# chymaera96/NeuralSampleID

Measured on AMD Instinct MI355X. Metric: audio clips/sec (contrastive step, grafp encoder), higher is better.
Workload: dtype bf16; 1 GPU; B=256 bf16 k=3 hipGraph 2-stream: grafp.yaml GraphEncoder('t') full contrastive step (fwd x2 views + NT-Xent + bwd + clip + Adam), synthetic (64,128) log-mel clip pairs per GPU, random-init weights; global_batch=256, k=3, parallelism=dp1, collectives=none (single process), gemm_arithmetic=bf16 MFMA operands, fp32 accumulate, activation_storage=bf16, views=two HIP streams (parallel graph branches), hipgraph=True

## Files before the change

include/nsid.h:

```cpp
#ifndef NSID_H
#define NSID_H
#include <stddef.h>
#include <stdint.h>

#ifdef __cplusplus
extern "C" {
#endif

#define NSID_OK 0
#define NSID_EINVAL (-1)
#define NSID_ELAUNCH (-2)

#define NSID_ACT_NONE 0
#define NSID_ACT_RELU 1
#define NSID_ACT_LEAKY 2
#define NSID_ACT_ELU 3

#define NSID_ROW_TILE 128

#define NSID_F32 0
#define NSID_BF16 1

#define NSID_GEMM_FP32 0
#define NSID_GEMM_BF16 1

int nsid_version(void);
int nsid_debug_gemm_trace(void* device_buf);
int nsid_debug_knn_trace(void* device_buf);
int nsid_set_gemm_precision(int mode);
int nsid_get_gemm_precision(void);
int nsid_set_tuning(const char* key, long value);
int nsid_get_tuning(const char* key, long* value);
int nsid_reset_tuning(void);
int nsid_tuning_count(void);
const char* nsid_tuning_key(int i);
long nsid_debug_counter(const char* key);
int nsid_debug_counters_reset(void);
int nsid_debug_counter_count(void);
const char* nsid_debug_counter_key(int i);
long nsid_gemm_g256_launches(void);
int nsid_row_tiles(int M);
long nsid_workspace_bytes(const char* op, long rows, long cols);

int nsid_linear_fwd(const void* x, int ldx, const void* w, int w_dtype, const float* bias, void* out, int ldo, int M,
                    int Nout, int K, int groups, const float* in_scale, const float* in_shift, int act_in, int act_out,
                    float* stat, int ksplit, int act_dtype , void* stream);
int nsid_linear_fwd_res(const void* x, int ldx, const void* w, int w_dtype, const float* bias, const void* addend, int ldadd,
                        void* out, int ldo, int M, int Nout, int K, int groups, const float* in_scale,
                        const float* in_shift, int act_in, int act_dtype, void* stream);
int nsid_ffn_fused_fwd(const void* x, const void* w1, const float* b1, const void* w2, const float* b2, void* out, int M, int C,
                       int H, void* stream);
int nsid_mrconv_fused_fwd(const void* y, const int32_t* idx, int B, int N, int C, int k, const void* w, const float* bias, void* out,
                          void* stream);
int nsid_linear_bwd_data(const void* dout, int ldd, const void* w, int w_dtype, const void* addend, int ldadd,
                         void* din, int ldi, int M, int Nout, int K, int groups,
                         int act_dtype , void* stream);
int nsid_linear_bwd_data_bn(const void* dout, int ldd, const void* w, int w_dtype, const void* addend, int ldadd,
                            void* din, int ldi, int M, int Nout, int K, int groups, int act_dtype, const void* bn_r,
                            const float* bn_scale, const float* bn_shift, const float* bn_mean, const float* bn_invstd,
                            int bn_act, float* bn_partial, void* stream);
int nsid_linear_bwd_data_bnapply(const void* dy, const void* r, const float* coef4, int act, void* dr, const void* w, int w_dtype,
                                 const void* addend, int ldadd, void* din, int ldi, int M, int Nout, int K, int groups,
                                 int act_dtype, const void* bn_r, const float* bn_scale, const float* bn_shift,
                                 const float* bn_mean, const float* bn_invstd, int bn_act, float* bn_partial, void* stream);
int nsid_linear_bwd_weight(const void* dout, int ldd, const void* x, int ldx, float* dw, int M, int Nout, int K,
                           int groups, const float* in_scale, const float* in_shift, int act_in,
                           int act_dtype , void* stream);
typedef struct nsid_wgrad_problem {
  const void* dout[2];
  const void* x[2];
  const float* in_scale[2];
  const float* in_shift[2];
  float* dw;
  int ldd, ldx, M, Nout, K, groups, act_in;
  int ds_out_nodes;
} nsid_wgrad_problem;
int nsid_linear_bwd_weight_grouped(const nsid_wgrad_problem* problems, int n, int act_dtype,
                                   int max_workgroups ,
                                   void* stream);
int nsid_colsum_acc(const void* x, int ldx, int M, int C, float* out, int dtype, void* stream);

int nsid_bn_finalize(const float* stat, int tiles, int C, int M, const float* gamma, const float* beta,
                     float* running_mean, float* running_var, int64_t* num_batches_tracked, float momentum,
                     float eps, float* scale, float* shift, float* mean, float* invstd, void* stream);
int nsid_bn_finalize_deferred(const float* stat, int tiles, int C, int M, const float* gamma, const float* beta, float eps,
                              float* scale, float* shift, float* mean, float* invstd, float* uvar, void* stream);
int nsid_bn_running_update(int n, const int* C, float* const* running_mean, float* const* running_var,
                           int64_t* const* num_batches_tracked, const float* const* mean_a, const float* const* uvar_a,
                           const float* const* mean_b, const float* const* uvar_b, float momentum, void* stream);
int nsid_bn_eval_affine(const float* gamma, const float* beta, const float* running_mean, const float* running_var,
                        float eps, int C, float* scale, float* shift, void* stream);
int nsid_bn_apply(const void* r, const float* scale, const float* shift, int act, const void* residual,
                  void* out, int M, int C, int dtype, void* stream);
int nsid_bn_bwd_reduce(const void* dout, const void* r, int M, int C, const float* scale, const float* shift,
                       const float* mean, const float* invstd, int act, float* partial, int dtype, void* stream);
int nsid_bn_bwd_finalize(const float* partial, int tiles, int C, int M, float* dgamma, float* dbeta, float* coef,
                         void* stream);
int nsid_bn_bwd_finalize_fused(const float* partial, int tiles, int C, int M, float* dgamma, float* dbeta, float* coef,
                               const float* scale, const float* shift, const float* mean, const float* invstd, float* coef4,
                               void* stream);
int nsid_bn_bwd_apply(const void* dout, const void* r, int M, int C, const float* scale, const float* shift,
                      const float* mean, const float* invstd, int act, const float* coef, void* dr, int dtype,
                      void* stream);

int nsid_knn_graph(const void* r, int ldr, const float* scale, const float* shift, int B, int N, int C, int k,
                   int dilation, int32_t* idx, int dtype, void* stream);

int nsid_mr_aggregate_fwd(const void* r, int ldr, const float* scale, const float* shift, const int32_t* idx, int B,
                          int N, int C, int k, void* u, uint8_t* argmax, int dtype, void* stream);
int nsid_mr_aggregate_bwd(const void* du, const int32_t* idx, const uint8_t* argmax, int B, int N, int C, int k,
                          void* dy, int dtype, void* stream);
int nsid_mr_aggregate_bwd_bn(const void* du, const int32_t* idx, const uint8_t* argmax, int B, int N, int C, int k, void* dy,
                             const void* bn_r, int bn_ldr, const float* bn_scale, const float* bn_shift, const float* bn_mean,
                             const float* bn_invstd, int bn_act, float* partial, int dtype, void* stream);

int nsid_batched_index_select_fwd(const float* x, const int32_t* idx, int B, int C, int N, int Nq, int k, float* out,
                                  void* stream);
int nsid_batched_index_select_bwd(const float* dout, const int32_t* idx, int B, int C, int N, int Nq, int k,
                                  float* dx , void* stream);

int nsid_downsample3_fwd(const void* x, int B, int N, int C, const void* wp, int w_dtype, const float* bias, void* out,
                         int Cout, float* stat, int act_dtype, void* stream);
int nsid_downsample3_bwd_weight(const void* dout, const void* x, float* dwp , int B, int N, int C, int Cout,
                                int act_dtype, void* stream);
int nsid_downsample3_bwd_data(const void* dout, const void* wp, const void* w_odd, int w_dtype, void* dx, int B, int N,
                              int C, int Cout, int act_dtype, void* stream);
int nsid_pack_ds_weight_bwd(const float* w, int Cout, int Cin, float* w_odd, void* stream);
int nsid_im2col3_fwd(const void* x, int B, int N, int C, void* col, int dtype, void* stream);
int nsid_im2col3_bwd(const void* dcol, int B, int N, int C, void* dx, int dtype, void* stream);
int nsid_pack_ds_weight(const float* w, int Cout, int Cin, float* wp, void* stream);
int nsid_dsact_fwd(const void* x, int B, int N, int C, const float* in_scale, const float* in_shift, int act_in, const float* w,
                   const float* bias, void* out, int Cout, float* stat, const float* out_scale, const float* out_shift, int act_out,
                   int act_dtype, void* stream);
int nsid_dsact_bwd_weight(const void* dout, const void* x, const float* in_scale, const float* in_shift, int act_in,
                          float* dw , int B, int N, int C, int Cout, int act_dtype, void* stream);
int nsid_dsact_bwd_data(const void* dout, const float* w, void* dx, int B, int N, int C, int Cout, const void* r_prev,
                        const float* scale, const float* shift, const float* mean, const float* invstd, int act, float* partial,
                        int act_dtype, void* stream);
int nsid_dsact_part_rows(int B, int N);
#define NSID_DS_PREPACK_MAX_LAYERS 8
int nsid_ds_prepack(int n, const float* const* w, void* const* wp16, void* const* wb16, float* const* dwp, const int* Cout,
                    const int* Cin, void* stream);
int nsid_unpack_ds_wgrad(const float* dwp, int Cout, int Cin, float* dw , void* stream);

int nsid_peak_patchify_fwd(const float* spec, const float* w, const float* bias, int B, int H, int W, int pb, int pf,
                           int F, void* out, int ldo, float* minmax, int out_dtype, void* stream);
int nsid_peak_patchify_bwd(const float* spec, const float* minmax, const void* out, const void* dout, int ldo,
                           int B, int H, int W, int pb, int pf, int F, float* dw , float* dbias ,
                           int out_dtype, void* stream);
int nsid_peak_patchify_bwd_ws(const float* spec, const float* minmax, const void* out, const void* dout, int ldo, int B, int H,
                              int W, int pb, int pf, int F, float* dw, float* dbias, float* ws, int out_dtype, void* stream);

int nsid_node_mean_fwd(const void* x, int B, int N, int C, float* out, int x_dtype, void* stream);
int nsid_node_mean_bwd(const float* dout, int B, int N, int C, void* dx, int dx_dtype, void* stream);
int nsid_elu_bwd(const float* dout, const float* out, long n, float* din, void* stream);
int nsid_l2norm_fwd(const float* p, int B, int d, float eps, float* z, float* norm, void* stream);
int nsid_l2norm_bwd(const float* dz, const float* z, const float* norm, int B, int d, float eps, float* dp,
                    void* stream);

int nsid_reflect_pad(const float* x, long L, int pad, float* out, void* stream);
int nsid_power_mel_db(const float* spec, long ld, int n_freq, const float* fb, const int* band, int n_mels, int T,
                      float* out, void* stream);
int nsid_unfold_segments(const float* logmel, int n_mels, int T, int n_frames, int step, int S, float* out, void* stream);
int nsid_logmel_fft(const float* wave, long in_stride, int B, long L, int n_fft, int hop, const float* window,
                    const float* twiddle, const float* fb, const int* band, int n_mels, float* out, long out_clip_stride,
                    long out_mel_stride, void* stream);

#define NSID_CQT_GROUP_BINS 8
#define NSID_CQT_RC 256
int nsid_cqt(const float* wave, long in_stride, int B, long L, int hop, int width, int n_bins, const int* groups, int n_groups,
             const float* taps, long taps_len, const float* scale, float* out, long out_clip_stride, long out_bin_stride,
             void* stream);

#define NSID_PACK_COLS 4
#define NSID_LOGMEL_RUN 8
#define NSID_CQT_TILE 32
int nsid_logmel_fft_ragged(const float* pack, const long* songs, int n_songs, long max_len, long total_runs, long total_cols,
                           int n_fft, int hop, const float* window, const float* twiddle, const float* fb, const int* band,
                           int n_mels, float* out, long ld, void* stream);
int nsid_cqt_ragged(const float* pack, const long* songs, int n_songs, long max_len, long total_tiles, long total_cols, int hop,
                    int width, int n_bins, const int* groups, int n_groups, const float* taps, long taps_len, const float* scale,
                    float* out, long ld, void* stream);
int nsid_unfold_segments_ragged(const float* spec, long ld, int n_rows, int n_frames, const long* seg_col, long s0, int nseg,
                                float* out, void* stream);

#define NSID_AUG_N_FFT 2048
#define NSID_AUG_HOP 512
#define NSID_AUG_BINS 1025
#define NSID_AUG_ZEROS 64
#define NSID_AUG_PRECISION 512
int nsid_aug_stft(const float* x_i, long stride_i, const float* x_j, long stride_j, int B, long L, const float* gain,
                  const float* window, const float* twiddle, float* spec, void* stream);
int nsid_aug_vocoder(const float* spec, int B, long L, const float* rate, float rate_lo, float rate_hi, float* out,
                     long T_out_max, void* stream);
int nsid_aug_istft(const float* spec, long T_out_max, int B, long L, const float* rate, float rate_lo, float rate_hi,
                   const float* window, const float* twiddle, float* wave, long wave_stride, void* stream);
int nsid_aug_finish(const float* wave, long wave_stride, int B, long L, const int* mode, const float* rate, float rate_lo,
                    float rate_hi, const float* table, float* out, long out_stride, void* stream);

#define NSID_AUG_FX_MAX_SECTIONS 64
#define NSID_AUG_FX_MAX_FRAMES 256
int nsid_aug_compress(const float* x, long stride_x, int B, long L, const int* mode1, const double* cmp, float* out, long stride_o,
                      void* stream);
int nsid_aug_biquad(const float* x, long stride_x, int B, long L, const int* mode1, const double* sos, int S, const int* n_sec,
                    float* out, long stride_o, void* stream);
int nsid_aug_frames(const float* x_i, long stride_i, const float* t1, long stride_t, const float* gain, int B, long L,
                    const int* mode2, const int* frame_size, const int* frame_ops, int F, float* out, long stride_o, void* stream);

#define NSID_RESAMPLE_MAX_C 8
#define NSID_RESAMPLE_LDS_BYTES 65536
int nsid_resample_sinc(const float* x, long stride_x, int C, long T, int orig, int nw, int width, const float* table,
                       const int* first, int ntap, int ts, float* y, long T_out, void* stream);
int nsid_stem_pairs_gate(const float* bank, long bank_elems, const long* base, const int* length, int n_tracks, const int* track,
                         const int* start, const float* key, const int* off_i, const int* off_j, int N, long L, long O, float silence,
                         int* status, float* snr, int* plan, void* stream);
int nsid_stem_pairs_build(const float* bank, long bank_elems, const long* base, const int* length, int n_tracks, const int* track,
                          const int* start, const int* off_i, const int* off_j, const int* status, const int* plan, int N, long L,
                          long O, int packed, int B_out, float* x_i, long stride_i, float* x_j, long stride_j, int* n_ok, void* stream);

int nsid_f32_to_bf16(const float* src, void* dst, long n, void* stream);

size_t nsid_ntxent_ws_floats(int Bg);
int nsid_ntxent_fwd_bwd(const float* z_i, const float* z_j, int Bg, int d, float tau, int p0, int np, float* ws,
                        float* loss_out, float* dz_i, float* dz_j, void* stream);

#define NSID_BL_MAX 2048
size_t nsid_baseline_loss_ws_floats(int M, int D);
int nsid_pair_ce_fwd_bwd(const float* z_i, const float* z_j, int B, int D, float* ws, float* out, float* dz_i, float* dz_j,
                         void* stream);
int nsid_triplet_fwd_bwd(const float* e, const int64_t* labels, int M, int D, double margin, float* ws, float* out, float* de,
                         void* stream);
int nsid_baseline_objective_fwd_bwd(const float* z_i, const float* z_j, int B, int D, double margin, double beta, double gamma,
                                    float* ws, float* out, float* dz_i, float* dz_j, void* stream);

#define NSID_BL_ROWS_MAX 4096
size_t nsid_baseline_loss_rows_ws_floats(int M, int D);
int nsid_baseline_objective_rows_fwd_bwd(const float* z_i_all, const float* z_j_all, int Bg, int D, int p0, int npairs,
                                         double margin, double beta, double gamma, float* ws, float* out, float* dz_i, float* dz_j,
// ... 125 lines not shown
```

neuralsampleid_amd/csrc/bn.hip:

```cpp
#include <cstdlib>
#include "nsid_common.h"

namespace {

constexpr int FIN_THREADS = 1024;

template <int FIN_CH>
__device__ __forceinline__ void tile_sums(const float* __restrict__ p0, const float* __restrict__ p1, int tiles,
                                          int C, int c, int tg, bool ok, double* red0, double* red1, double& sum,
                                          double& sq) {
  constexpr int FIN_TG = FIN_THREADS / FIN_CH;
  double a = 0.0, b = 0.0;
  if (ok) {
    constexpr int UB = 8;
    int t = tg;
    for (; t + (UB - 1) * FIN_TG < tiles; t += UB * FIN_TG) {
      float va[UB], vb[UB];
#pragma unroll
      for (int u = 0; u < UB; ++u) {
        va[u] = p0[(long)(t + u * FIN_TG) * C + c];
        vb[u] = p1[(long)(t + u * FIN_TG) * C + c];
      }
#pragma unroll
      for (int u = 0; u < UB; ++u) { a += (double)va[u]; b += (double)vb[u]; }
// ... 234 lines not shown
  long b = (nchunks + 255) / 256;
  const long cap = nsid_tune(NSID_T_stream_max_wg);
  return (int)(b > cap ? cap : (b < 1 ? 1 : b));
}

template <typename T>
__global__ __launch_bounds__(256) void colsum_atomic_kernel(const T* __restrict__ x, long ld, int M, int C,
                                                            float* __restrict__ out) {
  constexpr int N = Chunk<T>::N;
  constexpr int CQ = CR_CH / N, RG = 256 / CQ, ROWS = NSID_ROW_TILE / RG;
  __shared__ float red[RG][CR_CH];
  const int row0 = blockIdx.x * NSID_ROW_TILE;
  const int t = threadIdx.x, q = t % CQ, rgp = t / CQ;
  const int c = blockIdx.y * CR_CH + N * q;
  float s[N];
#pragma unroll
  for (int e = 0; e < N; ++e) s[e] = 0.f;
  if (c < C)
    for (int i = 0; i < ROWS; ++i) {
      const int row = row0 + rgp + RG * i;
      if (row < M) {
        float d[N];
        Chunk<T>::load(x + (long)row * ld + c, d);
#pragma unroll
        for (int e = 0; e < N; ++e) s[e] += d[e];
      }
    }
#pragma unroll
  for (int e = 0; e < N; ++e) red[rgp][N * q + e] = s[e];
  __syncthreads();
  if (t < CR_CH && blockIdx.y * CR_CH + t < C) {
    float a = 0.f;
    for (int g = 0; g < RG; ++g) a += red[g][t];
    atomicAdd(out + blockIdx.y * CR_CH + t, a);
  }
}

inline long chunk_keeping_grid(long nchunks, int CV, int U, long max_wg, bool* capped) {
  int g0 = CV, d256 = 256;
  while (d256 % 2 == 0 && g0 % 2 == 0) { d256 /= 2; g0 /= 2; }
  long want = (nchunks + 256L * U - 1) / (256L * U);
  if (capped) *capped = want > max_wg;
  if (want > max_wg) want = max_wg;
  if (want < 1) want = 1;
  return (want + g0 - 1) / g0 * g0;
}

inline int bn_fin_ch(int tiles) {
  const int t = (int)nsid_tune(NSID_T_bn_fin_tiles);
  return (t > 0 && tiles >= t) ? 16 : 64;
}
#define NSID_FIN_LAUNCH(kernel, tiles, C, stream, ...)                                                                      \
  do {                                                                                                                       \
    if (bn_fin_ch(tiles) == 16)                                                                                              \
      NSID_LAUNCH(kernel<16>, dim3(((C) + 15) / 16), dim3(FIN_THREADS), 0, static_cast<hipStream_t>(stream), __VA_ARGS__);   \
    else                                                                                                                     \
      NSID_LAUNCH(kernel<64>, dim3(((C) + 63) / 64), dim3(FIN_THREADS), 0, static_cast<hipStream_t>(stream), __VA_ARGS__);   \
  } while (0)

}

extern "C" int nsid_bn_finalize(const float* stat, int tiles, int C, int M, const float* gamma, const float* beta,
                                float* running_mean, float* running_var, int64_t* nbt, float momentum, float eps,
                                float* scale, float* shift, float* mean, float* invstd, void* stream) {
  NSID_REQUIRE(stat && gamma && beta && scale && shift && mean && invstd && C > 0 && M > 0);
  NSID_REQUIRE(tiles == nsid_row_tiles(M) || (tiles > 0 && tiles <= NSID_STEM7_STAT_MAX));
  NSID_REQUIRE((running_mean == nullptr) == (running_var == nullptr));
  NSID_FIN_LAUNCH(bn_finalize_kernel, tiles, C, stream, stat, tiles, C, M, gamma, beta, running_mean, running_var, nbt,
              momentum, eps, scale, shift, mean, invstd, static_cast<float*>(nullptr));
  return nsid_launch_status();
}

extern "C" int nsid_bn_finalize_deferred(const float* stat, int tiles, int C, int M, const float* gamma,
                                         const float* beta, float eps, float* scale, float* shift, float* mean,
                                         float* invstd, float* uvar, void* stream) {
  NSID_REQUIRE(stat && gamma && beta && scale && shift && mean && invstd && uvar && C > 0 && M > 0);
  NSID_REQUIRE(tiles == nsid_row_tiles(M));
  NSID_FIN_LAUNCH(bn_finalize_kernel, tiles, C, stream, stat, tiles, C, M, gamma, beta, static_cast<float*>(nullptr),
              static_cast<float*>(nullptr), static_cast<int64_t*>(nullptr), 0.f, eps, scale, shift, mean, invstd, uvar);
  return nsid_launch_status();
}

namespace {
constexpr int RU_LAYERS = 16;
struct RunUpdArgs {
  float* rm[RU_LAYERS]; float* rv[RU_LAYERS]; int64_t* nbt[RU_LAYERS];
  const float* mean_a[RU_LAYERS]; const float* uvar_a[RU_LAYERS];
  const float* mean_b[RU_LAYERS]; const float* uvar_b[RU_LAYERS];
  int C[RU_LAYERS];
  float momentum;
};
__global__ __launch_bounds__(256) void bn_running_update_kernel(const RunUpdArgs a) {
  const int l = blockIdx.x;
  const float m = a.momentum;
  const bool two = a.mean_b[l] != nullptr;
  if (threadIdx.x == 0 && a.nbt[l] != nullptr) *a.nbt[l] += two ? 2 : 1;
  for (int c = threadIdx.x; c < a.C[l]; c += blockDim.x) {
    float rm = running_blend(a.rm[l][c], a.mean_a[l][c], m);
    float rv = running_blend(a.rv[l][c], a.uvar_a[l][c], m);
    if (two) {
      rm = running_blend(rm, a.mean_b[l][c], m);
      rv = running_blend(rv, a.uvar_b[l][c], m);
    }
    a.rm[l][c] = rm;
    a.rv[l][c] = rv;
  }
}
}

extern "C" int nsid_bn_running_update(int n, const int* C, float* const* running_mean, float* const* running_var,
                                      int64_t* const* num_batches_tracked, const float* const* mean_a,
                                      const float* const* uvar_a, const float* const* mean_b,
                                      const float* const* uvar_b, float momentum, void* stream) {
  NSID_REQUIRE(n > 0 && C && running_mean && running_var && mean_a && uvar_a);
  for (int base = 0; base < n; base += RU_LAYERS) {
    RunUpdArgs a{};
    const int cnt = n - base < RU_LAYERS ? n - base : RU_LAYERS;
    for (int i = 0; i < cnt; ++i) {
      NSID_REQUIRE(C[base + i] > 0 && running_mean[base + i] && running_var[base + i] && mean_a[base + i] && uvar_a[base + i]);
      a.rm[i] = running_mean[base + i]; a.rv[i] = running_var[base + i];
      a.nbt[i] = num_batches_tracked ? num_batches_tracked[base + i] : nullptr;
      a.mean_a[i] = mean_a[base + i]; a.uvar_a[i] = uvar_a[base + i];
      a.mean_b[i] = mean_b ? mean_b[base + i] : nullptr; a.uvar_b[i] = uvar_b ? uvar_b[base + i] : nullptr;
      NSID_REQUIRE((a.mean_b[i] == nullptr) == (a.uvar_b[i] == nullptr));
      a.C[i] = C[base + i];
    }
    a.momentum = momentum;
    NSID_LAUNCH(bn_running_update_kernel, dim3(cnt), dim3(256), 0, static_cast<hipStream_t>(stream), a);
    const int rc = nsid_launch_status();
    if (rc != NSID_OK) return rc;
  }
  return NSID_OK;
}

extern "C" int nsid_bn_eval_affine(const float* gamma, const float* beta, const float* running_mean,
                                   const float* running_var, float eps, int C, float* scale, float* shift,
                                   void* stream) {
  NSID_REQUIRE(gamma && beta && running_mean && running_var && scale && shift && C > 0);
  NSID_LAUNCH(bn_eval_affine_kernel, dim3((C + 127) / 128), dim3(128), 0, static_cast<hipStream_t>(stream), gamma, beta,
              running_mean, running_var, eps, C, scale, shift);
  return nsid_launch_status();
}

extern "C" int nsid_bn_apply(const void* r, const float* scale, const float* shift, int act, const void* residual,
                             void* out, int M, int C, int dtype, void* stream) {
  NSID_REQUIRE(r && scale && shift && out && M > 0 && C > 0 && NSID_DTYPE_OK(dtype));
  NSID_REQUIRE(C % (dtype == NSID_BF16 ? 8 : 4) == 0 && nsid_aligned16(r) && nsid_aligned16(out));
  NSID_DISPATCH_DTYPE(dtype, T, {
    const long nchunks = (long)M * C / Chunk<T>::N;
    NSID_LAUNCH((bn_apply_kernel<T>), dim3(stream_grid(nchunks)), dim3(256), 0, static_cast<hipStream_t>(stream),
                static_cast<const T*>(r), scale, shift, act, static_cast<const T*>(residual), static_cast<T*>(out),
                nchunks, C / Chunk<T>::N);
  });
  return nsid_launch_status();
}

extern "C" int nsid_bn_bwd_reduce(const void* dout, const void* r, int M, int C, const float* scale,
                                  const float* shift, const float* mean, const float* invstd, int act, float* partial,
                                  int dtype, void* stream) {
  NSID_REQUIRE(dout && r && scale && shift && mean && invstd && partial && M > 0 && C > 0 && NSID_DTYPE_OK(dtype));
  NSID_REQUIRE(C % (dtype == NSID_BF16 ? 8 : 4) == 0);
  NSID_REQUIRE(act == NSID_ACT_NONE || act == NSID_ACT_RELU || act == NSID_ACT_LEAKY);
  const int tiles = nsid_row_tiles(M);
  NSID_DISPATCH_DTYPE(dtype, T, {
    NSID_LAUNCH((col_reduce_kernel<1, T>), dim3(tiles, (C + CR_CH - 1) / CR_CH), dim3(256), 0,
                static_cast<hipStream_t>(stream), static_cast<const T*>(dout), static_cast<const T*>(r), (long)C, M, C,
                scale, shift, mean, invstd, bn_slope(act), partial, tiles);
  });
  return nsid_launch_status();
}

extern "C" int nsid_bn_bwd_finalize(const float* partial, int tiles, int C, int M, float* dgamma, float* dbeta,
                                    float* coef, void* stream) {
  NSID_REQUIRE(partial && coef && C > 0 && M > 0 && tiles >= 1);
  NSID_FIN_LAUNCH(bn_bwd_finalize_kernel, tiles, C, stream, partial, tiles, C, M, dgamma, dbeta, coef, static_cast<const float*>(nullptr),
              static_cast<const float*>(nullptr), static_cast<const float*>(nullptr), static_cast<const float*>(nullptr),
              static_cast<float*>(nullptr));
  return nsid_launch_status();
}

extern "C" int nsid_bn_bwd_finalize_fused(const float* partial, int tiles, int C, int M, float* dgamma, float* dbeta,
                                          float* coef, const float* scale, const float* shift, const float* mean,
                                          const float* invstd, float* coef4, void* stream) {
  NSID_REQUIRE(partial && coef && coef4 && scale && shift && mean && invstd && C > 0 && M > 0 && tiles >= 1);
  NSID_FIN_LAUNCH(bn_bwd_finalize_kernel, tiles, C, stream, partial, tiles, C, M, dgamma, dbeta, coef, scale, shift, mean, invstd, coef4);
  return nsid_launch_status();
}

extern "C" int nsid_bn_bwd_apply(const void* dout, const void* r, int M, int C, const float* scale,
                                 const float* shift, const float* mean, const float* invstd, int act,
                                 const float* coef, void* dr, int dtype, void* stream) {
  NSID_REQUIRE(dout && r && scale && shift && mean && invstd && coef && dr && M > 0 && C > 0 && NSID_DTYPE_OK(dtype));
  NSID_REQUIRE(C % (dtype == NSID_BF16 ? 8 : 4) == 0);
  NSID_REQUIRE(act == NSID_ACT_NONE || act == NSID_ACT_RELU || act == NSID_ACT_LEAKY);
  NSID_DISPATCH_DTYPE(dtype, T, {
    constexpr int U = 4;
    const int CV = C / Chunk<T>::N;
    const long nchunks = (long)M * CV;
    int g0 = CV, d256 = 256;
    while (d256 % 2 == 0 && g0 % 2 == 0) { d256 /= 2; g0 /= 2; }
    long want = (nchunks + 256L * U - 1) / (256L * U);
    const long max_wg = nsid_tune(NSID_T_bn_bwd_apply_max_wg);
    nsid_count(NSID_C_bn_bwd_apply);
    if (want > max_wg) { want = max_wg; nsid_count(NSID_C_bn_bwd_apply_capped); }
    const long grid = (want + g0 - 1) / g0 * g0;
    NSID_LAUNCH((bn_bwd_apply_kernel<T, U>), dim3((int)grid), dim3(256), 0, static_cast<hipStream_t>(stream),
                static_cast<const T*>(dout), static_cast<const T*>(r), (long)M, CV, scale, shift, mean,
                invstd, bn_slope(act), coef, static_cast<T*>(dr));
  });
  return nsid_launch_status();
// ... 12 lines not shown
```

neuralsampleid_amd/csrc/gemm.hip:

```cpp
#include <algorithm>
#include <cstdlib>
#include "nsid_common.h"

namespace {

inline float act_slope(int act) { return act == NSID_ACT_RELU ? 0.f : (act == NSID_ACT_LEAKY ? 0.2f : 1.f); }

struct GemmArgs {
  const void* A; long lda; long a_goff;
  const void* B; long ldb; long b_goff;
  void* C; long ldc; long c_goff;
  int I, J, R;
  const float* a_scale; const float* a_shift; float a_slope; long a_aff_goff;
  const float* b_scale; const float* b_shift; float b_slope; long b_aff_goff;
  const float* bias; long bias_goff;
  const void* addend; long ldadd;
  float* stat; long stat_plane;
  long stat_ld;
  int rsplit;
  int rchunk;
  int atomic_out;
  int split_major;
  const void* bn_r; long bn_ldr;
  const float* bn_scale; const float* bn_shift; const float* bn_mean; const float* bn_invstd; float bn_slope;
// ... 632 lines not shown
                }
              p.bn_partial[((long)ti * STILES + t2) * p.bn_ld + col] = a0;
              p.bn_partial[p.bn_plane + ((long)ti * STILES + t2) * p.bn_ld + col] = a1;
            }
          }
        }
      }
    }
  }
  if (p.stat != nullptr) {
    const float* red = lds + WAVES * RB * ((BN / 2) + 4);
    if (threadIdx.x < BN) {
      const int j = j0 + threadIdx.x;
      if (FULL || j < p.J) {
        const long col = g * p.c_goff + j;
#pragma unroll
        for (int t2 = 0; t2 < STILES; ++t2) {
          float s = 0.f, q = 0.f;
#pragma unroll
          for (int k = 4 * WPT * t2; k < 4 * WPT * (t2 + 1); ++k) {
            s += red[(0 * WROWS * 4 + k) * BN + threadIdx.x];
            q += red[(1 * WROWS * 4 + k) * BN + threadIdx.x];
          }
          p.stat[((long)ti * STILES + t2) * p.stat_ld + col] = s;
          p.stat[p.stat_plane + ((long)ti * STILES + t2) * p.stat_ld + col] = q;
        }
      }
    }
  }
  if (trace && threadIdx.x == 0) {
    unsigned hw, xcc;
    asm volatile("s_getreg_b32 %0, hwreg(HW_REG_HW_ID)" : "=s"(hw));
    asm volatile("s_getreg_b32 %0, hwreg(HW_REG_XCC_ID)" : "=s"(xcc));
    const long lin = blockIdx.x + (long)gridDim.x * (blockIdx.y + (long)gridDim.y * blockIdx.z);
    trace[4 * lin + 0] = t_start;
    trace[4 * lin + 1] = t_loop;
    trace[4 * lin + 2] = __builtin_amdgcn_s_memrealtime();
    trace[4 * lin + 3] = ((unsigned long long)xcc << 32) | hw;
  }
}

template <int BM, int BN, bool A_RMAJOR, bool B_RMAJOR, bool H, bool ST, bool AAFF, bool WB = false, bool FULL = false,
          bool ARELU = false, int KS = 1, int PADX = 0, bool ABN = false>
__global__ __launch_bounds__(NT, KS > 1 ? 2 : ((FULL && WB && BM == 128 && !AAFF && (BN == 128) != ABN) ? 3 : 2))
void gemm_kernel(const GemmArgs p) {
  int bid = p.split_major ? blockIdx.y : blockIdx.x;
  const int split = p.split_major ? blockIdx.x : blockIdx.y;
  if (!p.split_major) {
    const int nwg = gridDim.x;
    if ((nwg & 7) == 0) bid = (bid & 7) * (nwg >> 3) + (bid >> 3);
  }
  gemm_body<BM, BN, A_RMAJOR, B_RMAJOR, H, ST, AAFF, WB, FULL, ARELU, KS, PADX, ABN>(p, bid, split, blockIdx.z);
}

template <int BM, int BN, bool FULL, bool H = true, bool ST = true, int PADX = 0>
__device__ __forceinline__ void wgrad_grouped_item(const WgGroupArgs& ga, const int w);

template <int BM, int BN, bool FULL, bool H = true, bool ST = true, int PADX = 0>
__global__ __launch_bounds__(256, FULL ? 1 : 2) void wgrad_grouped_kernel(const WgGroupArgs ga) {
  const int total = ga.wg0[ga.n];
  for (int w = blockIdx.x; w < total; w += gridDim.x) wgrad_grouped_item<BM, BN, FULL, H, ST, PADX>(ga, w);
}

template <int BM, int BN, bool FULL, bool H, bool ST, int PADX>
__device__ __forceinline__ void wgrad_grouped_item(const WgGroupArgs& ga, const int w) {
  int pi, split, bid, g, seg;
  if (!wgg_decode(ga, w, pi, split, bid, g, seg)) return;
  const WgProb& q = ga.prob[pi];
  GemmArgs p{};
  p.A = q.A[seg]; p.lda = q.lda; p.a_goff = q.I;
  p.B = q.B[seg]; p.ldb = q.ldb; p.b_goff = q.J;
  p.C = q.C; p.ldc = q.J; p.c_goff = (long)q.I * q.J;
  p.I = q.I; p.J = q.J; p.R = q.R;
  p.b_scale = q.bsc[seg]; p.b_shift = q.bsh[seg]; p.b_slope = q.slope; p.b_aff_goff = q.J;
  p.a_slope = 1.f; p.bn_slope = 1.f;
  p.atomic_out = 1;
  p.rchunk = q.rchunk; p.rsplit = q.nsplit;
  if constexpr (PADX == 2) {
    p.pad_period = q.pad_period; p.pad_phase = 0; p.pad_c0 = 0; p.pad_c1 = q.pad_c1; p.pad_safe = q.pad_c1;
  }
  gemm_body<BM, BN, false, false, H, ST, false, false, FULL, false, FULL ? 2 : 1, PADX>(p, bid, split, g);
}

__global__ void elu_inplace_kernel(float* __restrict__ x, long rows, int cols, long ld) {
  const long n = rows * cols;
  for (long i = (long)blockIdx.x * blockDim.x + threadIdx.x; i < n; i += (long)gridDim.x * blockDim.x) {
    float* q = x + (i / cols) * ld + (i % cols);
    const float v = *q;
    *q = v > 0.f ? v : expm1f(v);
  }
}

int g_gemm_precision = NSID_GEMM_FP32;
long g_g256_launches = 0;

template <int BM, int BN, bool AR, bool BR>
int launch(GemmArgs p, int groups, hipStream_t s, int act_dtype, bool w_bf16 = false) {
  const int tiles = ((p.I + BM - 1) / BM) * ((p.J + BN - 1) / BN);
  const bool st16 = act_dtype == NSID_BF16;
  const bool half = g_gemm_precision == NSID_GEMM_BF16 || st16;
  const int bk = half ? 32 : 16;
  p.rchunk = (p.rchunk + bk - 1) / bk * bk;
  p.rsplit = (p.R + p.rchunk - 1) / p.rchunk;
  p.split_major = p.rsplit > 1 && (p.rsplit % 8) == 0;
  dim3 grid(p.split_major ? p.rsplit : tiles, p.split_major ? tiles : p.rsplit, groups);
  constexpr bool CAN_AFF = AR && BR;
  const bool aff = CAN_AFF && p.a_scale != nullptr;
#define NSID_GEMM_GO(HH, SS)                                                                              \
  do {                                                                                                    \
    if (aff) NSID_LAUNCH((gemm_kernel<BM, BN, AR, BR, HH, SS, CAN_AFF>), grid, dim3(256), 0, s, p);        \
    else NSID_LAUNCH((gemm_kernel<BM, BN, AR, BR, HH, SS, false>), grid, dim3(256), 0, s, p);              \
  } while (0)
  const bool full = st16 && p.I % BM == 0 && p.J % BN == 0 && p.rchunk % (2 * bk) == 0 && p.R % p.rchunk == 0;
  const long deep_maxwg = nsid_tune(NSID_T_gemm_deep_max_wg);
  const int deep_kinds = (int)nsid_tune(NSID_T_gemm_deep_kinds);
  constexpr int kind_bit = AR ? (BR ? 1 : 2) : 4;
  const long wgs = (long)tiles * p.rsplit * groups;
  const int ks = (full && wgs <= deep_maxwg && nsid_tune(NSID_T_gemm_deep_ks) == 2 && (deep_kinds & kind_bit) && p.rchunk % 128 == 0) ? 2 : 1;
  if (p.abn_r != nullptr) {
    if (!(AR && !BR && BM == 128)) return NSID_EINVAL;
    if (!(st16 && w_bf16 && full)) return 1;
  }
  nsid_count(AR ? (BR ? NSID_C_gemm_fwd : NSID_C_gemm_bwd_data) : NSID_C_gemm_bwd_weight);
  if (p.split_major) nsid_count(NSID_C_gemm_split_major);
  if (aff) nsid_count(NSID_C_gemm_affine_load);
  if (AR && !BR && p.bn_r != nullptr) nsid_count(NSID_C_gemm_bn_sums);
  if (!AR) nsid_count(BM == BN ? NSID_C_wgrad_square : NSID_C_wgrad_rect);
  {
    const bool deep_path = st16 && full && (AR ? w_bf16 : true);
    if (deep_path) {
      nsid_count(NSID_C_gemm_full);
      if (ks == 2) nsid_count(NSID_C_gemm_ks2);
    }
  }
#define NSID_GEMM_DEEP_GO(AFF_, WB_, RELU_)                                                                                  \
  do {                                                                                                                       \
    if (ks == 2) NSID_LAUNCH((gemm_kernel<BM, BN, AR, BR, true, true, AFF_, WB_, true, RELU_, 2>), grid, dim3(256), 0, s, p); \
    else NSID_LAUNCH((gemm_kernel<BM, BN, AR, BR, true, true, AFF_, WB_, true, RELU_>), grid, dim3(256), 0, s, p);           \
  } while (0)
  if (p.abn_r != nullptr) {
    if constexpr (AR && !BR && BM == 128) {
      nsid_count(NSID_C_gemm_bn_apply_load);
      NSID_LAUNCH((gemm_kernel<BM, BN, AR, BR, true, true, false, true, true, false, 1, 0, true>), grid, dim3(256), 0, s, p);
      return nsid_launch_status();
    } else {
      return NSID_EINVAL;
    }
  }
  if constexpr (AR) {
    if (st16 && w_bf16) {
      const bool act_only = CAN_AFF && p.a_scale == nullptr && p.a_slope != 1.f;
      if (act_only) {
        if constexpr (CAN_AFF) {
          if (!full || p.a_slope != 0.f) return NSID_EINVAL;
          NSID_GEMM_DEEP_GO(false, true, true);
        }
      } else if (full) {
        if (aff) NSID_GEMM_DEEP_GO(CAN_AFF, true, false);
        else NSID_GEMM_DEEP_GO(false, true, false);
      } else {
        if (aff) NSID_LAUNCH((gemm_kernel<BM, BN, AR, BR, true, true, CAN_AFF, true>), grid, dim3(256), 0, s, p);
        else NSID_LAUNCH((gemm_kernel<BM, BN, AR, BR, true, true, false, true>), grid, dim3(256), 0, s, p);
      }
      return nsid_launch_status();
    }
  } else {
    if (st16 && full) {
      NSID_GEMM_DEEP_GO(false, false, false);
// ... 54 lines not shown
  p.bias = bias; p.bias_goff = Cout;
  p.stat = stat; p.stat_ld = Cout; p.stat_plane = (long)nsid_row_tiles(M) * Cout;
  p.rsplit = 1; p.rchunk = 3 * C;
  p.pad_period = No; p.pad_phase = 0; p.pad_c0 = 0; p.pad_c1 = C; p.pad_safe = C;
  hipStream_t s = static_cast<hipStream_t>(stream);
  const bool wb = w_dtype == NSID_BF16;
  if (Cout <= 64) return launch_pad<128, 64, true, true, 1>(p, 1, s, act_dtype, wb);
  return launch_pad<128, 128, true, true, 1>(p, 1, s, act_dtype, wb);
}


extern "C" int nsid_downsample3_bwd_weight(const void* dout, const void* x, float* dwp, int B, int N, int C, int Cout,
                                           int act_dtype, void* stream) {
  NSID_REQUIRE(dout && x && dwp && B > 0 && N > 0 && N % 2 == 0 && C > 0 && Cout > 0 && NSID_DTYPE_OK(act_dtype));
  const int ch = act_dtype == NSID_BF16 ? 8 : 4;
  NSID_REQUIRE(C % ch == 0 && Cout % ch == 0 && nsid_aligned16(dout) && nsid_aligned16(x));
  const int No = N / 2, M = B * No;
  const long esz = act_dtype == NSID_BF16 ? 2 : 4;
  GemmArgs p{};
  p.A = dout; p.lda = Cout; p.a_goff = Cout;
  p.B = static_cast<const char*>(x) - (long)C * esz; p.ldb = 2L * C; p.b_goff = 3L * C;
  p.C = dwp; p.ldc = 3L * C; p.c_goff = (long)Cout * 3 * C;
  p.I = Cout; p.J = 3 * C; p.R = M;
  p.b_slope = 1.f;
  p.atomic_out = 1;
  p.pad_period = No; p.pad_phase = 0; p.pad_c0 = 0; p.pad_c1 = C; p.pad_safe = C;
  const long tiles = (long)((Cout + 63) / 64) * ((3 * C + 63) / 64);
  long S = std::min<long>((M + 1023) / 1024, std::max<long>(1, 1024 / tiles));
  S = std::max<long>(S, (256 + tiles - 1) / tiles);
  S = std::min<long>(S, (M + 255) / 256);
  p.rsplit = (int)std::max<long>(S, 1);
  p.rchunk = (M + p.rsplit - 1) / p.rsplit;
  return launch_pad<64, 64, false, false, 2>(p, 1, static_cast<hipStream_t>(stream), act_dtype, false);
}

extern "C" int nsid_downsample3_bwd_data(const void* dout, const void* wp, const void* w_odd, int w_dtype, void* dx, int B,
                                         int N, int C, int Cout, int act_dtype, void* stream) {
  NSID_REQUIRE(dout && wp && w_odd && dx && B > 0 && N > 0 && N % 2 == 0 && C > 0 && Cout > 0 && NSID_DTYPE_OK(act_dtype));
  const int ch = act_dtype == NSID_BF16 ? 8 : 4;
  NSID_REQUIRE(C % ch == 0 && Cout % ch == 0 && nsid_aligned16(dout) && nsid_aligned16(wp) && nsid_aligned16(w_odd) &&
               nsid_aligned16(dx) && NSID_DTYPE_OK(w_dtype) && (w_dtype == NSID_F32 || act_dtype == NSID_BF16));
  const int No = N / 2, M = B * No;
  const long esz = act_dtype == NSID_BF16 ? 2 : 4, wsz = w_dtype == NSID_BF16 ? 2 : 4;
  hipStream_t s = static_cast<hipStream_t>(stream);
  const bool wb = w_dtype == NSID_BF16;
  GemmArgs p{};
  p.A = dout; p.lda = Cout; p.a_goff = Cout;
  p.B = static_cast<const char*>(wp) + (long)C * wsz; p.ldb = 3L * C; p.b_goff = 0;
  p.C = dx; p.ldc = 2L * C; p.c_goff = C;
  p.I = M; p.J = C; p.R = Cout;
  p.rsplit = 1; p.rchunk = Cout;
  p.bn_slope = 1.f;
  int rc = C <= 64 ? launch<128, 64, true, false>(p, 1, s, act_dtype, wb) : launch<128, 128, true, false>(p, 1, s, act_dtype, wb);
  if (rc != NSID_OK) return rc;
  GemmArgs q{};
  q.A = dout; q.lda = Cout; q.a_goff = 2L * Cout;
  q.B = w_odd; q.ldb = C; q.b_goff = 0;
  q.C = static_cast<char*>(dx) + (long)C * esz; q.ldc = 2L * C; q.c_goff = C;
  q.I = M; q.J = C; q.R = 2 * Cout;
  q.rsplit = 1; q.rchunk = 2 * Cout;
  q.bn_slope = 1.f;
  q.pad_period = No; q.pad_phase = No - 1; q.pad_c0 = Cout; q.pad_c1 = 2 * Cout; q.pad_safe = 0;
  return C <= 64 ? launch_pad<128, 64, true, false, 1>(q, 1, s, act_dtype, wb)
                 : launch_pad<128, 128, true, false, 1>(q, 1, s, act_dtype, wb);
}

void* g_gemm_trace_host = nullptr;
extern "C" int nsid_debug_gemm_trace(void* buf) {
  g_gemm_trace_host = buf;
  return hipMemcpyToSymbol(HIP_SYMBOL(g_gemm_trace), &buf, sizeof(buf)) == hipSuccess ? NSID_OK : NSID_EINVAL;
}
extern "C" int nsid_set_gemm_precision(int mode) {
  if (mode != NSID_GEMM_FP32 && mode != NSID_GEMM_BF16) return NSID_EINVAL;
  g_gemm_precision = mode;
  return NSID_OK;
}
extern "C" int nsid_get_gemm_precision(void) { return g_gemm_precision; }
extern "C" long nsid_gemm_g256_launches(void) { return g_g256_launches; }
extern "C" int nsid_row_tiles(int M) { return (M + NSID_ROW_TILE - 1) / NSID_ROW_TILE; }

static int linear_fwd_impl(const void* x, int ldx, const void* w, int w_dtype, const float* bias, void* out, int ldo,
                           int M, int Nout, int K, int groups, const float* in_scale, const float* in_shift, int act_in,
                           int act_out, float* stat, int ksplit, int act_dtype, const void* addend, int ldadd,
                           void* stream);

extern "C" int nsid_linear_fwd(const void* x, int ldx, const void* w, int w_dtype, const float* bias, void* out, int ldo,
                               int M, int Nout, int K, int groups, const float* in_scale, const float* in_shift,
                               int act_in, int act_out, float* stat, int ksplit, int act_dtype, void* stream) {
  return linear_fwd_impl(x, ldx, w, w_dtype, bias, out, ldo, M, Nout, K, groups, in_scale, in_shift, act_in, act_out, stat,
                         ksplit, act_dtype, nullptr, 0, stream);
}

extern "C" int nsid_linear_fwd_res(const void* x, int ldx, const void* w, int w_dtype, const float* bias,
                                   const void* addend, int ldadd, void* out, int ldo, int M, int Nout, int K, int groups,
                                   const float* in_scale, const float* in_shift, int act_in, int act_dtype,
                                   void* stream) {
  const int ch = act_dtype == NSID_BF16 ? 8 : 4;
  NSID_REQUIRE(addend && ldadd % ch == 0 && ldadd >= groups * Nout && nsid_aligned16(addend));
  return linear_fwd_impl(x, ldx, w, w_dtype, bias, out, ldo, M, Nout, K, groups, in_scale, in_shift, act_in,
                         NSID_ACT_NONE, nullptr, 1, act_dtype, addend, ldadd, stream);
}

static int linear_fwd_impl(const void* x, int ldx, const void* w, int w_dtype, const float* bias, void* out, int ldo,
                           int M, int Nout, int K, int groups, const float* in_scale, const float* in_shift, int act_in,
                           int act_out, float* stat, int ksplit, int act_dtype, const void* addend, int ldadd,
                           void* stream) {
  NSID_REQUIRE(x && w && out && M > 0 && Nout > 0 && K > 0 && groups > 0 && ksplit >= 1 && NSID_DTYPE_OK(act_dtype));
  NSID_REQUIRE(NSID_DTYPE_OK(w_dtype) && (w_dtype == NSID_F32 || (act_dtype == NSID_BF16 && K % 8 == 0)));
  const int ch = act_dtype == NSID_BF16 ? 8 : 4;
  NSID_REQUIRE(K % ch == 0 && ldx % ch == 0 && nsid_aligned16(x) && nsid_aligned16(w) && K % 4 == 0);
  NSID_REQUIRE(act_dtype == NSID_F32 || (ksplit == 1 && (act_out == NSID_ACT_NONE || act_out == NSID_ACT_RELU) && Nout % 8 == 0 && ldo % 8 == 0));
  NSID_REQUIRE(act_out != NSID_ACT_RELU || (ksplit == 1 && stat == nullptr && addend == nullptr));
  NSID_REQUIRE((ldx >= groups * K || (groups == 1 && ldx > 0)) && ldo >= groups * Nout);
  NSID_REQUIRE(Nout % 4 == 0 && ldo % 4 == 0 && nsid_aligned16(out) && (bias == nullptr || nsid_aligned16(bias)));
  NSID_REQUIRE((in_scale == nullptr) == (in_shift == nullptr));
  NSID_REQUIRE(ksplit == 1 || (stat == nullptr && (act_out == NSID_ACT_NONE || (act_out == NSID_ACT_ELU && act_dtype == NSID_F32))));
  NSID_REQUIRE(act_in != NSID_ACT_ELU && (act_out == NSID_ACT_NONE || act_out == NSID_ACT_ELU || act_out == NSID_ACT_RELU));
  NSID_REQUIRE(in_scale != nullptr || act_in == NSID_ACT_NONE ||
               (act_in == NSID_ACT_RELU && act_dtype == NSID_BF16 && w_dtype == NSID_BF16));
  GemmArgs p{};
  p.A = x; p.lda = ldx; p.a_goff = K;
  p.B = w; p.ldb = K; p.b_goff = (long)Nout * K;
  p.C = out; p.ldc = ldo; p.c_goff = Nout;
  p.I = M; p.J = Nout; p.R = K;
  p.a_scale = in_scale; p.a_shift = in_shift; p.a_slope = act_slope(act_in); p.a_aff_goff = K;
  p.bias = bias; p.bias_goff = Nout;
  p.addend = addend; p.ldadd = ldadd;
  p.stat = stat; p.stat_ld = (long)groups * Nout; p.stat_plane = (long)nsid_row_tiles(M) * groups * Nout;
  p.rsplit = ksplit;
  p.rchunk = (K + ksplit - 1) / ksplit;
  p.atomic_out = ksplit > 1;
  p.relu_out = act_out == NSID_ACT_RELU;
  hipStream_t s = static_cast<hipStream_t>(stream);
  const long t128 = (long)nsid_row_tiles(M) * ((Nout + 127) / 128) * groups;
  const bool half = g_gemm_precision == NSID_GEMM_BF16 || act_dtype == NSID_BF16;
  const int force_narrow = (int)nsid_tune(NSID_T_fwd_narrow);
  bool narrow = half ? (Nout <= 64 || (Nout <= 128 && K <= 256 && in_scale == nullptr)) : Nout <= 64;
  if (half && t128 < 128) narrow = true;
  if (force_narrow >= 0 && Nout > 64) narrow = force_narrow != 0;
  const bool wb = w_dtype == NSID_BF16;
  if ((nsid_tune(NSID_T_ws_gemm) & 1) && act_dtype == NSID_BF16 && wb && ksplit == 1 && act_out == NSID_ACT_NONE && addend == nullptr &&
      act_in != NSID_ACT_ELU) {
    const int rcw = nsid_ws_fwd_launch(x, ldx, w, bias, out, ldo, M, Nout, K, groups, in_scale, in_shift, act_slope(act_in), stat,
                                       p.stat_plane, p.stat_ld, s);
    if (rcw != 1) { nsid_count(NSID_C_ws_fwd); return rcw; }
  }
  const long g256_min = nsid_tune(NSID_T_g256_min);
  if (g256_min > 0 && (stat == nullptr || nsid_tune(NSID_T_g256_train) != 0) && act_dtype == NSID_BF16 && wb && groups == 1 && in_scale == nullptr && ksplit == 1 &&
      (act_out == NSID_ACT_NONE || act_out == NSID_ACT_RELU) && act_in == NSID_ACT_NONE && ldx >= K &&
      (long)(M / 256) * (Nout / 256) >= g256_min) {
    const int rc256 = nsid_gemm256_fwd_launch(x, ldx, w, bias, addend, ldadd, out, ldo, M, Nout, K, act_out == NSID_ACT_RELU, stat,
                                              p.stat_plane, p.stat_ld, s);
    if (rc256 != 1) { ++g_g256_launches; nsid_count(NSID_C_gemm256); return rc256; }
  }
  const int rc = narrow ? launch<128, 64, true, true>(p, groups, s, act_dtype, wb) : launch<128, 128, true, true>(p, groups, s, act_dtype, wb);
  if (rc != NSID_OK || act_out != NSID_ACT_ELU) return rc;
  const long n = (long)M * groups * Nout;
  NSID_LAUNCH(elu_inplace_kernel, dim3((int)((n + 255) / 256 > 2048 ? 2048 : (n + 255) / 256)), dim3(256), 0, s,
              static_cast<float*>(out), (long)M, groups * Nout, (long)ldo);
  return nsid_launch_status();
}

struct AbnArgs {
  const void* r; const float* coef4; int act; void* dr;
};
static int linear_bwd_data_impl(const void* dout, int ldd, const void* w, int w_dtype, const void* addend, int ldadd,
                                void* din, int ldi, int M, int Nout, int K, int groups, int act_dtype, void* stream,
                                const void* bn_r, const float* bn_scale, const float* bn_shift, const float* bn_mean,
                                const float* bn_invstd, int bn_act, float* bn_partial, const AbnArgs* abn = nullptr);

extern "C" int nsid_linear_bwd_data(const void* dout, int ldd, const void* w, int w_dtype, const void* addend, int ldadd,
                                    void* din, int ldi, int M, int Nout, int K, int groups, int act_dtype,
                                    void* stream) {
  return linear_bwd_data_impl(dout, ldd, w, w_dtype, addend, ldadd, din, ldi, M, Nout, K, groups, act_dtype, stream,
                              nullptr, nullptr, nullptr, nullptr, nullptr, NSID_ACT_NONE, nullptr);
}

extern "C" int nsid_linear_bwd_data_bn(const void* dout, int ldd, const void* w, int w_dtype, const void* addend,
                                       int ldadd, void* din, int ldi, int M, int Nout, int K, int groups, int act_dtype,
                                       const void* bn_r, const float* bn_scale, const float* bn_shift,
                                       const float* bn_mean, const float* bn_invstd, int bn_act, float* bn_partial,
                                       void* stream) {
  NSID_REQUIRE(bn_r && bn_scale && bn_shift && bn_mean && bn_invstd && bn_partial && act_dtype == NSID_BF16);
  NSID_REQUIRE(ldi == groups * K && (groups * K) % 8 == 0 && nsid_aligned16(bn_r));
  NSID_REQUIRE(bn_act == NSID_ACT_NONE || bn_act == NSID_ACT_RELU || bn_act == NSID_ACT_LEAKY);
  return linear_bwd_data_impl(dout, ldd, w, w_dtype, addend, ldadd, din, ldi, M, Nout, K, groups, act_dtype, stream,
                              bn_r, bn_scale, bn_shift, bn_mean, bn_invstd, bn_act, bn_partial);
}

extern "C" int nsid_linear_bwd_data_bnapply(const void* dy, const void* r, const float* coef4, int act, void* dr, const void* w,
                                            int w_dtype, const void* addend, int ldadd, void* din, int ldi, int M, int Nout, int K,
                                            int groups, int act_dtype, const void* bn_r, const float* bn_scale,
                                            const float* bn_shift, const float* bn_mean, const float* bn_invstd, int bn_act,
                                            float* bn_partial, void* stream) {
  NSID_REQUIRE(dy && r && coef4 && dr && nsid_aligned16(r) && nsid_aligned16(dr) && nsid_aligned16(coef4));
  NSID_REQUIRE(dr != dy && dr != r);
  NSID_REQUIRE(act == NSID_ACT_NONE || act == NSID_ACT_RELU || act == NSID_ACT_LEAKY);
  if (act_dtype != NSID_BF16 || w_dtype != NSID_BF16 || (groups * Nout) % 8 != 0) return 1;
  if (bn_r != nullptr) {
    NSID_REQUIRE(bn_scale && bn_shift && bn_mean && bn_invstd && bn_partial && ldi == groups * K && (groups * K) % 8 == 0 &&
                 nsid_aligned16(bn_r));
    NSID_REQUIRE(bn_act == NSID_ACT_NONE || bn_act == NSID_ACT_RELU || bn_act == NSID_ACT_LEAKY);
  }
  const AbnArgs abn{r, coef4, act, dr};
  return linear_bwd_data_impl(dy, groups * Nout, w, w_dtype, addend, ldadd, din, ldi, M, Nout, K, groups, act_dtype, stream, bn_r,
                              bn_scale, bn_shift, bn_mean, bn_invstd, bn_act, bn_partial, &abn);
}

static int linear_bwd_data_impl(const void* dout, int ldd, const void* w, int w_dtype, const void* addend, int ldadd,
                                void* din, int ldi, int M, int Nout, int K, int groups, int act_dtype, void* stream,
                                const void* bn_r, const float* bn_scale, const float* bn_shift, const float* bn_mean,
                                const float* bn_invstd, int bn_act, float* bn_partial, const AbnArgs* abn) {
  NSID_REQUIRE(dout && w && din && M > 0 && Nout > 0 && K > 0 && groups > 0 && NSID_DTYPE_OK(act_dtype));
  NSID_REQUIRE(NSID_DTYPE_OK(w_dtype) && (w_dtype == NSID_F32 || (act_dtype == NSID_BF16 && K % 8 == 0)));
  const bool wb = w_dtype == NSID_BF16;
  const int ch = act_dtype == NSID_BF16 ? 8 : 4;
  NSID_REQUIRE(Nout % ch == 0 && K % ch == 0 && ldd % ch == 0 && ldi % ch == 0 && nsid_aligned16(dout) && nsid_aligned16(w));
  NSID_REQUIRE(addend == nullptr || ldadd % ch == 0);
  NSID_REQUIRE(ldd >= groups * Nout && ldi >= groups * K && ldi % 4 == 0 && nsid_aligned16(din));
  NSID_REQUIRE(addend == nullptr || (ldadd % 4 == 0 && ldadd >= groups * K && nsid_aligned16(addend)));
  GemmArgs p{};
  p.A = dout; p.lda = ldd; p.a_goff = Nout;
  p.B = w; p.ldb = K; p.b_goff = (long)Nout * K;
  p.C = din; p.ldc = ldi; p.c_goff = K;
  p.I = M; p.J = K; p.R = Nout;
  p.addend = addend; p.ldadd = ldadd;
  p.rsplit = 1; p.rchunk = Nout;
  p.bn_r = bn_r; p.bn_ldr = (long)groups * K;
  p.bn_scale = bn_scale; p.bn_shift = bn_shift; p.bn_mean = bn_mean; p.bn_invstd = bn_invstd;
  p.bn_slope = act_slope(bn_act);
  p.bn_partial = bn_partial; p.bn_ld = (long)groups * K; p.bn_plane = (long)nsid_row_tiles(M) * groups * K;
  hipStream_t s = static_cast<hipStream_t>(stream);
  const long t128 = (long)nsid_row_tiles(M) * ((K + 127) / 128) * groups;
  const bool half = g_gemm_precision == NSID_GEMM_BF16 || act_dtype == NSID_BF16;
  const int force_narrow = (int)nsid_tune(NSID_T_bwd_narrow);
  bool narrow = half ? (K <= 64 || (K <= 128 && Nout <= 256)) : K <= 64;
  if (half && t128 < 128) narrow = true;
  if (force_narrow >= 0 && K > 64) narrow = force_narrow != 0;
  if ((nsid_tune(NSID_T_ws_gemm) & (abn ? 4 : 2)) && act_dtype == NSID_BF16 && wb &&
      (bn_r == nullptr || bn_partial != nullptr)) {
    const int rcw = nsid_ws_bwd_data_launch(dout, ldd, w, addend, ldadd, din, ldi, M, Nout, K, groups, bn_r, p.bn_ldr, bn_scale, bn_shift,
                                            bn_mean, bn_invstd, p.bn_slope, bn_partial, p.bn_plane, p.bn_ld, abn ? abn->r : nullptr,
                                            abn ? abn->coef4 : nullptr, (long)groups * Nout, abn ? act_slope(abn->act) : 1.f,
                                            abn ? abn->dr : nullptr, (long)groups * Nout, s);
    if (rcw != 1) { nsid_count(abn ? NSID_C_ws_bwd_bnapply : NSID_C_ws_bwd_data); return rcw; }
  }
  if (abn != nullptr) {
    narrow = K <= 64;
    p.abn_r = abn->r; p.abn_coef = abn->coef4; p.abn_plane = (long)groups * Nout; p.abn_slope = act_slope(abn->act);
    p.abn_dr = abn->dr; p.abn_lddr = (long)groups * Nout;
    if (K % (narrow ? 64 : 128) != 0 || M % 128 != 0 || Nout % 64 != 0) return 1;
  }
  if (act_dtype == NSID_F32 && addend == nullptr && bn_r == nullptr && abn == nullptr && groups == 1 && Nout >= 1024 && ldi == K) {
    const long tiles = (long)nsid_row_tiles(M) * ((K + (narrow ? 63 : 127)) / (narrow ? 64 : 128));
    const long maxt = nsid_tune(NSID_T_bwd_split_max_tiles);
    const long S = maxt > 0 && tiles <= maxt ? std::min<long>(256 / tiles, Nout / 256) : 1;
    if (S > 1) {
      const int rcz = nsid_fill_zero(din, (size_t)M * K * 4, stream);
      if (rcz != NSID_OK) return rcz;
      p.rsplit = (int)S;
      p.rchunk = (int)((Nout + S - 1) / S);
      p.atomic_out = 1;
      nsid_count(NSID_C_gemm_bwd_split);
    }
  }
  if (narrow) return launch<128, 64, true, false>(p, groups, s, act_dtype, wb);
  return launch<128, 128, true, false>(p, groups, s, act_dtype, wb);
}

extern "C" int nsid_linear_bwd_weight(const void* dout, int ldd, const void* x, int ldx, float* dw, int M, int Nout,
                                      int K, int groups, const float* in_scale, const float* in_shift, int act_in,
                                      int act_dtype, void* stream) {
  NSID_REQUIRE(dout && x && dw && M > 0 && Nout > 0 && K > 0 && groups > 0 && NSID_DTYPE_OK(act_dtype));
  const int ch = act_dtype == NSID_BF16 ? 8 : 4;
  NSID_REQUIRE(Nout % ch == 0 && K % ch == 0 && ldd % ch == 0 && ldx % ch == 0 && nsid_aligned16(dout) && nsid_aligned16(x));
  NSID_REQUIRE((in_scale == nullptr) == (in_shift == nullptr));
  GemmArgs p{};
  p.A = dout; p.lda = ldd; p.a_goff = Nout;
  p.B = x; p.ldb = ldx; p.b_goff = K;
  p.C = dw; p.ldc = K; p.c_goff = (long)Nout * K;
  p.I = Nout; p.J = K; p.R = M;
  p.b_scale = in_scale; p.b_shift = in_shift; p.b_slope = act_slope(act_in); p.b_aff_goff = K;
  p.atomic_out = 1;
  const bool use_wide = nsid_tune(NSID_T_wgrad_wide) != 0;
  if (use_wide && act_dtype == NSID_BF16 && nsid_aligned16(dout) && nsid_aligned16(x) &&
      (in_scale == nullptr || (nsid_aligned16(in_scale) && nsid_aligned16(in_shift)))) {
    const int rc = nsid_wgrad2_launch(dout, ldd, x, ldx, dw, M, Nout, K, groups, in_scale, in_shift, act_slope(act_in),
                                      static_cast<hipStream_t>(stream));
    if (rc != 1) return rc;
  }
  const long rect = nsid_tune(NSID_T_wgrad_rect);
  const long wg_rect = nsid_tune(NSID_T_wgrad_wgs_rect);
  const long wg_sq = nsid_tune(NSID_T_wgrad_wgs_sq);
  if (rect && act_dtype == NSID_BF16 && Nout % 128 == 0 && K % 64 == 0 && M % 1024 == 0) {
    const long tiles_r = (long)(Nout / 128) * (K / 64) * groups;
    const long S = std::min<long>(M / 1024, std::max<long>(1, wg_rect / tiles_r));
    const long rect_min = nsid_tune(NSID_T_wgrad_rect_min);
    if (tiles_r * S >= rect_min) {
      p.rsplit = (int)S;
      p.rchunk = (int)(M / S);
      return launch<128, 64, false, false>(p, groups, static_cast<hipStream_t>(stream), act_dtype);
    }
  }
  const bool half = g_gemm_precision == NSID_GEMM_BF16 || act_dtype == NSID_BF16;
  const long t128 = (long)((Nout + 127) / 128) * ((K + 127) / 128) * groups;
  const bool small = half || (Nout <= 64 || K <= 64) || t128 * ((M + 511) / 512) < 256;
  const int bm = small ? 64 : 128;
  const long tiles = (long)((Nout + bm - 1) / bm) * ((K + bm - 1) / bm) * groups;
  long S;
  if (half) {
    S = std::min<long>((M + 1023) / 1024, std::max<long>(1, wg_sq / tiles));
    const long sq_min = nsid_tune(NSID_T_wgrad_sq_min);
    S = std::max<long>(S, (sq_min + tiles - 1) / tiles);
    S = std::min<long>(S, (M + 255) / 256);
  } else {
    S = std::min<long>((512 + tiles - 1) / tiles, (M + 511) / 512);
  }
  int rsplit = (int)std::max<long>(S, 1);
  p.rsplit = rsplit;
  p.rchunk = (M + rsplit - 1) / rsplit;
  hipStream_t s = static_cast<hipStream_t>(stream);
  if (small) return launch<64, 64, false, false>(p, groups, s, act_dtype);
  return launch<128, 128, false, false>(p, groups, s, act_dtype);
}

extern "C" int nsid_linear_bwd_weight_grouped(const nsid_wgrad_problem* problems, int n, int act_dtype, int max_workgroups,
                                              void* stream) {
  NSID_REQUIRE(problems && n > 0 && NSID_DTYPE_OK(act_dtype) && max_workgroups >= 0);
  const bool st16 = act_dtype == NSID_BF16;
  const int ch = st16 ? 8 : 4;
  hipStream_t s = static_cast<hipStream_t>(stream);
  const long rows_target = std::max<long>(128, nsid_tune(NSID_T_wgg_rows));
  const long rows_sq = std::max<long>(128, nsid_tune(NSID_T_wgg_rows_sq)), rows_gen = std::max<long>(32, nsid_tune(NSID_T_wgg_rows_gen));
  const bool use_w3 = nsid_tune(NSID_T_wgg_w3) != 0;
  const bool use_w4 = nsid_tune(NSID_T_wgrad256) != 0;
  const long rows_w4 = std::max<long>(128, nsid_tune(NSID_T_wgg_rows256));
  constexpr int NCLS = 8;
  WgGroupArgs ga[NCLS];
  long wgs[NCLS] = {0, 0, 0, 0, 0, 0, 0, 0};
  const bool half = g_gemm_precision == NSID_GEMM_BF16 || st16;
  for (int c = 0; c < NCLS; ++c) ga[c].n = 0;
// ... 102 lines not shown
```

neuralsampleid_amd/csrc/misc.hip:

```cpp
#include <algorithm>
#include "nsid_common.h"

namespace {

inline int grid_for(long n, int cap = 2048) {
  long b = (n + 255) / 256;
  return (int)(b > cap ? cap : (b < 1 ? 1 : b));
}

template <typename T>
__global__ __launch_bounds__(256) void im2col3_fwd_kernel(const T* __restrict__ x, int B, int N, int No, int C,
                                                          T* __restrict__ col) {
  constexpr int NV = Chunk<T>::N;
  const int CV = C / NV;
  const long total = (long)B * No * 3 * CV;
  for (long q = (long)blockIdx.x * blockDim.x + threadIdx.x; q < total; q += (long)gridDim.x * blockDim.x) {
    const int cv = (int)(q % CV);
    const int t = (int)((q / CV) % 3);
    const long orow = q / (3L * CV);
    const int b = (int)(orow / No), no = (int)(orow % No);
    const int n = 2 * no - 1 + t;
    float v[NV];
#pragma unroll
    for (int e = 0; e < NV; ++e) v[e] = 0.f;
// ... 308 lines not shown
__global__ __launch_bounds__(256) void patchify_bwd2_kernel(const float* __restrict__ spec, const float* __restrict__ minmax,
                                                            const T* __restrict__ out, const T* __restrict__ dout, int ldo,
                                                            float* __restrict__ ws) {
  constexpr int H = 64, W = 128, PBk = 4, PFk = 8, F = 8, Hp = 16, Wp = 16, NP = 256, LDW = W + PATCH_PAD;
  __shared__ __attribute__((aligned(16))) float g[NP * F];
  __shared__ __attribute__((aligned(16))) float xs[H * LDW];
  __shared__ float red[(Wp + Hp) * F];
  const int t = threadIdx.x, b = blockIdx.x;
  const float* x = spec + (long)b * H * W;
  const float lo = minmax[2 * b], range = minmax[2 * b + 1] - lo;
  {
    const long o = ((long)b * NP + t) * ldo;
    float ov[8], dv[8];
    if constexpr (Chunk<T>::N == 8) {
      Chunk<T>::load(out + o, ov);
      Chunk<T>::load(dout + o, dv);
    } else {
      Chunk<T>::load(out + o, ov); Chunk<T>::load(out + o + 4, ov + 4);
      Chunk<T>::load(dout + o, dv); Chunk<T>::load(dout + o + 4, dv + 4);
    }
    f32x4 v[8];
#pragma unroll
    for (int u = 0; u < 8; ++u) v[u] = *reinterpret_cast<const f32x4*>(x + 4 * (t + 256 * u));
#pragma unroll
    for (int e = 0; e < 8; ++e) g[t * F + e] = ov[e] > 0.f ? dv[e] : 0.f;
#pragma unroll
    for (int u = 0; u < 8; ++u) {
      const int i4 = 4 * (t + 256 * u), hh = i4 / W, ww = i4 % W;
      *reinterpret_cast<f32x4*>(xs + hh * LDW + ww) =
          f32x4{(v[u][0] - lo) / range, (v[u][1] - lo) / range, (v[u][2] - lo) / range, (v[u][3] - lo) / range};
    }
  }
  __syncthreads();
  {
    const int f = t % F, k2 = t / F;
    float a = 0.f;
    if (k2 < Wp) { for (int ph = 0; ph < Hp; ++ph) a += g[(ph * Wp + k2) * F + f]; }
    else { for (int pw = 0; pw < Wp; ++pw) a += g[((k2 - Wp) * Wp + pw) * F + f]; }
    red[t] = a;
  }
  __syncthreads();
  const int f = t >> 5, ij = t & 31, i = ij >> 3, j = ij & 7;
  float a_t = 0.f, a_f = 0.f;
#pragma unroll
  for (int q = 0; q < 16; ++q) {
    a_t += red[q * F + f] * linspace01(q * PFk + j, W);
    a_f += red[(Wp + q) * F + f] * linspace01(q * PBk + i, H);
  }
  float part[4] = {0.f, 0.f, 0.f, 0.f};
  for (int ph = 0; ph < Hp; ++ph) {
    const float* srow = g + (ph * Wp) * F + f;
    const float* xrow = xs + (ph * PBk + i) * LDW + j;
#pragma unroll
    for (int pw = 0; pw < Wp; ++pw) part[pw & 3] += srow[pw * F] * xrow[pw * PFk];
  }
  float* wsb = ws + (long)b * PB2_OUT;
  wsb[f * 96 + ij] = a_t;
  wsb[f * 96 + 32 + ij] = a_f;
  wsb[f * 96 + 64 + ij] = (part[0] + part[1]) + (part[2] + part[3]);
  if (t < F) {
    float a = 0.f;
    for (int pw = 0; pw < Wp; ++pw) a += red[pw * F + t];
    wsb[768 + t] = a;
  }
}

__global__ __launch_bounds__(256) void patchify_bwd2_reduce_kernel(const float* __restrict__ ws, int B, float* __restrict__ dw,
                                                                   float* __restrict__ dbias) {
  __shared__ float part[256];
  const int t = threadIdx.x, q = blockIdx.x * 64 + (t & 63), sl = t >> 6;
  float a = 0.f;
  if (q < PB2_OUT)
    for (int b = sl; b < B; b += 4) a += ws[(long)b * PB2_OUT + q];
  part[t] = a;
  __syncthreads();
  if (sl == 0 && q < PB2_OUT) {
    a = (part[t] + part[t + 64]) + (part[t + 128] + part[t + 192]);
    atomicAdd(q < 768 ? dw + q : dbias + (q - 768), a);
  }
}

template <typename T>
__global__ __launch_bounds__(256) void node_mean_fwd_kernel(const T* __restrict__ x, int N, int C,
                                                            float* __restrict__ out) {
  constexpr int NV = Chunk<T>::N;
  const int b = blockIdx.x, CV = C / NV;
  for (int cv = blockIdx.y * blockDim.x + threadIdx.x; cv < CV; cv += gridDim.y * blockDim.x) {
    float s[NV];
#pragma unroll
    for (int e = 0; e < NV; ++e) s[e] = 0.f;
    for (int n = 0; n < N; ++n) {
      float v[NV];
      Chunk<T>::load(x + ((long)b * N + n) * C + NV * cv, v);
#pragma unroll
      for (int e = 0; e < NV; ++e) s[e] += v[e];
    }
#pragma unroll
    for (int e = 0; e < NV; ++e) out[(long)b * C + NV * cv + e] = s[e] / (float)N;
  }
}
template <typename T>
__global__ __launch_bounds__(256) void node_mean_bwd_kernel(const float* __restrict__ dout, int N, int C,
                                                            long nchunks, T* __restrict__ dx) {
  constexpr int NV = Chunk<T>::N;
  const int CV = C / NV;
  for (long q = (long)blockIdx.x * blockDim.x + threadIdx.x; q < nchunks; q += (long)gridDim.x * blockDim.x) {
    const int cv = (int)(q % CV);
    const long b = q / ((long)CV * N);
    float v[NV];
#pragma unroll
    for (int e = 0; e < NV; ++e) v[e] = dout[b * C + NV * cv + e] / (float)N;
    Chunk<T>::store(dx + q * NV, v);
  }
}

__global__ void elu_bwd_kernel(const float* __restrict__ dout, const float* __restrict__ out, long n,
                               float* __restrict__ din) {
  for (long i = (long)blockIdx.x * blockDim.x + threadIdx.x; i < n; i += (long)gridDim.x * blockDim.x) {
    const float o = out[i];
    din[i] = dout[i] * (o > 0.f ? 1.f : o + 1.f);
  }
}

__global__ __launch_bounds__(256) void l2norm_fwd_kernel(const float* __restrict__ p, int B, int d, float eps,
                                                         float* __restrict__ z, float* __restrict__ norm) {
  const int row = blockIdx.x * 4 + (threadIdx.x >> 6), lane = threadIdx.x & 63;
  if (row >= B) return;
  float ss = 0.f;
  for (int c = lane; c < d; c += 64) { const float v = p[(long)row * d + c]; ss += v * v; }
  ss = wave_sum(ss);
  const float nr = sqrtf(ss), den = fmaxf(nr, eps);
  for (int c = lane; c < d; c += 64) z[(long)row * d + c] = p[(long)row * d + c] / den;
  if (lane == 0) norm[row] = nr;
}
__global__ __launch_bounds__(256) void l2norm_bwd_kernel(const float* __restrict__ dz, const float* __restrict__ z,
                                                         const float* __restrict__ norm, int B, int d, float eps,
                                                         float* __restrict__ dp) {
  const int row = blockIdx.x * 4 + (threadIdx.x >> 6), lane = threadIdx.x & 63;
  if (row >= B) return;
  float dot = 0.f;
  for (int c = lane; c < d; c += 64) dot += z[(long)row * d + c] * dz[(long)row * d + c];
  dot = wave_sum(dot);
  const float nr = norm[row];
  for (int c = lane; c < d; c += 64) {
    const long o = (long)row * d + c;
    dp[o] = nr > eps ? (dz[o] - z[o] * dot) / nr : dz[o] / eps;
  }
}

constexpr int SUMSQ_PER_BLOCK = 256 * 4 * 16;
__global__ __launch_bounds__(256) void sumsq_kernel(const float* __restrict__ g, long n, float* __restrict__ partial) {
  __shared__ double red[4];
  const long base = (long)blockIdx.x * SUMSQ_PER_BLOCK;
  double s = 0.0;
  for (int it = 0; it < 16; ++it) {
    const long i = base + ((long)it * 256 + threadIdx.x) * 4;
    if (i + 3 < n) {
      const f32x4 v = *reinterpret_cast<const f32x4*>(g + i);
      s += (double)v[0] * v[0] + (double)v[1] * v[1] + (double)v[2] * v[2] + (double)v[3] * v[3];
    } else {
      for (long j = i; j < n && j < i + 4; ++j) s += (double)g[j] * g[j];
    }
  }
  s = wave_sum_d(s);
  if ((threadIdx.x & 63) == 0) red[threadIdx.x >> 6] = s;
  __syncthreads();
  if (threadIdx.x == 0) partial[blockIdx.x] = (float)(red[0] + red[1] + red[2] + red[3]);
}

__global__ __launch_bounds__(256) void adam_kernel(float* __restrict__ p, const float* __restrict__ g,
                                                   float* __restrict__ m, float* __restrict__ v, long n,
                                                   const float* __restrict__ hyper, const int64_t* __restrict__ step,
                                                   const float* __restrict__ partial, int nblocks,
                                                   float* __restrict__ gnorm_out) {
  __shared__ float coef_s;
  __shared__ int skip_s;
  __shared__ double red[4];
  {
    double s = 0.0;
    for (int i = threadIdx.x; i < nblocks; i += blockDim.x) s += (double)partial[i];
    s = wave_sum_d(s);
    if ((threadIdx.x & 63) == 0) red[threadIdx.x >> 6] = s;
    __syncthreads();
    if (threadIdx.x == 0) {
      const float norm = (float)sqrt(red[0] + red[1] + red[2] + red[3]);
      const float max_norm = hyper[4];
      float c = 1.f;
      if (max_norm > 0.f) { c = max_norm / (norm + 1e-6f); c = c < 1.f ? c : 1.f; }
      coef_s = c;
      skip_s = !isfinite(norm);
      if (blockIdx.x == 0 && gnorm_out != nullptr) gnorm_out[0] = norm;
    }
    __syncthreads();
  }
  if (skip_s) return;
  const float coef = coef_s;
  const float lr = hyper[0], b1 = hyper[1], b2 = hyper[2], eps = hyper[3];
  const double t = (double)(*step + 1);
  const float bc1 = (float)(1.0 - pow((double)b1, t));
  const float bc2_sqrt = (float)sqrt(1.0 - pow((double)b2, t));
// ... 81 lines not shown
extern "C" int nsid_pack_ds_weight_bwd(const float* w, int Cout, int Cin, float* wb, void* stream) {
  NSID_REQUIRE(w && wb && Cout > 0 && Cin > 0);
  NSID_LAUNCH(pack_ds_weight_bwd_kernel, dim3(grid_for(2L * Cout * Cin)), dim3(256), 0, static_cast<hipStream_t>(stream),
              w, Cout, Cin, wb);
  return nsid_launch_status();
}
extern "C" int nsid_unpack_ds_wgrad(const float* dwp, int Cout, int Cin, float* dw, void* stream) {
  NSID_REQUIRE(dwp && dw && Cout > 0 && Cin > 0);
  NSID_LAUNCH(unpack_ds_wgrad_kernel, dim3(grid_for((long)Cout * 3 * Cin)), dim3(256), 0,
                     static_cast<hipStream_t>(stream), dwp, Cout, Cin, dw);
  return nsid_launch_status();
}

extern "C" int nsid_ds_prepack(int n, const float* const* w, void* const* wp16, void* const* wb16, float* const* dwp, const int* Cout,
                               const int* Cin, void* stream) {
  NSID_REQUIRE(n > 0 && n <= DSP_LAYERS && w && wp16 && wb16 && Cout && Cin);
  DsPrepArgs a{};
  long most = 0;
  for (int i = 0; i < n; ++i) {
    NSID_REQUIRE(w[i] && wp16[i] && wb16[i] && Cout[i] > 0 && Cin[i] > 0);
    a.w[i] = w[i]; a.wp16[i] = static_cast<__bf16*>(wp16[i]); a.wb16[i] = static_cast<__bf16*>(wb16[i]);
    a.dwp[i] = dwp ? dwp[i] : nullptr; a.Cout[i] = Cout[i]; a.Cin[i] = Cin[i];
    most = std::max(most, (long)Cout[i] * 3 * Cin[i]);
  }
  NSID_LAUNCH(ds_prepack_kernel, dim3(grid_for(most, 256), n), dim3(256), 0, static_cast<hipStream_t>(stream), a);
  return nsid_launch_status();
}
extern "C" int nsid_peak_patchify_fwd(const float* spec, const float* w, const float* bias, int B, int H, int W, int pb,
                                      int pf, int F, void* out, int ldo, float* minmax, int out_dtype, void* stream) {
  NSID_REQUIRE(spec && w && bias && out && B > 0 && H > 1 && W > 1 && pb > 0 && pf > 0 && F > 0);
  NSID_REQUIRE(H % pb == 0 && W % pf == 0 && ldo >= F && NSID_DTYPE_OK(out_dtype));
  const size_t bytes = ((size_t)F * 3 * pb * pf + 8 + (size_t)H * (W + 8)) * sizeof(float);
  NSID_REQUIRE(bytes <= NSID_LDS_MAX && W % 4 == 0 && (F * 3 * pb * pf) % 4 == 0 && nsid_aligned16(spec) && pb * pf <= 64);
  NSID_DISPATCH_DTYPE(out_dtype, T, {
    if (pb == 4 && pf == 8) {
      NSID_LAUNCH_LDS((patchify_fwd_kernel<T, 32, 4, 8>), dim3(B), dim3(256), bytes, static_cast<hipStream_t>(stream), spec, w,
                      bias, H, W, pb, pf, F, static_cast<T*>(out), ldo, minmax);
    } else if (pb * pf == 32) {
      NSID_LAUNCH_LDS((patchify_fwd_kernel<T, 32>), dim3(B), dim3(256), bytes, static_cast<hipStream_t>(stream), spec, w,
                      bias, H, W, pb, pf, F, static_cast<T*>(out), ldo, minmax);
    } else {
      NSID_LAUNCH_LDS((patchify_fwd_kernel<T, 64>), dim3(B), dim3(256), bytes, static_cast<hipStream_t>(stream), spec, w,
                      bias, H, W, pb, pf, F, static_cast<T*>(out), ldo, minmax);
    }
  });
  return nsid_launch_status();
}
extern "C" int nsid_peak_patchify_bwd(const float* spec, const float* minmax, const void* out, const void* dout,
                                      int ldo, int B, int H, int W, int pb, int pf, int F, float* dw, float* dbias,
                                      int out_dtype, void* stream) {
  NSID_REQUIRE(spec && minmax && out && dout && dw && dbias && B > 0 && H % pb == 0 && W % pf == 0 && ldo >= F);
  NSID_REQUIRE(NSID_DTYPE_OK(out_dtype));
  int bands = 1;
  auto lds_bytes = [&](int nb) {
    const int Hb = H / nb;
    return ((size_t)(Hb / pb) * (W / pf) * F + (size_t)Hb * (W + 8) + (size_t)(Hb / pb + W / pf) * F) * sizeof(float);
  };
  while (lds_bytes(bands) > 64 * 1024 && (H / pb) % (2 * bands) == 0) bands *= 2;
  const size_t bytes = lds_bytes(bands);
  NSID_REQUIRE(bytes <= 64 * 1024 && (long)F * 3 * pb * pf <= 4 * 256 && F <= 256 && W % 4 == 0 && nsid_aligned16(spec));
  NSID_REQUIRE(((H / bands / pb) * (W / pf) * F) % 4 == 0 && (long)B * bands < (1L << 30));
  NSID_DISPATCH_DTYPE(out_dtype, T, {
    NSID_LAUNCH((patchify_bwd_kernel<T>), dim3(B * bands < 256 ? B * bands : 256), dim3(256), bytes, static_cast<hipStream_t>(stream),
                spec, minmax, static_cast<const T*>(out), static_cast<const T*>(dout), ldo, B, H, W, pb, pf, F, dw, dbias, bands);
  });
  return nsid_launch_status();
}

extern "C" int nsid_peak_patchify_bwd_ws(const float* spec, const float* minmax, const void* out, const void* dout, int ldo, int B,
                                         int H, int W, int pb, int pf, int F, float* dw, float* dbias, float* ws, int out_dtype,
                                         void* stream) {
  NSID_REQUIRE(spec && minmax && out && dout && dw && dbias && ws && B > 0 && ldo >= F && NSID_DTYPE_OK(out_dtype));
  NSID_REQUIRE(H == 64 && W == 128 && pb == 4 && pf == 8 && F == 8 && ldo % (out_dtype == NSID_BF16 ? 8 : 4) == 0);
  NSID_REQUIRE(nsid_aligned16(spec) && nsid_aligned16(out) && nsid_aligned16(dout));
  hipStream_t s = static_cast<hipStream_t>(stream);
  NSID_DISPATCH_DTYPE(out_dtype, T, {
    NSID_LAUNCH((patchify_bwd2_kernel<T>), dim3(B), dim3(256), 0, s, spec, minmax, static_cast<const T*>(out),
                static_cast<const T*>(dout), ldo, ws);
  });
  NSID_LAUNCH(patchify_bwd2_reduce_kernel, dim3((PB2_OUT + 63) / 64), dim3(256), 0, s, ws, B, dw, dbias);
  return nsid_launch_status();
}

extern "C" int nsid_node_mean_fwd(const void* x, int B, int N, int C, float* out, int x_dtype, void* stream) {
  NSID_REQUIRE(x && out && B > 0 && N > 0 && C > 0 && NSID_DTYPE_OK(x_dtype) && nsid_aligned16(x));
  const int nv = x_dtype == NSID_BF16 ? 8 : 4;
  NSID_REQUIRE(C % nv == 0);
  NSID_DISPATCH_DTYPE(x_dtype, T, {
    NSID_LAUNCH((node_mean_fwd_kernel<T>), dim3(B, (C / nv + 255) / 256), dim3(256), 0,
                static_cast<hipStream_t>(stream), static_cast<const T*>(x), N, C, out);
  });
  return nsid_launch_status();
}
extern "C" int nsid_node_mean_bwd(const float* dout, int B, int N, int C, void* dx, int dx_dtype, void* stream) {
  NSID_REQUIRE(dout && dx && B > 0 && N > 0 && C > 0 && NSID_DTYPE_OK(dx_dtype) && nsid_aligned16(dx));
  const int nv = dx_dtype == NSID_BF16 ? 8 : 4;
  NSID_REQUIRE(C % nv == 0);
  const long nchunks = (long)B * N * (C / nv);
  NSID_DISPATCH_DTYPE(dx_dtype, T, {
    NSID_LAUNCH((node_mean_bwd_kernel<T>), dim3(grid_for(nchunks)), dim3(256), 0, static_cast<hipStream_t>(stream),
                dout, N, C, nchunks, static_cast<T*>(dx));
  });
  return nsid_launch_status();
}
extern "C" int nsid_elu_bwd(const float* dout, const float* out, long n, float* din, void* stream) {
  NSID_REQUIRE(dout && out && din && n > 0);
  NSID_LAUNCH(elu_bwd_kernel, dim3(grid_for(n)), dim3(256), 0, static_cast<hipStream_t>(stream), dout, out, n,
                     din);
  return nsid_launch_status();
}
extern "C" int nsid_l2norm_fwd(const float* p, int B, int d, float eps, float* z, float* norm, void* stream) {
  NSID_REQUIRE(p && z && norm && B > 0 && d > 0);
  NSID_LAUNCH(l2norm_fwd_kernel, dim3((B + 3) / 4), dim3(256), 0, static_cast<hipStream_t>(stream), p, B, d, eps,
                     z, norm);
  return nsid_launch_status();
}
extern "C" int nsid_l2norm_bwd(const float* dz, const float* z, const float* norm, int B, int d, float eps, float* dp,
                               void* stream) {
  NSID_REQUIRE(dz && z && norm && dp && B > 0 && d > 0);
  NSID_LAUNCH(l2norm_bwd_kernel, dim3((B + 3) / 4), dim3(256), 0, static_cast<hipStream_t>(stream), dz, z, norm,
                     B, d, eps, dp);
  return nsid_launch_status();
}

extern "C" int nsid_sumsq_blocks(long n) { return (int)((n + SUMSQ_PER_BLOCK - 1) / SUMSQ_PER_BLOCK); }
extern "C" int nsid_sumsq_partial(const float* g, long n, float* partial, void* stream) {
  NSID_REQUIRE(g && partial && n > 0 && nsid_aligned16(g));
  NSID_LAUNCH(sumsq_kernel, dim3(nsid_sumsq_blocks(n)), dim3(256), 0, static_cast<hipStream_t>(stream), g, n,
                     partial);
  return nsid_launch_status();
}
extern "C" int nsid_adam_step(float* p, const float* g, float* m, float* v, long n, const float* hyper, int64_t* step,
                              const float* partial, int nblocks, float* gnorm_out, void* stream) {
  NSID_REQUIRE(p && g && m && v && hyper && step && partial && n > 0 && nblocks > 0);
  hipStream_t s = static_cast<hipStream_t>(stream);
  NSID_LAUNCH(adam_kernel, dim3(grid_for(n, 4096)), dim3(256), 0, s, p, g, m, v, n, hyper, step, partial,
                     nblocks, gnorm_out);
  NSID_LAUNCH(adam_tick_kernel, dim3(1), dim3(1), 0, s, step, (const float*)gnorm_out);
  return nsid_launch_status();
}

__global__ void reflect_pad_kernel(const float* __restrict__ x, long L, int pad, float* __restrict__ out) {
  const long n = L + 2L * pad;
  for (long i = (long)blockIdx.x * blockDim.x + threadIdx.x; i < n; i += (long)gridDim.x * blockDim.x) {
    long j = i - pad;
    if (j < 0) j = -j;
    if (j >= L) j = 2 * (L - 1) - j;
    out[i] = x[j];
  }
}

__global__ __launch_bounds__(256) void power_mel_db_kernel(const float* __restrict__ spec, long ld, int n_freq,
                                                           const float* __restrict__ fb, const int* __restrict__ band,
                                                           int n_mels, int T, float* __restrict__ out) {
  extern __shared__ float pw[];
  const int t = blockIdx.x;
  const float* row = spec + (long)t * ld;
  for (int f = threadIdx.x; f < n_freq; f += blockDim.x) {
    const float re = row[f], im = row[n_freq + f];
    pw[f] = re * re + im * im;
  }
  __syncthreads();
  for (int m = threadIdx.x; m < n_mels; m += blockDim.x) {
    float acc = 0.f;
    for (int f = band[2 * m]; f < band[2 * m + 1]; ++f) acc += fb[(long)m * n_freq + f] * pw[f];
    out[(long)m * T + t] = 10.0f * log10f(fmaxf(acc, 1e-10f));
  }
}

__global__ void unfold_segments_kernel(const float* __restrict__ lm, int n_mels, int T, int n_frames, int step, int S,
                                       float* __restrict__ out) {
  const long n = (long)S * n_mels * n_frames;
  for (long i = (long)blockIdx.x * blockDim.x + threadIdx.x; i < n; i += (long)gridDim.x * blockDim.x) {
    const int f = (int)(i % n_frames), m = (int)((i / n_frames) % n_mels);
    const long s = i / ((long)n_frames * n_mels);
    out[i] = lm[(long)m * T + s * step + f];
  }
}

__global__ void unfold_segments_ragged_kernel(const float* __restrict__ spec, long ld, int n_rows, int n_frames,
                                              const long* __restrict__ seg_col, long s0, int nseg, float* __restrict__ out) {
  const long n = (long)nseg * n_rows * n_frames;
  for (long i = (long)blockIdx.x * blockDim.x + threadIdx.x; i < n; i += (long)gridDim.x * blockDim.x) {
    const int f = (int)(i % n_frames), m = (int)((i / n_frames) % n_rows);
    const long s = i / ((long)n_frames * n_rows);
    out[i] = spec[(long)m * ld + seg_col[s0 + s] + f];
  }
}

extern "C" int nsid_unfold_segments_ragged(const float* spec, long ld, int n_rows, int n_frames, const long* seg_col, long s0,
                                           int nseg, float* out, void* stream) {
  NSID_REQUIRE(spec && seg_col && out && n_rows > 0 && n_frames > 0 && ld >= n_frames && s0 >= 0 && nseg > 0);
  nsid_count(NSID_C_unfold_segments_ragged);
  NSID_LAUNCH(unfold_segments_ragged_kernel, dim3(grid_for((long)nseg * n_rows * n_frames)), dim3(256), 0,
              static_cast<hipStream_t>(stream), spec, ld, n_rows, n_frames, seg_col, s0, nseg, out);
  return nsid_launch_status();
}

extern "C" int nsid_reflect_pad(const float* x, long L, int pad, float* out, void* stream) {
  NSID_REQUIRE(x && out && L > 1 && pad >= 0 && pad < L);
  NSID_LAUNCH(reflect_pad_kernel, dim3(grid_for(L + 2L * pad)), dim3(256), 0, static_cast<hipStream_t>(stream), x, L, pad,
              out);
  return nsid_launch_status();
}
extern "C" int nsid_power_mel_db(const float* spec, long ld, int n_freq, const float* fb, const int* band, int n_mels,
                                 int T, float* out, void* stream) {
  NSID_REQUIRE(spec && fb && band && out && n_freq > 0 && n_mels > 0 && T > 0 && ld >= 2L * n_freq);
  NSID_REQUIRE((size_t)n_freq * sizeof(float) <= 48 * 1024);
  NSID_LAUNCH(power_mel_db_kernel, dim3(T), dim3(256), (size_t)n_freq * sizeof(float), static_cast<hipStream_t>(stream),
              spec, ld, n_freq, fb, band, n_mels, T, out);
  return nsid_launch_status();
}
extern "C" int nsid_unfold_segments(const float* logmel, int n_mels, int T, int n_frames, int step, int S, float* out,
                                    void* stream) {
  NSID_REQUIRE(logmel && out && n_mels > 0 && n_frames > 0 && step > 0 && S > 0 && (long)(S - 1) * step + n_frames <= T);
  NSID_LAUNCH(unfold_segments_kernel, dim3(grid_for((long)S * n_mels * n_frames)), dim3(256), 0,
              static_cast<hipStream_t>(stream), logmel, n_mels, T, n_frames, step, S, out);
  return nsid_launch_status();
}

__global__ __launch_bounds__(256) void f32_to_bf16_kernel(const float* __restrict__ src, __bf16* __restrict__ dst, long n8) {
  for (long i = (long)blockIdx.x * blockDim.x + threadIdx.x; i < n8; i += (long)gridDim.x * blockDim.x) {
    float v[8];
    Chunk<float>::load(src + 8 * i, v);
    Chunk<float>::load(src + 8 * i + 4, v + 4);
    Chunk<__bf16>::store(dst + 8 * i, v);
  }
}
extern "C" int nsid_f32_to_bf16(const float* src, void* dst, long n, void* stream) {
  NSID_REQUIRE(src && dst && n > 0 && n % 8 == 0 && nsid_aligned16(src) && nsid_aligned16(dst));
  NSID_LAUNCH(f32_to_bf16_kernel, dim3(grid_for(n / 8, 4096)), dim3(256), 0, static_cast<hipStream_t>(stream), src,
              static_cast<__bf16*>(dst), n / 8);
  return nsid_launch_status();
}

extern "C" int nsid_bcn_to_rows(const float* x, int B, int C, int N, void* rows, int ld, int rows_dtype, void* stream) {
  NSID_REQUIRE(x && rows && B > 0 && C > 0 && N > 0 && ld >= C && NSID_DTYPE_OK(rows_dtype));
  NSID_DISPATCH_DTYPE(rows_dtype, T, {
    NSID_LAUNCH((transpose_kernel<float, T>), dim3((N + 31) / 32, (C + 31) / 32, B), dim3(256), 0,
                static_cast<hipStream_t>(stream), x, (long)C * N, (long)N, static_cast<T*>(rows), (long)N * ld, (long)ld,
                C, N);
  });
  return nsid_launch_status();
}
extern "C" int nsid_rows_to_bcn(const void* rows, int ld, int B, int C, int N, float* x, int rows_dtype, void* stream) {
  NSID_REQUIRE(x && rows && B > 0 && C > 0 && N > 0 && ld >= C && NSID_DTYPE_OK(rows_dtype));
  NSID_DISPATCH_DTYPE(rows_dtype, T, {
    NSID_LAUNCH((transpose_kernel<T, float>), dim3((C + 31) / 32, (N + 31) / 32, B), dim3(256), 0,
                static_cast<hipStream_t>(stream), static_cast<const T*>(rows), (long)N * ld, (long)ld, x, (long)C * N,
                (long)N, N, C);
  });
  return nsid_launch_status();
}

__global__ __launch_bounds__(256) void fill_zero_kernel(f32x4* __restrict__ p, long n16) {
  const f32x4 z = {0.f, 0.f, 0.f, 0.f};
  for (long i = (long)blockIdx.x * blockDim.x + threadIdx.x; i < n16; i += (long)gridDim.x * blockDim.x) p[i] = z;
}
__global__ void fill_zero_tail_kernel(unsigned char* __restrict__ p, long n) {
  for (long i = (long)blockIdx.x * blockDim.x + threadIdx.x; i < n; i += (long)gridDim.x * blockDim.x) p[i] = 0;
}
__global__ void scale_f32_kernel(const float* __restrict__ x, const float* __restrict__ s, long n, float* __restrict__ out) {
  const float f = s != nullptr ? s[0] : 1.f;
  for (long i = (long)blockIdx.x * blockDim.x + threadIdx.x; i < n; i += (long)gridDim.x * blockDim.x) out[i] = x[i] * f;
}

extern "C" int nsid_fill_zero(void* p, size_t bytes, void* stream) {
  NSID_REQUIRE(p && bytes > 0 && nsid_aligned16(p));
  const long n16 = (long)(bytes / 16);
  hipStream_t s = static_cast<hipStream_t>(stream);
  if (n16 > 0) {
    NSID_LAUNCH(fill_zero_kernel, dim3(grid_for(n16, 2048)), dim3(256), 0, s, static_cast<f32x4*>(p), n16);
    if (nsid_launch_status() != NSID_OK) return NSID_ELAUNCH;
  }
  if (bytes % 16) {
    NSID_LAUNCH(fill_zero_tail_kernel, dim3(1), dim3(64), 0, s, static_cast<unsigned char*>(p) + 16 * n16,
                (long)(bytes % 16));
    return nsid_launch_status();
  }
  return NSID_OK;
}
extern "C" int nsid_scale_f32(const float* x, const float* scale, long n, float* out, void* stream) {
  NSID_REQUIRE(x && out && n > 0);
  NSID_LAUNCH(scale_f32_kernel, dim3(grid_for(n, 1024)), dim3(256), 0, static_cast<hipStream_t>(stream), x, scale, n, out);
  return nsid_launch_status();
}
```

neuralsampleid_amd/csrc/nsid_common.h:

```cpp
#pragma once
#include <hip/hip_runtime.h>
#include <stdint.h>
#include <stdio.h>

#include "../../include/nsid.h"

typedef float f32x2 __attribute__((ext_vector_type(2)));
typedef float f32x4 __attribute__((ext_vector_type(4)));
typedef uint32_t u32x4 __attribute__((ext_vector_type(4)));
typedef __bf16 bf16x4 __attribute__((ext_vector_type(4)));
typedef __bf16 bf16x8 __attribute__((ext_vector_type(8)));

template <typename T> struct Chunk;
template <> struct Chunk<float> {
  static constexpr int N = 4;
  __device__ static __forceinline__ void load(const float* p, float* v) {
    const f32x4 x = *reinterpret_cast<const f32x4*>(p);
#pragma unroll
    for (int e = 0; e < 4; ++e) v[e] = x[e];
  }
  __device__ static __forceinline__ void store(float* p, const float* v) {
    *reinterpret_cast<f32x4*>(p) = f32x4{v[0], v[1], v[2], v[3]};
  }
};
template <> struct Chunk<__bf16> {
  static constexpr int N = 8;
  __device__ static __forceinline__ void load(const __bf16* p, float* v) {
    const bf16x8 x = *reinterpret_cast<const bf16x8*>(p);
#pragma unroll
    for (int e = 0; e < 8; ++e) v[e] = (float)x[e];
  }
  __device__ static __forceinline__ void store(__bf16* p, const float* v) {
    bf16x8 x;
#pragma unroll
    for (int e = 0; e < 8; ++e) x[e] = (__bf16)v[e];
    *reinterpret_cast<bf16x8*>(p) = x;
  }
};

template <int N>
__device__ __forceinline__ void load_channels(const float* __restrict__ p, int c, float* v) {
#pragma unroll
  for (int e = 0; e < N; e += 4) {
    const f32x4 x = *reinterpret_cast<const f32x4*>(p + c + e);
    v[e] = x[0]; v[e + 1] = x[1]; v[e + 2] = x[2]; v[e + 3] = x[3];
  }
}

#define NSID_DISPATCH_DTYPE(dtype, T, ...)                    \
  do {                                                        \
    if ((dtype) == NSID_BF16) { typedef __bf16 T; __VA_ARGS__; } \
    else { typedef float T; __VA_ARGS__; }                    \
  } while (0)
#define NSID_DTYPE_OK(d) ((d) == NSID_F32 || (d) == NSID_BF16)

#define NSID_WAVE 64

__device__ __forceinline__ float nsid_act(float v, int act) {
  switch (act) {
    case NSID_ACT_RELU: return v < 0.f ? 0.f : v;
    case NSID_ACT_LEAKY: return v > 0.f ? v : 0.2f * v;
    case NSID_ACT_ELU: return v > 0.f ? v : expm1f(v);
    default: return v;
  }
}
__device__ __forceinline__ float nsid_act_grad(float pre, int act) {
  switch (act) {
    case NSID_ACT_RELU: return pre > 0.f ? 1.f : 0.f;
    case NSID_ACT_LEAKY: return pre > 0.f ? 1.f : 0.2f;
    default: return 1.f;
  }
}

__device__ __forceinline__ float wave_sum(float v) {
  v += __builtin_bit_cast(float, __builtin_amdgcn_update_dpp(0, __builtin_bit_cast(int, v), 0xB1, 0xF, 0xF, true));
  v += __builtin_bit_cast(float, __builtin_amdgcn_update_dpp(0, __builtin_bit_cast(int, v), 0x4E, 0xF, 0xF, true));
  v += __builtin_bit_cast(float, __builtin_amdgcn_update_dpp(0, __builtin_bit_cast(int, v), 0x141, 0xF, 0xF, true));
  v += __builtin_bit_cast(float, __builtin_amdgcn_update_dpp(0, __builtin_bit_cast(int, v), 0x140, 0xF, 0xF, true));
  v += __builtin_bit_cast(float, __builtin_amdgcn_update_dpp(0, __builtin_bit_cast(int, v), 0x142, 0xA, 0xF, true));
  v += __builtin_bit_cast(float, __builtin_amdgcn_update_dpp(0, __builtin_bit_cast(int, v), 0x143, 0xC, 0xF, true));
  return __builtin_bit_cast(float, __builtin_amdgcn_readlane(__builtin_bit_cast(int, v), 63));
}
__device__ __forceinline__ double wave_sum_d(double v) {
#pragma unroll
  for (int o = 32; o > 0; o >>= 1) v += __shfl_xor(v, o, 64);
  return v;
}
__device__ __forceinline__ float wave_max(float v) {
#pragma unroll
  for (int o = 32; o > 0; o >>= 1) v = fmaxf(v, __shfl_xor(v, o, 64));
  return v;
}
__device__ __forceinline__ float wave_min(float v) {
#pragma unroll
  for (int o = 32; o > 0; o >>= 1) v = fminf(v, __shfl_xor(v, o, 64));
  return v;
}

__device__ __forceinline__ int lane_id() { return (int)__builtin_amdgcn_mbcnt_hi(~0u, __builtin_amdgcn_mbcnt_lo(~0u, 0u)); }
__device__ __forceinline__ f32x4 ld4(const float* p) { return *reinterpret_cast<const f32x4*>(p); }

template <int VM, int LGKM = 0xF>
__device__ __forceinline__ void nsid_waitcnt() {
  static_assert(VM >= 0 && VM < 64 && LGKM >= 0 && LGKM < 16, "6-bit vmcnt, 4-bit lgkmcnt");
  __builtin_amdgcn_s_waitcnt((VM & 0xF) | ((VM >> 4) << 14) | (7 << 4) | (LGKM << 8));
}
template <int N> __device__ __forceinline__ void wait_vm() { nsid_waitcnt<N>(); }
__device__ __forceinline__ void wait_lgkm0() { nsid_waitcnt<63, 0>(); }

__device__ __forceinline__ void glds16(const char* sbase, unsigned voff, unsigned dst) {
  unsigned keep;
  asm volatile("s_mov_b32 %0, m0\n\ts_mov_b32 m0, %3\n\ts_nop 0\n\tglobal_load_lds_dwordx4 %1, %2\n\ts_mov_b32 m0, %0"
               : "=&s"(keep) : "v"(voff), "s"(sbase), "s"(dst) : "memory");
}

inline hipError_t g_nsid_launch_error = hipSuccess;
static inline void nsid_note_launch(hipError_t e) {
  if (g_nsid_launch_error == hipSuccess) g_nsid_launch_error = e;
}
static inline int nsid_launch_status() {
  const hipError_t e = g_nsid_launch_error;
  g_nsid_launch_error = hipSuccess;
  if (e != hipSuccess) fprintf(stderr, "[nsid] kernel launch failed: %s\n", hipGetErrorString(e));
  return e == hipSuccess ? NSID_OK : NSID_ELAUNCH;
}

#define NSID_LAUNCH(kernel, grid, block, shmem, stream, ...)                \
  do {                                                                      \
    (void)hipGetLastError();                                                \
    hipLaunchKernelGGL(kernel, grid, block, shmem, stream, __VA_ARGS__);    \
    nsid_note_launch(hipGetLastError());                                    \
  } while (0)

constexpr int NSID_LDS_MAX = 160 * 1024;
inline hipError_t nsid_set_lds_cap(const void* kernel) {
  hipFuncAttributes a;
  const hipError_t e = hipFuncGetAttributes(&a, kernel);
  if (e != hipSuccess) return e;
  return hipFuncSetAttribute(kernel, hipFuncAttributeMaxDynamicSharedMemorySize, NSID_LDS_MAX - (int)a.sharedSizeBytes);
}
template <auto Kernel>
inline hipError_t nsid_big_lds() {
  static const hipError_t e = nsid_set_lds_cap(reinterpret_cast<const void*>(Kernel));
  return e;
}
#define NSID_LAUNCH_LDS(kernel, grid, block, bytes, stream, ...)            \
  do {                                                                      \
    nsid_note_launch(nsid_big_lds<kernel>());                               \
    NSID_LAUNCH(kernel, grid, block, bytes, stream, __VA_ARGS__);           \
  } while (0)
static inline bool nsid_aligned16(const void* p) { return (reinterpret_cast<uintptr_t>(p) & 15u) == 0; }

#define NSID_REQUIRE(cond) \
  do {                     \
    if (!(cond)) return NSID_EINVAL; \
  } while (0)

#define NSID_TUNING_TABLE(X)                                                                                                  \
  X(stream_max_wg, 2048)                              \
  X(bn_bwd_apply_max_wg, 384)        \
  X(gemm_deep_ks, 2)                 \
  X(gemm_deep_max_wg, 1024)     \
  X(gemm_deep_kinds, 5)         \
  X(bwd_split_max_tiles, 64)    \
  X(fwd_narrow, -1)                                         \
  X(bwd_narrow, -1)                                                                                                           \
  X(g256_min, 512)                                  \
  X(g256_train, 0)                            \
  X(g256_grid, 0)                                           \
  X(wgrad_wide, 1)                                     \
  X(wgrad_rect, 1)                                                                          \
  X(wgrad_wgs_rect, 256)                         \
  X(wgrad_wgs_sq, 1024)                                                                                                       \
  X(wgrad_rect_min, 256)                                                                                                      \
  X(wgrad_sq_min, 256)                                                                                                        \
  X(w3_wgs, 256)                                                                                                              \
  X(w3_min_tiles, 64)                                                                                                         \
  X(knn_strips, 0)                                            \
  X(knn_pair_min, 512)                 \
  X(knn_raw16, 1)               \
  X(knn_raw_wpe, 6)             \
  X(knn_sel_min_n, 128)               \
  X(mr_grid_stride, 0)                              \
  X(mr_split, 0)                                             \
  X(ffn_regs, 3)                \
  X(mr_key_min_k, 8)            \
  X(mr_bwd_sorted_min_k, 3)     \
  X(ffn_waves, 8)                                                \
  X(ffn256, 1)                  \
  X(mrconv_variant, 7)          \
  X(mrconv_pg_wgs, 768)         \
  X(wgg_rows, 4096)             \
  X(wgg_rows_sq, 1024)          \
  X(wgg_rows_gen, 512)          \
  X(bn_fin_tiles, 0)            \
  X(wgg_w3, 1)                  \
  X(wgrad256, 1)                \
  X(wgg_rows256, 4096)          \
  X(ws_gemm, 7)

enum NsidTuneKey {
#define NSID_TUNE_ENUM(name, def) NSID_T_##name,
  NSID_TUNING_TABLE(NSID_TUNE_ENUM)
#undef NSID_TUNE_ENUM
  NSID_T_COUNT
};
extern long g_nsid_tune[NSID_T_COUNT];
static inline long nsid_tune(NsidTuneKey k) { return g_nsid_tune[k]; }

#define NSID_COUNTER_TABLE(X)                                                                  \
  X(gemm_fwd) X(gemm_bwd_data) X(gemm_bwd_weight)              \
  X(gemm_full)                                    \
  X(gemm_ks2)                                                           \
  X(gemm_bwd_split)          \
  X(gemm_split_major)           \
  X(gemm_affine_load)          \
  X(gemm_relu_load)                                                                             \
  X(gemm_bn_sums)              \
  X(gemm_bn_apply_load)     \
  X(gemm256)                                                                   \
  X(ws_fwd) X(ws_bwd_data) X(ws_bwd_bnapply)                    \
  X(wgrad_rect) X(wgrad_square) X(wgrad3) X(wgrad_grouped) X(wgrad_grouped_w3) X(wgrad_grouped_256)                                                 \
  X(bn_bwd_apply) X(bn_bwd_apply_capped)                                                        \
  X(knn2) X(knn2_pair) X(knn2_raw) X(knn_rank) X(knn_sel) X(knn_strips) X(knn_big)                                                  \
  X(mr_fwd_lds) X(mr_fwd_grid) X(mr_fwd_key) X(mr_bwd_sorted)                                                                  \
  X(ffn_fused)                                 \
  X(mrconv_fused)          \
  X(row_sqnorm) X(flat_l2_topk) X(flat_l2_topk_wide) X(seq_scores)    \
  X(clf_node_rows) X(clf_pair_scores)            \
  X(clf_node_rows_n) X(clf_pair_scores_n)        \
  X(clf_mine) X(clf_attn_fwd) X(clf_head_fwd) X(clf_head_bwd) X(clf_attn_bwd) X(clf_seg_reduce)    \
  X(clf_attn_fwd_n) X(clf_attn_bwd_n) X(clf_seg_reduce_n)    \
  X(logmel_fft)            \
  X(cqt)                   \
  X(aug_stft) X(aug_vocoder) X(aug_istft) X(aug_finish)    \
  X(aug_compress) X(aug_biquad) X(aug_frames)    \
  X(conv2d_3x3) X(conv2d_1x1) X(ibn_relu) X(stem7_pool) X(gem_pool)    \
  X(pair_ce) X(triplet) X(baseline_objective) X(baseline_objective_rows)    \
  X(gem_pool_bwd)          \
  X(conv2d_bwd_data) X(conv2d_bwd_weight) X(col_stat) X(ibn_relu_bwd) X(bn_add_relu) X(relu_bwd)    \
  X(stem7_stat) X(stem7_pool_train) X(stem7_bwd)    \
  X(resample_sinc) X(stem_pairs_gate) X(stem_pairs_build)    \
  X(logmel_fft_ragged) X(cqt_ragged) X(unfold_segments_ragged)    \
  X(song_vote) X(song_vote_clf) X(vote_candidates)    \
  X(pair_sim) X(local_align)    \
  X(flat_l2_topk_excl) X(flat_l2_topk_wide_excl)

constexpr int NSID_STEM7_STAT_MAX = 1024;

enum NsidCounterKey {
#define NSID_CNT_ENUM(name) NSID_C_##name,
  NSID_COUNTER_TABLE(NSID_CNT_ENUM)
#undef NSID_CNT_ENUM
  NSID_C_COUNT
};
extern long g_nsid_counter[NSID_C_COUNT];
static inline void nsid_count(NsidCounterKey k) { ++g_nsid_counter[k]; }

__device__ __forceinline__ int nsid_pack_song(const long* __restrict__ songs, const int n_songs, const long b) {
  int lo = 0, hi = n_songs - 1;
  while (lo < hi) {
    const int mid = (lo + hi + 1) >> 1;
    if (songs[(long)NSID_PACK_COLS * mid + 3] <= b) lo = mid; else hi = mid - 1;
  }
  return lo;
}

constexpr int WGG_MAXP = 28;
struct WgProb {
  const void* A[2];
  const void* B[2];
  const float* bsc[2];
  const float* bsh[2];
  float* C;
  int lda, ldb, I, J, R;
  int groups, rchunk;
  int seg_splits, nsplit;
  int tiles, nwg;
  float slope;
  int pad_period, pad_c1;
};
struct WgGroupArgs {
  int n, pad;
  int wg0[WGG_MAXP + 1];
  WgProb prob[WGG_MAXP];
};
static_assert(sizeof(WgProb) == 128 && sizeof(WgGroupArgs) + 256 <= 4096, "the problem table travels in the kernel arguments");


__device__ __forceinline__ bool wgg_decode(const WgGroupArgs& ga, const int w, int& pi, int& split, int& bid, int& g, int& seg) {
  pi = 0;
  for (int i = 1; i < ga.n; ++i) pi += (w >= ga.wg0[i]) ? 1 : 0;
  pi = __builtin_amdgcn_readfirstlane(pi);
  const WgProb& q = ga.prob[pi];
  const int l = w - ga.wg0[pi];
  if (l >= q.nwg) return false;
  const int S = q.nsplit;
  int rest;
  if (S < 8 && (8 % S) == 0) {
    const int x = l & 7, per = 8 / S;
    split = x % S;
    rest = (l >> 3) * per + x / S;
  } else {
    split = l % S;
    rest = l / S;
  }
  if (rest >= q.tiles * q.groups) return false;
  g = rest / q.tiles;
  bid = rest % q.tiles;
  seg = split >= q.seg_splits ? 1 : 0;
  split -= seg * q.seg_splits;
  return true;
}
int nsid_wgrad3_grouped_launch(const WgGroupArgs& ga, int grid, bool affine, hipStream_t stream);
int nsid_wgrad4_grouped_launch(const WgGroupArgs& ga, int grid, hipStream_t stream);

int nsid_wgrad2_launch(const void* dout, int ldd, const void* x, int ldx, float* dw, int M, int Nout, int K, int groups,
                       const float* in_scale, const float* in_shift, float slope, hipStream_t stream);

int nsid_gemm256_fwd_launch(const void* x, int ldx, const void* w, const float* bias, const void* addend, int ldadd, void* out,
                            int ldo, int M, int Nout, int K, bool relu_out, float* stat, long stat_plane, long stat_ld,
                            hipStream_t stream);
int nsid_ws_fwd_launch(const void* x, int ldx, const void* w, const float* bias, void* out, int ldo, int M, int Nout, int K,
                       int groups, const float* in_scale, const float* in_shift, float in_slope, float* stat, long stat_plane,
                       long stat_ld, hipStream_t stream);
int nsid_ws_bwd_data_launch(const void* dout, int ldd, const void* w, const void* addend, int ldadd, void* din, int ldi, int M, int Nout,
                            int K, int groups, const void* bn_r, long bn_ldr, const float* bn_scale, const float* bn_shift,
                            const float* bn_mean, const float* bn_invstd, float bn_slope, float* bn_partial, long bn_plane, long bn_ld,
// ... 8 lines not shown
```

neuralsampleid_amd/csrc/ntxent.hip:

```cpp
#include "nsid_common.h"

namespace {

constexpr int RB = 16;
constexpr int CBK = 128;

__device__ __forceinline__ const float* zrow(const float* z_i, const float* z_j, int row, int d) {
  return ((row & 1) ? z_j : z_i) + (long)(row >> 1) * d;
}

__device__ __forceinline__ void stage_rows(float* dst, int ld, const float* z_i, const float* z_j, int row0, int nrows,
                                           int M, int d) {
  const int d4 = d >> 2;
  constexpr int UB = 8;
  for (int q0 = threadIdx.x; q0 < nrows * d4; q0 += UB * blockDim.x) {
    f32x4 v[UB];
#pragma unroll
    for (int u = 0; u < UB; ++u) {
      const int q = q0 + u * blockDim.x;
      const int rr = q / d4, c = (q % d4) * 4;
      v[u] = f32x4{0.f, 0.f, 0.f, 0.f};
      if (q < nrows * d4 && row0 + rr < M) v[u] = *reinterpret_cast<const f32x4*>(zrow(z_i, z_j, row0 + rr, d) + c);
    }
#pragma unroll
    for (int u = 0; u < UB; ++u) {
      const int q = q0 + u * blockDim.x;
      const int rr = q / d4, c = (q % d4) * 4;
      if (q < nrows * d4) *reinterpret_cast<f32x4*>(dst + rr * ld + c) = v[u];
    }
  }
}

constexpr int PF_MAX = 16;
struct Prefetch { f32x4 v[PF_MAX]; };

__device__ __forceinline__ void prefetch_rows(Prefetch& pf, const float* z_i, const float* z_j, int row0, int nrows, int M,
                                              int d) {
  const int d4 = d >> 2;
#pragma unroll
  for (int u = 0; u < PF_MAX; ++u) {
    const int q = threadIdx.x + u * 256;
    const int rr = q / d4, c = (q % d4) * 4;
    pf.v[u] = f32x4{0.f, 0.f, 0.f, 0.f};
    if (q < nrows * d4 && row0 + rr < M) pf.v[u] = *reinterpret_cast<const f32x4*>(zrow(z_i, z_j, row0 + rr, d) + c);
  }
}

__device__ __forceinline__ void commit_rows(float* dst, int ld, const Prefetch& pf, int nrows, int d) {
  const int d4 = d >> 2;
#pragma unroll
  for (int u = 0; u < PF_MAX; ++u) {
    const int q = threadIdx.x + u * 256;
    const int rr = q / d4, c = (q % d4) * 4;
    if (q < nrows * d4) *reinterpret_cast<f32x4*>(dst + rr * ld + c) = pf.v[u];
  }
}

template <int NT>
__device__ __forceinline__ void sim_tiles(const float* zi_w, const float* zj_t, int ld, int d, int lr, int rq,
                                          f32x4 (&acc)[NT]) {
#pragma unroll
  for (int u = 0; u < NT; ++u) acc[u] = f32x4{0.f, 0.f, 0.f, 0.f};
  const float* pa = zj_t + lr * ld + 4 * rq;
  const float* pb = zi_w + lr * ld + 4 * rq;
  for (int ch = 0; ch < d; ch += 16) {
    const f32x4 fb = *reinterpret_cast<const f32x4*>(pb + ch);
    f32x4 fa[NT];
#pragma unroll
    for (int u = 0; u < NT; ++u) fa[u] = *reinterpret_cast<const f32x4*>(pa + u * 16 * ld + ch);
#pragma unroll
    for (int e = 0; e < 4; ++e)
#pragma unroll
      for (int u = 0; u < NT; ++u) acc[u] = __builtin_amdgcn_mfma_f32_16x16x4f32(fa[u][e], fb[e], acc[u], 0, 0, 0);
  }
}


__global__ __launch_bounds__(256) void ntxent_lse_kernel(const float* __restrict__ z_i, const float* __restrict__ z_j,
                                                         int M, int d, float tau, int cols_per_group,
                                                         float* __restrict__ lse, float* __restrict__ rowloss,
                                                         float* __restrict__ part_out) {
  extern __shared__ __attribute__((aligned(16))) float sm[];
  const int ld = d + 4;
  float* zi_s = sm;
  float* zj_s = sm + RB * ld;
  float* part = zj_s + CBK * ld;
  const int i0 = blockIdx.x * RB;
  const int lane = threadIdx.x & 63, wave = threadIdx.x >> 6, lr = lane & 15, rq = lane >> 4;
  stage_rows(zi_s, ld, z_i, z_j, i0, RB, M, d);
  const int i = i0 + lr;
  float mrun = -__builtin_inff(), srun = 0.f, pos = 0.f;
  constexpr int TPW = CBK / 16 / 4;
  const bool pipelined = CBK * (d >> 2) <= PF_MAX * 256;
  Prefetch pf;
  const int jbeg = blockIdx.y * cols_per_group, jend = min(M, jbeg + cols_per_group);
  if (pipelined) {
    prefetch_rows(pf, z_i, z_j, jbeg, CBK, M, d);
    __syncthreads();
    commit_rows(zj_s, ld, pf, CBK, d);
  }
  for (int j0 = jbeg; j0 < jend; j0 += CBK) {
    if (pipelined) {
      __syncthreads();
      prefetch_rows(pf, z_i, z_j, j0 + CBK, CBK, M, d);
    } else {
      __syncthreads();
      stage_rows(zj_s, ld, z_i, z_j, j0, CBK, M, d);
      __syncthreads();
    }
    f32x4 acc[TPW];
    sim_tiles<TPW>(zi_s, zj_s + 16 * (wave * TPW) * ld, ld, d, lr, rq, acc);
#pragma unroll
    for (int u = 0; u < TPW; ++u) {
#pragma unroll
      for (int e = 0; e < 4; ++e) {
        const int j = j0 + 16 * (wave * TPW + u) + 4 * rq + e;
        const float a = acc[u][e] / tau;
        if (j < M && j != i) {
          if (j == (i ^ 1)) pos = a;
          const float mn = fmaxf(mrun, a);
          srun = srun * expf(mrun - mn) + expf(a - mn);
          mrun = mn;
        }
      }
    }
    if (pipelined) {
      __syncthreads();
      commit_rows(zj_s, ld, pf, CBK, d);
    }
  }
#pragma unroll
  for (int o = 16; o <= 32; o <<= 1) {
    const float m2 = __shfl_xor(mrun, o, 64), s2 = __shfl_xor(srun, o, 64), p2 = __shfl_xor(pos, o, 64);
    const float mn = fmaxf(mrun, m2);
    const float e1 = mrun == -__builtin_inff() ? 0.f : expf(mrun - mn);
    const float e2 = m2 == -__builtin_inff() ? 0.f : expf(m2 - mn);
    srun = srun * e1 + s2 * e2;
    mrun = mn;
    pos += p2;
  }
  if (rq == 0) { part[(wave * 3 + 0) * 16 + lr] = mrun; part[(wave * 3 + 1) * 16 + lr] = srun; part[(wave * 3 + 2) * 16 + lr] = pos; }
  __syncthreads();
  if (threadIdx.x < 16 && i0 + (int)threadIdx.x < M) {
    float m = -__builtin_inff(), sacc = 0.f, p = 0.f;
#pragma unroll
    for (int w = 0; w < 4; ++w) {
      const float m2 = part[(w * 3 + 0) * 16 + threadIdx.x], s2 = part[(w * 3 + 1) * 16 + threadIdx.x];
      const float mn = fmaxf(m, m2);
      const float e1 = m == -__builtin_inff() ? 0.f : expf(m - mn);
      const float e2 = m2 == -__builtin_inff() ? 0.f : expf(m2 - mn);
      sacc = sacc * e1 + s2 * e2;
      m = mn;
      p += part[(w * 3 + 2) * 16 + threadIdx.x];
    }
    if (gridDim.y > 1) {
      float* po = part_out + (long)blockIdx.y * 3 * M + i0 + threadIdx.x;
      po[0] = m; po[M] = sacc; po[2 * M] = p;
    } else {
      const float l = m + logf(sacc);
      lse[i0 + threadIdx.x] = l;
      rowloss[i0 + threadIdx.x] = l - p;
    }
  }
}

__global__ void ntxent_lse_merge_kernel(const float* __restrict__ part, int groups, int M, float* __restrict__ lse,
                                        float* __restrict__ rowloss) {
  const int i = blockIdx.x * blockDim.x + threadIdx.x;
  if (i >= M) return;
  float m = -__builtin_inff(), sacc = 0.f, p = 0.f;
  for (int g = 0; g < groups; ++g) {
    const float m2 = part[(long)g * 3 * M + i], s2 = part[(long)g * 3 * M + M + i];
    const float mn = fmaxf(m, m2);
    const float e1 = m == -__builtin_inff() ? 0.f : expf(m - mn);
    const float e2 = m2 == -__builtin_inff() ? 0.f : expf(m2 - mn);
    sacc = sacc * e1 + s2 * e2;
    m = mn;
    p += part[(long)g * 3 * M + 2 * M + i];
  }
  const float l = m + logf(sacc);
  lse[i] = l;
  rowloss[i] = l - p;
}

template <int DT>
__global__ __launch_bounds__(256) void ntxent_grad_kernel(const float* __restrict__ z_i, const float* __restrict__ z_j,
                                                          int M, int d, float tau, const float* __restrict__ lse,
                                                          int row0, int nrows, int cols_per_group,
                                                          float* __restrict__ dz_i, float* __restrict__ dz_j) {
  extern __shared__ __attribute__((aligned(16))) float sm[];
  const int ld = d + 4;
  float* zi_s = sm;
  float* zj_s = sm + RB * ld;
  const int i0 = row0 + blockIdx.x * RB;
  const int lane = threadIdx.x & 63, wave = threadIdx.x >> 6, lr = lane & 15, rq = lane >> 4;
  stage_rows(zi_s, ld, z_i, z_j, i0, RB, M, d);
  const int i = i0 + lr;
  const bool iok = i < row0 + nrows && i < M;
  const float lse_i = iok ? lse[i] : 0.f;
  f32x4 out[DT];
#pragma unroll
  for (int c = 0; c < DT; ++c) out[c] = f32x4{0.f, 0.f, 0.f, 0.f};
  constexpr int TPW = CBK / 16 / 4;
  const bool pipelined = CBK * (d >> 2) <= PF_MAX * 256;
  Prefetch pf;
  const int jbeg = blockIdx.y * cols_per_group, jend = min(M, jbeg + cols_per_group);
  if (pipelined) {
    prefetch_rows(pf, z_i, z_j, jbeg, CBK, M, d);
    __syncthreads();
    commit_rows(zj_s, ld, pf, CBK, d);
  }
  for (int j0 = jbeg; j0 < jend; j0 += CBK) {
    if (pipelined) {
      __syncthreads();
      prefetch_rows(pf, z_i, z_j, j0 + CBK, CBK, M, d);
    } else {
      __syncthreads();
      stage_rows(zj_s, ld, z_i, z_j, j0, CBK, M, d);
      __syncthreads();
    }
    f32x4 acc[TPW];
    sim_tiles<TPW>(zi_s, zj_s + 16 * (wave * TPW) * ld, ld, d, lr, rq, acc);
#pragma unroll
    for (int u = 0; u < TPW; ++u) {
      const int jt = wave * TPW + u;
      f32x4 q;
#pragma unroll
      for (int e = 0; e < 4; ++e) {
        const int j = j0 + 16 * jt + 4 * rq + e;
        float v = 0.f;
        if (iok && j < M && j != i) {
          const float a = acc[u][e] / tau;
          v = expf(a - lse_i) + expf(a - lse[j]);
          if (j == (i ^ 1)) v -= 2.f;
        }
        q[e] = v;
      }
      const float* zb = zj_s + (16 * jt + 4 * rq) * ld + lr;
#pragma unroll
      for (int c = 0; c < DT; ++c)
#pragma unroll
        for (int e = 0; e < 4; ++e)
          out[c] = __builtin_amdgcn_mfma_f32_16x16x4f32(q[e], zb[e * ld + 16 * c], out[c], 0, 0, 0);
    }
    if (pipelined) {
      __syncthreads();
      commit_rows(zj_s, ld, pf, CBK, d);
    }
  }
  __syncthreads();
  float* red = zj_s;
#pragma unroll
  for (int e = 0; e < 4; ++e)
#pragma unroll
    for (int c = 0; c < DT; ++c) red[(wave * 16 + 4 * rq + e) * ld + 16 * c + lr] = out[c][e];
  __syncthreads();
  const float sc = 1.f / ((float)M * tau);
  for (int q = threadIdx.x; q < RB * d; q += blockDim.x) {
    const int rr = q / d, c = q % d;
    const int row = i0 + rr;
    if (row < row0 + nrows && row < M) {
      const float v = (red[rr * ld + c] + red[(16 + rr) * ld + c]) + (red[(32 + rr) * ld + c] + red[(48 + rr) * ld + c]);
      float* dst = ((row & 1) ? dz_j : dz_i) + (long)((row >> 1) - (row0 >> 1)) * d;
      if (gridDim.y > 1) atomicAdd(dst + c, v * sc);
      else dst[c] = v * sc;
    }
  }
}

__global__ __launch_bounds__(256) void ntxent_loss_kernel(const float* __restrict__ rowloss, int row0, int nrows, int M,
                                                          float* __restrict__ loss_out) {
  __shared__ double red[4];
  double s = 0.0;
  for (int i = threadIdx.x; i < nrows; i += blockDim.x) s += (double)rowloss[row0 + i];
  s = wave_sum_d(s);
  if ((threadIdx.x & 63) == 0) red[threadIdx.x >> 6] = s;
  __syncthreads();
  if (threadIdx.x == 0) loss_out[0] = (float)((red[0] + red[1] + red[2] + red[3]) / (double)M);
}

}

constexpr int LSE_MAX_GROUPS = 16;
extern "C" size_t nsid_ntxent_ws_floats(int Bg) { return (size_t)4 * Bg + 8 + (size_t)LSE_MAX_GROUPS * 3 * 2 * Bg; }

extern "C" int nsid_ntxent_fwd_bwd(const float* z_i, const float* z_j, int Bg, int d, float tau, int p0, int np,
                                   float* ws, float* loss_out, float* dz_i, float* dz_j, void* stream) {
  NSID_REQUIRE(z_i && z_j && ws && loss_out && Bg > 0 && np > 0 && p0 >= 0 && p0 + np <= Bg && tau > 0.f);
  NSID_REQUIRE(d % 16 == 0 && d <= 256 && nsid_aligned16(z_i) && nsid_aligned16(z_j));
  NSID_REQUIRE((dz_i == nullptr) == (dz_j == nullptr));
  const int M = 2 * Bg;
  float* lse = ws;
  float* rowloss = ws + M;
  hipStream_t s = static_cast<hipStream_t>(stream);
  const size_t bytes = ((size_t)(RB + CBK) * (d + 4) + 4 * 3 * 16) * sizeof(float);
  {
    const int row_tiles = (M + RB - 1) / RB, nblocks = (M + CBK - 1) / CBK;
    int cg = row_tiles >= 512 ? 1 : (512 + row_tiles - 1) / row_tiles;
    if (cg > nblocks) cg = nblocks;
    if (cg > LSE_MAX_GROUPS) cg = LSE_MAX_GROUPS;
    const int cols_per_group = (nblocks + cg - 1) / cg * CBK;
    cg = (M + cols_per_group - 1) / cols_per_group;
    float* part = ws + 2 * M + 8;
    NSID_LAUNCH_LDS(ntxent_lse_kernel, dim3(row_tiles, cg), dim3(256), bytes, s, z_i, z_j, M, d, tau, cols_per_group, lse,
                    rowloss, part);
    if (cg > 1) NSID_LAUNCH(ntxent_lse_merge_kernel, dim3((M + 255) / 256), dim3(256), 0, s, part, cg, M, lse, rowloss);
  }
  NSID_LAUNCH(ntxent_loss_kernel, dim3(1), dim3(256), 0, s, rowloss, 2 * p0, 2 * np, M, loss_out);
  if (dz_i != nullptr) {
    const int row0 = 2 * p0, nrows = 2 * np;
    const int row_tiles = (nrows + RB - 1) / RB, nblocks = (M + CBK - 1) / CBK;
    int cg = row_tiles >= 128 ? 1 : (256 + row_tiles - 1) / row_tiles;
    if (cg > nblocks) cg = nblocks;
    const int cols_per_group = (nblocks + cg - 1) / cg * CBK;
    cg = (M + cols_per_group - 1) / cols_per_group;
    if (cg > 1) {
      if (hipMemsetAsync(dz_i, 0, (size_t)np * d * sizeof(float), s) != hipSuccess ||
          hipMemsetAsync(dz_j, 0, (size_t)np * d * sizeof(float), s) != hipSuccess) {
        (void)nsid_launch_status();
        return NSID_ELAUNCH;
      }
    }
    dim3 grid(row_tiles, cg);
#define NSID_NTX_CASE(DTV)                                                                                   \
  case DTV:                                                                                                  \
    NSID_LAUNCH_LDS((ntxent_grad_kernel<DTV>), grid, dim3(256), bytes, s, z_i, z_j, M, d, tau, lse, row0,    \
                    nrows, cols_per_group, dz_i, dz_j);                                                      \
    break;
    switch (d / 16) {
      NSID_NTX_CASE(1) NSID_NTX_CASE(2) NSID_NTX_CASE(4) NSID_NTX_CASE(8) NSID_NTX_CASE(16)
      default:
        (void)nsid_launch_status();
        return NSID_EINVAL;
    }
#undef NSID_NTX_CASE
  }
  return nsid_launch_status();
}
```

neuralsampleid_amd/functional.py:

```python
from typing import Dict, List, Optional

import torch

from . import ops
from .ops import ACT_ELU, ACT_LEAKY, ACT_NONE, ACT_RELU, BNAffine

Tensor = torch.Tensor


class KnnTape:

    def __init__(self, replay: Optional[List[Tensor]] = None, cyclic: bool = False, patch=None):
        self.replay = list(replay) if replay is not None else None
        self.recorded: List[Tensor] = []
        self.pos = 0
        self.cyclic = cyclic
        self.patch = list(patch) if patch is not None else None
        self.patched: List[Tensor] = []


TAPE: Optional[KnnTape] = None

EXACT_BIAS_GRAD = False

# ... 424 lines not shown
    col, x, wp, r, aff, B, N, C = (S[k_] for k_ in ("col", "x", "wp", "r", "aff", "B", "N", "C"))
    Mo, Co = r.shape
    dr = ops.bn_backward(dout, r, aff, ACT_NONE, G["conv.1.weight"], G["conv.1.bias"], partial=_link_partial(S))
    _bias_grad_before_bn(dr, G["conv.0.bias"])
    prep = S.get("prep")
    if prep is not None:
        dwp = S.get("dwp_slot")
        if dwp is None:
            dwp = ops.zeros(prep["dwp"].shape[1:], prep["dwp"].device)
        if _deferring() and DEFER_DS and dr.dtype == torch.bfloat16:
            if S.get("dwp_slot") is not None:
                dwp = prep["dwp"][0]
            DEFERRED.add(dr, x, dwp, Mo, Co, 3 * C, 1, None, None, ACT_NONE, ("ds", B, N, C, G["conv.0.weight"]))
        else:
            ops.downsample3_bwd_weight(dr, x, dwp, B, N, C, Co)
            ops.unpack_ds_wgrad(dwp, G["conv.0.weight"])
        return ops.downsample3_bwd_data(dr, None, None, B, N, C, Co, w16=(prep["wp16"], prep["wb16"]))
    dwp = ops.zeros(wp.shape, wp.device)
    if col is None:
        ops.downsample3_bwd_weight(dr, x, dwp, B, N, C, Co)
        ops.unpack_ds_wgrad(dwp, G["conv.0.weight"])
        return ops.downsample3_bwd_data(dr, wp, ops.pack_ds_weight_bwd(P["conv.0.weight"]), B, N, C, Co)
    ops.linear_bwd_weight(dr, col, dwp, Mo, Co, 3 * C)
    ops.unpack_ds_wgrad(dwp, G["conv.0.weight"])
    dcol = ops.linear_bwd_data(dr, wp, Mo, Co, 3 * C)
    return ops.im2col3_bwd(dcol, B, N, C)


DGL_DOWNSAMPLES = 3


def dgl_chain_forward(nodes: Tensor, P, S: Optional[dict], B: int, N: int, training: bool) -> Tensor:
    if S is not None and not training:
        raise NotImplementedError("backward through the eval-mode DGL passthrough encoder is not implemented: run it under "
                                  "torch.no_grad() in eval mode, or train() it")
    M, K = nodes.shape
    C = P["stem.0.weight"].shape[0]
    r, aff = conv_bn(nodes, M, K, C, P["stem.0.weight"], None, _bn(P, S, "stem.1."), training)
    layers = [(r, aff, ACT_LEAKY, N, C)]
    act = ACT_LEAKY
    for l_ in range(DGL_DOWNSAMPLES):
        pre = f"ds{l_}.conv."
        w = P[pre + "0.weight"]
        Co, No = w.shape[0], ops.ds_out_nodes(N)
        gamma, beta, rm, rv, nbt, _ = _bn(P, S, pre + "1.")
        if training:
            r, stat = ops.dsact_fwd(r, B, N, C, w, P[pre + "0.bias"], Co, aff, act, want_stat=True)
            aff = bn_affine_from(stat, B * No, gamma, beta, rm, rv, nbt, True)
        else:
            r, _ = ops.dsact_fwd(r, B, N, C, w, P[pre + "0.bias"], Co, aff, act,
                                 out_aff=ops.bn_eval_affine(gamma, beta, rm, rv), act_out=ACT_RELU)
            aff = None
        act, N, C = (ACT_RELU if training else ACT_NONE), No, Co
        layers.append((r, aff, act, N, C))
    if not training:
        return r
    out = ops.bn_apply(r, aff, ACT_RELU)
    if S is not None:
        S.update(nodes=nodes, layers=layers, B=B)
    return out


def dgl_chain_backward(dout: Tensor, P, S, G) -> Tensor:
    layers, B, nodes = S["layers"], S["B"], S["nodes"]
    last = f"ds{DGL_DOWNSAMPLES - 1}.conv.1."
    dr = ops.bn_backward(dout, layers[-1][0], layers[-1][1], ACT_RELU, G[last + "weight"], G[last + "bias"])
    for l_ in reversed(range(DGL_DOWNSAMPLES)):
        pre = f"ds{l_}.conv."
        r, aff, act, N, C = layers[l_]
        Co = dr.shape[1]
        _bias_grad_before_bn(dr, G[pre + "0.bias"])
        ops.dsact_bwd_weight(dr, r, G[pre + "0.weight"], B, N, C, Co, aff, act)
        g, part = ops.dsact_bwd_data(dr, P[pre + "0.weight"], B, N, C, Co, r, aff, act, want_partial=True)
        bn = "stem.1." if l_ == 0 else f"ds{l_ - 1}.conv.1."
        dr = ops.bn_backward(g, r, aff, ACT_NONE, G[bn + "weight"], G[bn + "bias"], inplace=True, partial=part)
    M, K = nodes.shape
    C = dr.shape[1]
    ops.linear_bwd_weight(dr, nodes, ops.w2d(G["stem.0.weight"]), M, C, K)
    return ops.linear_bwd_data(dr, ops.w2d(P["stem.0.weight"]), M, C, K)


HEAD_FC1_KSPLIT = 1
HEAD_KSPLIT = True


def proj_mean_forward(x: Tensor, P, S: Optional[dict], B: int, N: int) -> Tensor:
    M, C = x.shape
    E = P["weight"].shape[0]
    xm = ops.node_mean_fwd(x, B, N, C)
    h, _ = ops.linear_fwd(xm, ops.w2d(P["weight"]), P["bias"], B, E, C,
                          ksplit=4 if (HEAD_KSPLIT and S is not None and C >= 512 and B <= 512) else 1)
    if S is not None:
        S.update(xm=xm, B=B, N=N, C=C, xdtype=x.dtype)
    return h


def proj_mean_backward(dh: Tensor, P, S, G) -> Tensor:
    xm, B, N, C = S["xm"], S["B"], S["N"], S["C"]
    E = dh.shape[1]
    _wgrad(dh, xm, ops.w2d(G["weight"]), B, E, C)
    _bias_grad(dh, G["bias"])
    dxm = ops.linear_bwd_data(dh, ops.w2d(P["weight"]), B, E, C)
    return ops.node_mean_bwd(dxm, B, N, C, S["xdtype"])


def projector_forward(h: Tensor, P, S: Optional[dict], eps: float = 1e-10) -> Tensor:
    B, Hin = h.shape
    Hid, D = P["0.weight"].shape[0], P["2.weight"].shape[0]
    a1, _ = ops.linear_fwd(h, P["0.weight"], P["0.bias"], B, Hid, Hin, act_out=ACT_ELU,
                           ksplit=HEAD_FC1_KSPLIT if (Hin >= 1024 and B <= 512 and h.dtype == torch.float32) else 1)
    ks = 8 if (Hid >= 2048 and S is not None) else 1
    p, _ = ops.linear_fwd(a1, P["2.weight"], P["2.bias"], B, D, Hid, ksplit=ks)
    z, norm = ops.l2norm_fwd(p, eps)
    if S is not None:
        S.update(h=h, a1=a1, z=z, norm=norm, eps=eps)
    return z


def projector_backward(dz: Tensor, P, S, G) -> Tensor:
    h, a1, z, norm, eps = S["h"], S["a1"], S["z"], S["norm"], S["eps"]
    B, Hin = h.shape
    Hid, D = a1.shape[1], z.shape[1]
    dp = ops.l2norm_bwd(dz, z, norm, eps)
    _wgrad(dp, a1, G["2.weight"], B, D, Hid)
    _bias_grad(dp, G["2.bias"])
    da1 = ops.linear_bwd_data(dp, P["2.weight"], B, D, Hid)
    dpre = ops.elu_bwd(da1, a1)
    _wgrad(dpre, h, G["0.weight"], B, Hid, Hin)
    _bias_grad(dpre, G["0.bias"])
    return ops.linear_bwd_data(dpre, P["0.weight"], B, Hid, Hin)


def patchify_forward(spec: Tensor, P, S: Optional[dict], pb: int, pf: int) -> Tensor:
    out, minmax = ops.peak_patchify_fwd(spec, P["convs.0.weight"], P["convs.0.bias"], pb, pf, ACT_DTYPE)
    if S is not None:
        S.update(spec=spec, minmax=minmax, out=out, pb=pb, pf=pf)
    return out


DEFER_PATCHIFY = 1


def patchify_backward(dout: Tensor, P, S, G) -> None:
    args = (S["spec"], S["minmax"], S["out"], dout, S["pb"], S["pf"], G["convs.0.weight"], G["convs.0.bias"])
    if _deferring() and DEFER_PATCHIFY:
        DEFERRED.add_call(lambda: ops.peak_patchify_bwd(*args), args[:4])
    else:
        ops.peak_patchify_bwd(*args)


class _BlockFn(torch.autograd.Function):

    @staticmethod
    def forward(ctx, fwd, bwd, names, buffers, meta, grad_on, x, *params):
        P = dict(zip(names, params))
        P.update(buffers)
        need = grad_on and any(ctx.needs_input_grad)
        S = {} if need else None
        out = fwd(x.contiguous(), P, S, *meta)
        ctx.S, ctx.P, ctx.bwd, ctx.names = S, P, bwd, names
        ctx.x_needs = x.requires_grad
        return out

    @staticmethod
    def backward(ctx, dout):
        P, S, names = ctx.P, ctx.S, ctx.names
        direct = DIRECT_GRADS and all(P[n].grad is not None and P[n].grad.is_contiguous() for n in names)
        G = {n: (P[n].grad if direct else ops.zeros(P[n].shape, P[n].device)) for n in names}
        global _IN_DIRECT_BACKWARD
        n_def = len(DEFERRED.items)
        _IN_DIRECT_BACKWARD = direct
        try:
            dx = ctx.bwd(dout.contiguous(), P, S, G)
        finally:
            _IN_DIRECT_BACKWARD = False
        ctx.S = None
        if direct and GRAD_READY_HOOK is not None:
            if len(DEFERRED.items) > n_def:
                DEFERRED.note_hook([P[n] for n in names], n_def)
            else:
                GRAD_READY_HOOK([P[n] for n in names])
        head = (None, None, None, None, None, None, dx if ctx.x_needs else None)
        return head + tuple(None if direct else G[n] for n in names)


def run_block(fwd, bwd, module_params: Dict[str, Tensor], module_buffers: Dict[str, Tensor], x: Tensor, *meta):
    names = tuple(module_params.keys())
    return _BlockFn.apply(fwd, bwd, names, module_buffers, meta, torch.is_grad_enabled(), x, *module_params.values())


class _ToRows(torch.autograd.Function):
    @staticmethod
    def forward(ctx, x):
        ctx.shape = x.shape
        return ops.bcn_to_rows(x.contiguous(), ACT_DTYPE)

    @staticmethod
    def backward(ctx, d):
        B, N = ctx.shape[0], ctx.shape[2]
        return ops.rows_to_bcn(d.contiguous(), B, N).reshape(ctx.shape)


class _FromRows(torch.autograd.Function):
    @staticmethod
    def forward(ctx, rows, B, N):
        ctx.rows_dtype = rows.dtype
        return ops.rows_to_bcn(rows.contiguous(), B, N)

    @staticmethod
    def backward(ctx, d):
        return ops.bcn_to_rows(d.contiguous(), ctx.rows_dtype), None, None


# ... 25 lines not shown
```

neuralsampleid_amd/ops.py:

```python
import math
import os
from typing import Optional, Tuple

import numpy as np
import torch

from ._lib import DEFINES as _H
from ._lib import call, get_tuning, launch_counters, lib, reset_tuning, set_tuning

ACT_NONE, ACT_RELU, ACT_LEAKY, ACT_ELU = _H["NSID_ACT_NONE"], _H["NSID_ACT_RELU"], _H["NSID_ACT_LEAKY"], _H["NSID_ACT_ELU"]
ROW_TILE = _H["NSID_ROW_TILE"]
BN_MOMENTUM = 0.1
BN_EPS = 1e-5


class KernelProfile:

    def __init__(self):
        self.records = []
        self.bracket_ms = self._empty_bracket_ms()

    @staticmethod
    def plug(ms: float = 120.0) -> None:
        torch.cuda._sleep(int(ms * 1e-3 * 2.0e9))
# ... 120 lines not shown
    return w.reshape(w.shape[0], -1)


WEIGHT_EPOCH = 0
STATS_EPOCH = 0


def bump_state_epoch(weights: bool = True, stats: bool = True) -> None:
    global WEIGHT_EPOCH, STATS_EPOCH
    if weights:
        WEIGHT_EPOCH += 1
    if stats:
        STATS_EPOCH += 1


class WeightShadows:

    def __init__(self):
        self.entries = {}

    def register(self, w: torch.Tensor, shadow: torch.Tensor, owner: torch.Tensor, fresh: bool = False) -> None:
        import weakref
        self.entries[w.data_ptr()] = [shadow, (w._version, WEIGHT_EPOCH) if fresh else None, w.numel(), weakref.ref(owner)]

    def mark_fresh(self, w: torch.Tensor) -> None:
        e = self.entries.get(w.data_ptr())
        if e is not None:
            e[1] = (w._version, WEIGHT_EPOCH)

    def clear(self) -> None:
        self.entries.clear()

    def purge(self) -> int:
        dead = [k for k, e in self.entries.items() if e[3]() is None]
        for k in dead:
            del self.entries[k]
        return len(dead)

    def operand(self, w: torch.Tensor) -> torch.Tensor:
        e = self.entries.get(w.data_ptr())
        if e is not None and e[3]() is None:
            del self.entries[w.data_ptr()]
            e = None
        if e is None or e[2] != w.numel():
            return f32_to_bf16(w)
        key = (w._version, WEIGHT_EPOCH)
        if e[1] != key:
            f32_to_bf16(w, e[0])
            e[1] = key
        return e[0]


SHADOWS = WeightShadows()


def register_weight_shadows(module) -> int:
    n = 0
    for p in module.parameters():
        if p.is_cuda and p.dim() >= 2 and p.numel() % 8 == 0 and p.data_ptr() not in SHADOWS.entries:
            SHADOWS.register(p.data, torch.empty(p.numel(), device=p.device, dtype=torch.bfloat16), owner=p)
            n += 1
    return n


def f32_to_bf16(src: torch.Tensor, dst: Optional[torch.Tensor] = None) -> torch.Tensor:
    _chk(src)
    n = src.numel()
    if dst is None:
        dst = torch.empty(((n + 7) // 8 * 8,), device=src.device, dtype=torch.bfloat16)
    if n % 8:
        dst[:n].copy_(src.reshape(-1))
        return dst
    _tk("f32_to_bf16_kernel", 6.0 * n, lambda: call("nsid_f32_to_bf16", _p(src), _p(dst), n, _stream()), (n, 1, 0, 1))
    return dst


def _weight(w: torch.Tensor, dt: int, K: int):
    if dt == BF16 and K % 8 == 0 and w.numel() % 8 == 0:
        return SHADOWS.operand(w), BF16
    return w, F32


def linear_fwd(x, w, bias, M, Nout, K, groups=1, in_scale=None, in_shift=None, act_in=ACT_NONE, act_out=ACT_NONE,
               want_stat=False, ksplit=1, out=None, addend=None, in_aff=None) -> Tuple[torch.Tensor, Optional[torch.Tensor]]:
    if in_aff is not None:
        in_scale, in_shift = in_aff.scale, in_aff.shift
    _chk(w, bias, in_scale, in_shift)
    dt = _act(x, out, addend)
    if addend is not None and (want_stat or ksplit != 1 or act_out != ACT_NONE):
        raise ValueError("the residual addend rides with a plain epilogue (no statistics, no split-K, no output activation)")
    ldx = x.shape[-1]
    if out is None:
        out = torch.empty((M, groups * Nout), device=x.device, dtype=x.dtype)
        if ksplit > 1:
            fill_zero(out)
    stat = torch.empty((2, row_tiles(M), groups * Nout), device=x.device, dtype=torch.float32) if want_stat else None
    half = dt == BF16 or lib.nsid_get_gemm_precision() == GEMM_BF16
    narrow = (Nout <= 64 or (Nout <= 128 and K <= 256 and in_scale is None)) if half else Nout <= 64
    if half and row_tiles(M) * ((Nout + 127) // 128) * groups < 128:
        narrow = True
    esz = x.element_size()
    wop, wdt = _weight(w, dt, K)
    name_ = "gemm_kernel<128,%d,true,true>" % (64 if narrow else 128)
    n256 = lib.nsid_gemm_g256_launches() if PROFILE is not None else 0
    nws = _cnt("ws_fwd")
    name = lambda: ("ws_fwd_kernel" if _cnt("ws_fwd") > nws else
                    ("gemm256_fwd_kernel" if lib.nsid_gemm_g256_launches() > n256 else name_))
    if in_scale is None and act_in != ACT_NONE:
        bn_ = 64 if narrow else 128
        bm_ = 128
        if not (act_in == ACT_RELU and dt == BF16 and wdt == BF16 and M % bm_ == 0 and Nout % bn_ == 0 and K % 64 == 0
                and ksplit == 1):
            raise ValueError("activation-on-load without an affine needs ReLU, bf16 storage, bf16 weights and whole tiles")
    if addend is not None:
        _timed(name, 2.0 * M * Nout * K * groups,
               groups * (esz * M * K + float(wop.element_size()) * Nout * K + 2 * esz * M * Nout), lambda: call(
            "nsid_linear_fwd_res", _p(x), ldx, _p(wop), wdt, _p(bias), _p(addend), addend.shape[-1], _p(out),
            out.shape[-1], M, Nout, K, groups, _p(in_scale), _p(in_shift), act_in, dt, _stream()), (M, Nout, K, groups))
        return out, None
    _timed(name, 2.0 * M * Nout * K * groups,
           groups * (esz * M * K + float(wop.element_size()) * Nout * K + esz * M * Nout), lambda: call(
        "nsid_linear_fwd", _p(x), ldx, _p(wop), wdt, _p(bias), _p(out), out.shape[-1], M, Nout, K, groups, _p(in_scale),
        _p(in_shift), act_in, act_out, _p(stat), ksplit, dt, _stream()), (M, Nout, K, groups))
    return out, stat


FUSE_EVAL_FFN = True


def ffn_fused_fwd(x, w1f, b1f, w2f, b2f, M, C, H):
    _chk(w1f, b1f, w2f, b2f)
    if _act(x) != BF16 or x.shape != (M, C) or not FUSE_EVAL_FFN:
        return None
    w1, d1 = _weight(w1f, BF16, C)
    w2, d2 = _weight(w2f, BF16, H)
    if d1 != BF16 or d2 != BF16:
        return None
    out = torch.empty_like(x)
    rc = [0]

    def launch():
        rc[0] = lib.nsid_ffn_fused_fwd(_p(x), _p(w1), _p(b1f), _p(w2), _p(b2f), _p(out), M, C, H, _stream())
    _timed("ffn_fused_kernel", 4.0 * M * C * H, 2.0 * x.element_size() * M * C + 4.0 * C * H, launch, (M, C, H, 1))
    if rc[0] == 1:
        if PROFILE is not None:
            PROFILE.records.pop()
        return None
    if rc[0] != 0:
        raise RuntimeError(f"nsid_ffn_fused_fwd failed: {rc[0]}")
    return out


FUSE_EVAL_MRCONV = True


def mrconv_fused_fwd(y, idx, B, N, C, wf, bf):
    _chk(wf, bf)
    if not FUSE_EVAL_MRCONV or _act(y) != BF16 or y.shape != (B * N, C) or idx.dtype != torch.int32 or not idx.is_contiguous():
        return None
    w, dw = _weight(wf, BF16, C // 2)
    if dw != BF16:
        return None
    k = idx.shape[-1]
    out = torch.empty((B * N, 2 * C), device=y.device, dtype=y.dtype)
    rc = [0]

    def launch():
        rc[0] = lib.nsid_mrconv_fused_fwd(_p(y), _p(idx), B, N, C, k, _p(w), _p(bf), _p(out), _stream())
    _timed("mrconv_fused_kernel", 2.0 * B * N * (C // 2) * (C // 2) * 4, float(B) * N * (3 * C * y.element_size() + k * 4), launch,
           (B * N, C // 2, C // 2, 4))
    if rc[0] == 1:
        if PROFILE is not None:
            PROFILE.records.pop()
        return None
    if rc[0] != 0:
        raise RuntimeError(f"nsid_mrconv_fused_fwd failed: {rc[0]}")
    return out


FUSE_BN_BWD_REDUCE = True


def linear_bwd_data(dout, w, M, Nout, K, groups=1, addend=None, out=None, bn=None):
    _chk(w)
    dt = _act(dout, addend, out)
    if out is None:
        out = torch.empty((M, groups * K), device=dout.device, dtype=dout.dtype)
    half = dt == BF16 or lib.nsid_get_gemm_precision() == GEMM_BF16
    narrow = (K <= 64 or (K <= 128 and Nout <= 256)) if half else K <= 64
    if half and row_tiles(M) * ((K + 127) // 128) * groups < 128:
        narrow = True
    name_ = "gemm_kernel<128,%d,true,false>" % (64 if narrow else 128)
    nws = _cnt("ws_bwd_data")
    name = lambda: "ws_bwd_kernel" if _cnt("ws_bwd_data") > nws else name_
    esz = dout.element_size()
    wop, wdt = _weight(w, dt, K)
    want_pair = bn is not None
    bn = bn or None
    fuse = bn is not None and FUSE_BN_BWD_REDUCE and dt == BF16 and out.shape[-1] == groups * K and (groups * K) % 8 == 0
    if fuse and tuple(bn[0].shape) != (M, groups * K):
        fuse = False
    nbytes = groups * (esz * M * Nout + float(wop.element_size()) * Nout * K
                       + esz * M * K * ((2 if addend is not None else 1) + (1 if fuse else 0)))
    if fuse:
        r, aff, act = bn
        _act(r, out)
        partial = torch.empty((2, row_tiles(M), groups * K), device=dout.device, dtype=torch.float32)
        _timed(name, 2.0 * M * Nout * K * groups, nbytes, lambda: call(
            "nsid_linear_bwd_data_bn", _p(dout), dout.shape[-1], _p(wop), wdt, _p(addend),
            0 if addend is None else addend.shape[-1], _p(out), out.shape[-1], M, Nout, K, groups, dt, _p(r),
            _p(aff.scale), _p(aff.shift), _p(aff.mean), _p(aff.invstd), act, _p(partial), _stream()),
            (M, Nout, K, groups))
        return out, partial
    _timed(name, 2.0 * M * Nout * K * groups, nbytes, lambda: call(
        "nsid_linear_bwd_data", _p(dout), dout.shape[-1], _p(wop), wdt, _p(addend),
        0 if addend is None else addend.shape[-1], _p(out), out.shape[-1], M, Nout, K, groups, dt, _stream()),
        (M, Nout, K, groups))
    return (out, None) if want_pair else out


FUSE_BN_BWD_APPLY = 4
SITE_FFN, SITE_GCONV, SITE_FC1, SITE_FC2, SITE_FFN2 = 1, 2, 4, 8, 16
WS_BWD_SHAPES = {(64, 64, 1), (32, 32, 4), (64, 128, 1), (256, 64, 1), (64, 256, 1), (128, 128, 1), (64, 64, 4), (128, 256, 1),
                 (128, 128, 4)}


def bn_backward_linear_bwd_data(dy, r, aff: "BNAffine", act, dgamma, dbeta, partial, w, M, Nout, K, groups=1, addend=None,
                                bn=None, site=SITE_FFN, inplace=True):
    dt = _act(dy, r, addend)
    C = r.shape[1]
    tiles = row_tiles(M)
    s = _stream()
    wop, wdt = _weight(w, dt, K)
    enabled = FUSE_BN_BWD_APPLY is True or (FUSE_BN_BWD_APPLY and (int(FUSE_BN_BWD_APPLY) & site))
    ws_form = (dt == BF16 and wdt == BF16 and M % 128 == 0 and (Nout, K, groups) in WS_BWD_SHAPES and (get_tuning("ws_gemm") & 4) != 0)
    enabled = enabled or ws_form
    fusable = (enabled and dt == BF16 and wdt == BF16 and tuple(r.shape) == (M, groups * Nout) and
               tuple(dy.shape) == (M, groups * Nout) and M % 128 == 0 and
               (ws_form or (Nout % 64 == 0 and K % 64 == 0 and (K <= 64 or K % 128 == 0))))
    if not fusable:
        dr = bn_backward(dy, r, aff, act, dgamma, dbeta, inplace=inplace, partial=partial)
        return (dr,) + linear_bwd_data(dr, w, M, Nout, K, groups, addend=addend, bn=bn if bn is not None else False)
    if partial is None:
        partial = torch.empty((2, tiles, C), device=r.device, dtype=torch.float32)
        part_ = partial
        _tk("col_reduce_kernel", 2.0 * r.element_size() * M * C, lambda: call(
            "nsid_bn_bwd_reduce", _p(dy), _p(r), M, C, _p(aff.scale), _p(aff.shift), _p(aff.mean), _p(aff.invstd), act, _p(part_),
            dt, s), (M, C, 0, 1))
    ptiles = partial.shape[1]
    coef = torch.empty((6, C), device=r.device, dtype=torch.float32)
    if not (DIAG_SKIP_FINALIZE & 2):
        _tk("bn_bwd_finalize_kernel", 8.0 * ptiles * C + 40.0 * C, lambda: call(
            "nsid_bn_bwd_finalize_fused", _p(partial), ptiles, C, M, _p(dgamma), _p(dbeta), _p(coef), _p(aff.scale), _p(aff.shift),
            _p(aff.mean), _p(aff.invstd), _p(coef[2]), s), (M, C, 0, 1))
    dr = torch.empty_like(dy)
    din = torch.empty((M, groups * K), device=dy.device, dtype=dy.dtype)
    want_pair = bn is not None
    bn = bn or None
    fuse_sums = bn is not None and FUSE_BN_BWD_REDUCE and (groups * K) % 8 == 0 and tuple(bn[0].shape) == (M, groups * K)
    part_out = torch.empty((2, tiles, groups * K), device=dy.device, dtype=torch.float32) if fuse_sums else None
    br, baff, bact = bn if fuse_sums else (None, None, ACT_NONE)
    esz = dy.element_size()
    nbytes = groups * (3 * esz * M * Nout + float(wop.element_size()) * Nout * K
                       + esz * M * K * ((2 if addend is not None else 1) + (1 if fuse_sums else 0)))
    rc = [0]

    def launch():
        rc[0] = lib.nsid_linear_bwd_data_bnapply(
            _p(dy), _p(r), _p(coef[2]), act, _p(dr), _p(wop), wdt, _p(addend), 0 if addend is None else addend.shape[-1], _p(din),
            din.shape[-1], M, Nout, K, groups, dt, _p(br), _p(baff.scale) if baff else None, _p(baff.shift) if baff else None,
            _p(baff.mean) if baff else None, _p(baff.invstd) if baff else None, bact, _p(part_out), s)
    _timed("ws_bwd_kernel +bn_apply_load" if ws_form else "gemm_kernel<128,%d,true,false> +bn_apply_load" % (64 if K <= 64 else 128),
           2.0 * M * Nout * K * groups, nbytes, launch, (M, Nout, K, groups))
    if rc[0] == 1:
        if PROFILE is not None:
            PROFILE.records.pop()
        call("nsid_bn_bwd_apply", _p(dy), _p(r), M, C, _p(aff.scale), _p(aff.shift), _p(aff.mean), _p(aff.invstd), act, _p(coef),
             _p(dr), dt, s)
        res = linear_bwd_data(dr, w, M, Nout, K, groups, addend=addend, out=din, bn=bn if bn is not None else False)
        return (dr,) + res
    if rc[0] != 0:
        raise RuntimeError(f"nsid_linear_bwd_data_bnapply failed: {rc[0]}")
    return dr, din, part_out


def linear_bwd_weight(dout, x, dw, M, Nout, K, groups=1, in_scale=None, in_shift=None, act_in=ACT_NONE) -> None:
    _chk(dw, in_scale, in_shift)
    dt = _act(dout, x)
    t128 = ((Nout + 127) // 128) * ((K + 127) // 128) * groups
    half = dt == BF16 or lib.nsid_get_gemm_precision() == GEMM_BF16
    small = half or Nout <= 64 or K <= 64 or t128 * ((M + 511) // 512) < 256
    name = "gemm_kernel<%s,false,false>" % ("64,64" if small else "128,128")
    if dt == BF16 and Nout % 128 == 0 and K % 64 == 0 and M % 1024 == 0:
        tiles_r = (Nout // 128) * (K // 64) * groups
        if tiles_r * min(M // 1024, max(1, 512 // tiles_r)) >= 256 and get_tuning("wgrad_rect") != 0:
            name = "gemm_kernel<128,64,false,false>"
    if dt == BF16 and Nout % 128 == 0 and K % 128 == 0 and M % 128 == 0 and (Nout // 128) * (K // 128) * groups >= 64:
        name = "wgrad3_kernel"
# ... 80 lines not shown


_IDENTITY_AFFINE = {}


def identity_affine(C: int, device) -> BNAffine:
    key = (C, str(device))
    a = _IDENTITY_AFFINE.get(key)
    if a is None:
        a = _IDENTITY_AFFINE[key] = BNAffine(torch.ones(C, device=device), torch.zeros(C, device=device), identity=True)
    return a


_FOLDED = {}


def folded_conv_bn(w2d, bias, gamma, beta, running_mean, running_var, eps=BN_EPS, source=None):
    import weakref
    src = w2d if source is None else source
    versions = (src.data_ptr(), src._version, None if bias is None else (bias.data_ptr(), bias._version), gamma._version,
                beta._version, running_mean._version, running_var._version, eps, WEIGHT_EPOCH, STATS_EPOCH)
    cacheable = not torch.cuda.is_current_stream_capturing()
    e = _FOLDED.get(id(gamma))
    if e is not None and e[0]() is gamma and e[1] == versions:
        return e[2], e[3]
    with torch.no_grad():
        if callable(w2d):
            w2d = w2d()
        s = gamma.detach() / torch.sqrt(running_var + eps)
        w_fold = (w2d.detach() * s[:, None]).contiguous()
        b_fold = (beta.detach() - running_mean * s) if bias is None else (bias.detach() * s + beta.detach() - running_mean * s)
        b_fold = b_fold.contiguous()
        if w_fold.numel() % 8 == 0:
            SHADOWS.register(w_fold, f32_to_bf16(w_fold), owner=w_fold, fresh=True)
    if cacheable:
        _cache_constants(_FOLDED, id(gamma), (weakref.ref(gamma), versions, w_fold, b_fold))
    return w_fold, b_fold


def _cache_constants(cache, key, entry) -> None:
    torch.cuda.current_stream().synchronize()
    if len(cache) > 4096:
        for k in [k for k, v in cache.items() if v[0]() is None]:
            del cache[k]
    cache[key] = entry


def bn_finalize(stat, M, gamma, beta, running_mean, running_var, num_batches_tracked,
                momentum=BN_MOMENTUM, eps=BN_EPS, tiles=None) -> BNAffine:
    C = gamma.numel()
    tiles = row_tiles(M) if tiles is None else int(tiles)
    buf = torch.empty((4, C), device=gamma.device, dtype=torch.float32)
    if running_mean is not None:
        bump_state_epoch(weights=False)
    _tk("bn_finalize_kernel", 8.0 * tiles * C + 16.0 * C, lambda: call(
        "nsid_bn_finalize", _p(stat), tiles, C, M, _p(gamma), _p(beta), _p(running_mean), _p(running_var),
        _p(num_batches_tracked), momentum, eps, _p(buf[0]), _p(buf[1]), _p(buf[2]), _p(buf[3]), _stream()), (M, C, 0, 1))
    return BNAffine(buf[0], buf[1], buf[2], buf[3])


DIAG_SKIP_FINALIZE = 0
_DIAG_CONST = {}


def _diag_const(C, device):
    key = (C, str(device))
    if key not in _DIAG_CONST:
        _DIAG_CONST[key] = (torch.ones(C, device=device), torch.zeros(C, device=device), torch.zeros((2, C), device=device))
    return _DIAG_CONST[key]


def bn_finalize_deferred(stat, M, gamma, beta, eps=BN_EPS):
    C = gamma.numel()
    if DIAG_SKIP_FINALIZE & 1:
        one, zero, _ = _diag_const(C, gamma.device)
        return BNAffine(one, zero, zero, one), one
    buf = torch.empty((5, C), device=gamma.device, dtype=torch.float32)
    _tk("bn_finalize_kernel", 8.0 * row_tiles(M) * C + 20.0 * C, lambda: call(
        "nsid_bn_finalize_deferred", _p(stat), row_tiles(M), C, M, _p(gamma), _p(beta), eps, _p(buf[0]), _p(buf[1]),
        _p(buf[2]), _p(buf[3]), _p(buf[4]), _stream()), (M, C, 0, 1))
    return BNAffine(buf[0], buf[1], buf[2], buf[3]), buf[4]


def bn_running_update(layers_a, layers_b=None, momentum=BN_MOMENTUM) -> None:
    import ctypes
    n = len(layers_a)
    if n == 0:
        return
    if layers_b is not None and len(layers_b) != n:
        raise ValueError("both views must have run the same BatchNorm layers")
    bump_state_epoch(weights=False)
    arr = lambda vals: (ctypes.c_void_p * n)(*[None if v is None else v.data_ptr() for v in vals])
    Cs = (ctypes.c_int * n)(*[la[0].numel() for la in layers_a])
    for la in layers_a:
        _chk(la[0], la[1], la[3], la[4])
    if layers_b is not None:
        for la, lb in zip(layers_a, layers_b):
            if la[0].data_ptr() != lb[0].data_ptr():
                raise ValueError("the two views disagree on the layer order")
            _chk(lb[3], lb[4])
    call("nsid_bn_running_update", n, Cs, arr([la[0] for la in layers_a]), arr([la[1] for la in layers_a]),
         arr([la[2] for la in layers_a]), arr([la[3] for la in layers_a]), arr([la[4] for la in layers_a]),
         None if layers_b is None else arr([lb[3] for lb in layers_b]),
         None if layers_b is None else arr([lb[4] for lb in layers_b]), momentum, _stream())


_EVAL_AFFINE = {}


def bn_eval_affine(gamma, beta, running_mean, running_var, eps=BN_EPS) -> BNAffine:
    import weakref
    versions = (gamma._version, beta._version, running_mean._version, running_var._version,
                beta.data_ptr(), running_mean.data_ptr(), running_var.data_ptr(), WEIGHT_EPOCH, STATS_EPOCH)
    cacheable = not torch.cuda.is_current_stream_capturing()
    e = _EVAL_AFFINE.get(id(gamma))
    if e is not None and e[0]() is gamma and e[1] == versions and e[2] == eps:
        if e[4] != _stream() and cacheable:
            torch.cuda.current_stream().wait_event(e[5])
        return e[3]
    C = gamma.numel()
    buf = torch.empty((2, C), device=gamma.device, dtype=torch.float32)
    call("nsid_bn_eval_affine", _p(gamma), _p(beta), _p(running_mean), _p(running_var), eps, C, _p(buf[0]),
         _p(buf[1]), _stream())
    aff = BNAffine(buf[0], buf[1])
    if cacheable:
        ev = torch.cuda.Event()
        ev.record()
        if len(_EVAL_AFFINE) > 4096:
            for k in [k for k, v in _EVAL_AFFINE.items() if v[0]() is None]:
                del _EVAL_AFFINE[k]
        _EVAL_AFFINE[id(gamma)] = (weakref.ref(gamma), versions, eps, aff, _stream(), ev)
    return aff


def bn_apply(r, aff: BNAffine, act=ACT_NONE, residual=None, out=None) -> torch.Tensor:
    dt = _act(r, residual, out)
    M, C = r.shape
    if out is None:
        out = torch.empty_like(r)
    _tk("bn_apply_kernel", r.element_size() * M * C * (3 if residual is not None else 2), lambda: call(
        "nsid_bn_apply", _p(r), _p(aff.scale), _p(aff.shift), act, _p(residual), _p(out), M, C, dt, _stream()), (M, C, 0, 1))
    return out


def bn_backward(dout, r, aff: BNAffine, act, dgamma, dbeta, inplace=False, partial=None) -> torch.Tensor:
    dt = _act(dout, r)
    M, C = r.shape
    tiles = row_tiles(M) if partial is None else partial.shape[1]
    s = _stream()
    coef = torch.empty((2, C), device=r.device, dtype=torch.float32)
    if partial is None:
        partial = torch.empty((2, tiles, C), device=r.device, dtype=torch.float32)
        part_ = partial
        _tk("col_reduce_kernel", 2.0 * r.element_size() * M * C, lambda: call(
            "nsid_bn_bwd_reduce", _p(dout), _p(r), M, C, _p(aff.scale), _p(aff.shift), _p(aff.mean), _p(aff.invstd),
            act, _p(part_), dt, s), (M, C, 0, 1))
    if DIAG_SKIP_FINALIZE & 2:
        coef = _diag_const(C, r.device)[2]
    else:
        _tk("bn_bwd_finalize_kernel", 8.0 * tiles * C + 16.0 * C, lambda: call(
            "nsid_bn_bwd_finalize", _p(partial), tiles, C, M, _p(dgamma), _p(dbeta), _p(coef), s), (M, C, 0, 1))
    dr = dout if inplace else torch.empty_like(dout)
    _tk("bn_bwd_apply_kernel", 3.0 * r.element_size() * M * C, lambda: call(
        "nsid_bn_bwd_apply", _p(dout), _p(r), M, C, _p(aff.scale), _p(aff.shift), _p(aff.mean), _p(aff.invstd),
        act, _p(coef), _p(dr), dt, s), (M, C, 0, 1))
    return dr
# ... 220 lines not shown
    return wp


def unpack_ds_wgrad(dwp, dw) -> None:
    _chk(dwp, dw)
    call("nsid_unpack_ds_wgrad", _p(dwp), dw.shape[0], dw.shape[1], _p(dw), _stream())


def dsact_fwd(x, B, N, C, w, bias, Cout, in_aff: Optional["BNAffine"] = None, act_in=ACT_NONE, want_stat=False,
              out_aff: Optional["BNAffine"] = None, act_out=ACT_NONE):
    dt = _act(x)
    _chk(w, bias, *((in_aff.scale, in_aff.shift) if in_aff is not None else ()),
         *((out_aff.scale, out_aff.shift) if out_aff is not None else ()))
    No = ds_out_nodes(N)
    M = B * No
    out = torch.empty((M, Cout), device=x.device, dtype=x.dtype)
    stat = torch.empty((2, row_tiles(M), Cout), device=x.device, dtype=torch.float32) if want_stat else None
    _timed("dsact_fwd_kernel", 2.0 * M * Cout * 3 * C, float(x.element_size()) * (B * N * C + M * Cout), lambda: call(
        "nsid_dsact_fwd", _p(x), B, N, C, _p(in_aff.scale) if in_aff else None, _p(in_aff.shift) if in_aff else None, act_in,
        _p(w), _p(bias), _p(out), Cout, _p(stat), _p(out_aff.scale) if out_aff else None, _p(out_aff.shift) if out_aff else None,
        act_out, dt, _stream()), (M, Cout, 3 * C, 1))
    return out, stat


def dsact_bwd_weight(dout, x, dw, B, N, C, Cout, in_aff: Optional["BNAffine"] = None, act_in=ACT_NONE) -> None:
    dt = _act(dout, x)
    _chk(dw, *((in_aff.scale, in_aff.shift) if in_aff is not None else ()))
    M = dout.shape[0]
    _timed("dsact_wgrad_kernel", 2.0 * M * Cout * 3 * C, float(x.element_size()) * (B * N * C + M * Cout), lambda: call(
        "nsid_dsact_bwd_weight", _p(dout), _p(x), _p(in_aff.scale) if in_aff else None, _p(in_aff.shift) if in_aff else None,
        act_in, _p(dw), B, N, C, Cout, dt, _stream()), (Cout, 3 * C, M, 1))


def dsact_bwd_data(dout, w, B, N, C, Cout, r_prev=None, aff: Optional["BNAffine"] = None, act=ACT_NONE, want_partial=False):
    dt = _act(dout, r_prev)
    _chk(w)
    if r_prev is not None:
        _chk(aff.scale, aff.shift)
    if want_partial:
        _chk(aff.mean, aff.invstd)
    dx = torch.empty((B * N, C), device=dout.device, dtype=dout.dtype)
    partial = torch.empty((2, int(lib.nsid_dsact_part_rows(B, N)), C), device=dout.device, dtype=torch.float32) \
        if want_partial else None
    M = dout.shape[0]
    _timed("dsact_dgrad_kernel", 2.0 * M * Cout * 3 * C, float(dout.element_size()) * (M * Cout + 2 * B * N * C), lambda: call(
        "nsid_dsact_bwd_data", _p(dout), _p(w), _p(dx), B, N, C, Cout, _p(r_prev), _p(aff.scale) if aff else None,
        _p(aff.shift) if aff else None, _p(aff.mean) if want_partial else None, _p(aff.invstd) if want_partial else None, act,
        _p(partial), dt, _stream()), (B * N, C, 3 * Cout, 1))
    return dx, partial


def peak_patchify_fwd(spec, w, bias, pb, pf, out_dtype=torch.float32):
    _chk(spec, w, bias)
    B, H, W = spec.shape
    F = w.shape[0]
    n = (H // pb) * (W // pf)
    out = torch.empty((B * n, F), device=spec.device, dtype=out_dtype)
    minmax = torch.empty((B, 2), device=spec.device, dtype=torch.float32)
    _tk("patchify_fwd_kernel", 4.0 * B * H * W + float(out.element_size()) * B * n * F, lambda: call(
        "nsid_peak_patchify_fwd", _p(spec), _p(w), _p(bias), B, H, W, pb, pf, F, _p(out), F, _p(minmax), _act(out),
        _stream()), (B * n, F, pb * pf * 3, 1))
    return out, minmax


PATCHIFY_BWD_WS = True


def peak_patchify_bwd(spec, minmax, out, dout, pb, pf, dw, dbias) -> None:
    _chk(spec, minmax, dw, dbias)
    B, H, W = spec.shape
    F = out.shape[-1]
    nbytes = 4.0 * B * H * W + 2.0 * out.element_size() * out.numel()
    if PATCHIFY_BWD_WS and (H, W, pb, pf, F) == (64, 128, 4, 8, 8) and out.is_contiguous() and dout.is_contiguous():
        ws = torch.empty((B, 776), device=spec.device, dtype=torch.float32)
        _tk("patchify_bwd2_kernel", nbytes + 8.0 * ws.numel(), lambda: call(
            "nsid_peak_patchify_bwd_ws", _p(spec), _p(minmax), _p(out), _p(dout), F, B, H, W, pb, pf, F, _p(dw), _p(dbias), _p(ws),
            _act(out, dout), _stream()), (out.shape[0], out.shape[1], pb * pf * 3, 1))
        return
    _tk("patchify_bwd_kernel", nbytes, lambda: call(
        "nsid_peak_patchify_bwd", _p(spec), _p(minmax), _p(out), _p(dout), out.shape[-1], B, H, W, pb, pf,
        out.shape[-1], _p(dw), _p(dbias), _act(out, dout), _stream()), (out.shape[0], out.shape[1], pb * pf * 3, 1))


def node_mean_fwd(x, B, N, C) -> torch.Tensor:
    out = torch.empty((B, C), device=x.device, dtype=torch.float32)
    _tk("node_mean_fwd_kernel", float(x.element_size()) * B * N * C, lambda: call(
        "nsid_node_mean_fwd", _p(x), B, N, C, _p(out), _act(x), _stream()), (B * N, C, 0, 1))
    return out


def node_mean_bwd(dout, B, N, C, dtype=torch.float32) -> torch.Tensor:
    _chk(dout)
    dx = torch.empty((B * N, C), device=dout.device, dtype=dtype)
    _tk("node_mean_bwd_kernel", float(dx.element_size()) * B * N * C, lambda: call(
        "nsid_node_mean_bwd", _p(dout), B, N, C, _p(dx), _act(dx), _stream()), (B * N, C, 0, 1))
    return dx


def elu_bwd(dout, out) -> torch.Tensor:
    _chk(dout, out)
    din = torch.empty_like(dout)
    call("nsid_elu_bwd", _p(dout), _p(out), out.numel(), _p(din), _stream())
    return din


def l2norm_fwd(p, eps):
    _chk(p)
    B, d = p.shape
    z = torch.empty_like(p)
    norm = torch.empty((B,), device=p.device, dtype=torch.float32)
    call("nsid_l2norm_fwd", _p(p), B, d, eps, _p(z), _p(norm), _stream())
    return z, norm


def l2norm_bwd(dz, z, norm, eps) -> torch.Tensor:
    _chk(dz, z, norm)
    B, d = z.shape
    dp = torch.empty_like(z)
    call("nsid_l2norm_bwd", _p(dz), _p(z), _p(norm), B, d, eps, _p(dp), _stream())
    return dp


def ntxent_fwd_bwd(z_i, z_j, tau, p0=0, npairs=None, want_grad=True):
    _chk(z_i, z_j)
    Bg, d = z_i.shape
    npairs = Bg if npairs is None else npairs
    ws = torch.empty((lib.nsid_ntxent_ws_floats(Bg),), device=z_i.device, dtype=torch.float32)
    loss = torch.empty((1,), device=z_i.device, dtype=torch.float32)
    dzi = torch.empty((npairs, d), device=z_i.device, dtype=torch.float32) if want_grad else None
    dzj = torch.empty((npairs, d), device=z_i.device, dtype=torch.float32) if want_grad else None
    _timed("ntxent_kernels", 2.0 * (2 * Bg) * (2 * npairs) * d * (2 if want_grad else 1), 4.0 * d * (2 * Bg + 2 * npairs), lambda: call(
        "nsid_ntxent_fwd_bwd", _p(z_i), _p(z_j), Bg, d, float(tau), p0, npairs, _p(ws), _p(loss), _p(dzi), _p(dzj),
        _stream()), (2 * npairs, 2 * Bg, d, 1))
    return loss, dzi, dzj


BL_MAX = _H["NSID_BL_MAX"]


def _bl_check(name, M, d):
    if d % 16 != 0 or not 16 <= d <= BL_MAX or not 1 <= M <= BL_MAX:
        raise ValueError(f"{name}: D % 16 == 0, 16 <= D <= {BL_MAX} and at most {BL_MAX} rows are supported, got {M} rows of {d}")


def _bl_ws(M, d, device):
    return torch.empty((lib.nsid_baseline_loss_ws_floats(M, d),), device=device, dtype=torch.float32)


def _bl_mining(ws, M):
    Mp = (M + 63) // 64 * 64
    ints = ws[Mp:4 * Mp].view(torch.int32)
    flags = ints[2 * Mp:2 * Mp + M]
    return {"pidx": ints[:M], "nidx": ints[Mp:Mp + M], "valid": (flags & 1).bool(), "active": (flags & 2).bool()}


def pair_ce_fwd_bwd(z_i, z_j, want_grad=True):
    _chk(z_i, z_j)
    B, d = z_i.shape
    if z_j.shape != z_i.shape:
        raise ValueError(f"pair_ce_fwd_bwd: z_i {tuple(z_i.shape)} and z_j {tuple(z_j.shape)} differ")
    _bl_check("pair_ce_fwd_bwd", 2 * B, d)
    ws = _bl_ws(2 * B, d, z_i.device)
    out = torch.empty((1,), device=z_i.device, dtype=torch.float32)
    dzi = torch.empty_like(z_i) if want_grad else None
    dzj = torch.empty_like(z_j) if want_grad else None
    M = 2 * B
    _timed("baseline_loss_kernels<ce>", 2.0 * M * M * d * (2 if want_grad else 1), 4.0 * d * M * (2 if want_grad else 1), lambda: call(
        "nsid_pair_ce_fwd_bwd", _p(z_i), _p(z_j), B, d, _p(ws), _p(out), _p(dzi), _p(dzj), _stream()), (M, M, d, 1))
    return out, dzi, dzj


def triplet_fwd_bwd(e, labels, margin=0.2, want_grad=True, mining=False):
    _chk(e)
    if not (labels.is_cuda and labels.dtype == torch.int64 and labels.is_contiguous()):
        raise RuntimeError("triplet_fwd_bwd: labels must be a contiguous int64 tensor on the GPU")
    M, d = e.shape
    if labels.numel() != M:
        raise ValueError(f"triplet_fwd_bwd: {M} embeddings and {labels.numel()} labels")
    _bl_check("triplet_fwd_bwd", M, d)
    ws = _bl_ws(M, d, e.device)
    out = torch.empty((2,), device=e.device, dtype=torch.float32)
    de = torch.empty_like(e) if want_grad else None
    _timed("baseline_loss_kernels<triplet>", 2.0 * M * M * d, 4.0 * d * M * (2 if want_grad else 1), lambda: call(
        "nsid_triplet_fwd_bwd", _p(e), _p(labels), M, d, float(margin), _p(ws), _p(out), _p(de), _stream()), (M, M, d, 1))
# ... 1367 lines not shown
```

Before: 36540 clips/s.

## Fold split-K output zeroing into preceding head kernels and widen BN running-update batch

Split-K GEMMs in the projection head (proj_mean fc, projector fc2, projector bwd-data fc1) need a zeroed fp32 output before atomic accumulation. That zero fill is now done inside the kernel that runs just before each one (node_mean_fwd, the fc1 ELU epilogue, elu_bwd), which removes separate memset launches. The BN running-stat update also packs up to 64 layers per launch, using uint16 channel counts, with a tunable chunk size. Truncated parts of the diff also restructure the NT-Xent grad kernel so the final merge happens in the same launch. The main risk is ordering: the zeroing kernel must finish before the atomic GEMM starts.

New measurement: 36710 clips/s, median of 6. No clear change (+0.5%).

```diff
diff --git a/include/nsid.h b/include/nsid.h
--- a/include/nsid.h
+++ b/include/nsid.h
@@ -45,6 +45,9 @@
 int nsid_linear_fwd(const void* x, int ldx, const void* w, int w_dtype, const float* bias, void* out, int ldo, int M,
                     int Nout, int K, int groups, const float* in_scale, const float* in_shift, int act_in, int act_out,
                     float* stat, int ksplit, int act_dtype , void* stream);
+int nsid_linear_fwd_z(const void* x, int ldx, const void* w, int w_dtype, const float* bias, void* out, int ldo, int M,
+                      int Nout, int K, int groups, const float* in_scale, const float* in_shift, int act_in, int act_out,
+                      float* stat, int ksplit, int act_dtype, float* zero, long zero_floats, void* stream);
 int nsid_linear_fwd_res(const void* x, int ldx, const void* w, int w_dtype, const float* bias, const void* addend, int ldadd,
                         void* out, int ldo, int M, int Nout, int K, int groups, const float* in_scale,
                         const float* in_shift, int act_in, int act_dtype, void* stream);
@@ -55,6 +58,8 @@
 int nsid_linear_bwd_data(const void* dout, int ldd, const void* w, int w_dtype, const void* addend, int ldadd,
                          void* din, int ldi, int M, int Nout, int K, int groups,
                          int act_dtype , void* stream);
+int nsid_linear_bwd_data_z(const void* dout, int ldd, const void* w, int w_dtype, const void* addend, int ldadd,
+                           void* din, int ldi, int M, int Nout, int K, int groups, int act_dtype, void* stream);
 int nsid_linear_bwd_data_bn(const void* dout, int ldd, const void* w, int w_dtype, const void* addend, int ldadd,
                             void* din, int ldi, int M, int Nout, int K, int groups, int act_dtype, const void* bn_r,
                             const float* bn_scale, const float* bn_shift, const float* bn_mean, const float* bn_invstd,
@@ -83,6 +88,7 @@
 int nsid_bn_finalize(const float* stat, int tiles, int C, int M, const float* gamma, const float* beta,
                      float* running_mean, float* running_var, int64_t* num_batches_tracked, float momentum,
                      float eps, float* scale, float* shift, float* mean, float* invstd, void* stream);
+#define NSID_BN_RUN_LAYERS 64
 int nsid_bn_finalize_deferred(const float* stat, int tiles, int C, int M, const float* gamma, const float* beta, float eps,
                               float* scale, float* shift, float* mean, float* invstd, float* uvar, void* stream);
 int nsid_bn_running_update(int n, const int* C, float* const* running_mean, float* const* running_var,
@@ -154,6 +160,8 @@
 int nsid_node_mean_fwd(const void* x, int B, int N, int C, float* out, int x_dtype, void* stream);
 int nsid_node_mean_bwd(const float* dout, int B, int N, int C, void* dx, int dx_dtype, void* stream);
 int nsid_elu_bwd(const float* dout, const float* out, long n, float* din, void* stream);
+int nsid_node_mean_fwd_z(const void* x, int B, int N, int C, float* out, int x_dtype, float* zero, long zero_floats, void* stream);
+int nsid_elu_bwd_z(const float* dout, const float* out, long n, float* din, float* zero, long zero_floats, void* stream);
 int nsid_l2norm_fwd(const float* p, int B, int d, float eps, float* z, float* norm, void* stream);
 int nsid_l2norm_bwd(const float* dz, const float* z, const float* norm, int B, int d, float eps, float* dp,
                     void* stream);
diff --git a/neuralsampleid_amd/csrc/bn.hip b/neuralsampleid_amd/csrc/bn.hip
--- a/neuralsampleid_amd/csrc/bn.hip
+++ b/neuralsampleid_amd/csrc/bn.hip
@@ -340,14 +340,15 @@
 }
 
 namespace {
-constexpr int RU_LAYERS = 16;
+constexpr int RU_LAYERS = NSID_BN_RUN_LAYERS;
 struct RunUpdArgs {
   float* rm[RU_LAYERS]; float* rv[RU_LAYERS]; int64_t* nbt[RU_LAYERS];
   const float* mean_a[RU_LAYERS]; const float* uvar_a[RU_LAYERS];
   const float* mean_b[RU_LAYERS]; const float* uvar_b[RU_LAYERS];
-  int C[RU_LAYERS];
+  uint16_t C[RU_LAYERS];
   float momentum;
 };
+static_assert(sizeof(RunUpdArgs) + 256 <= 4096, "the layer table travels in the kernel arguments (4 KB with the 256 hidden bytes)");
 __global__ __launch_bounds__(256) void bn_running_update_kernel(const RunUpdArgs a) {
   const int l = blockIdx.x;
   const float m = a.momentum;
@@ -371,19 +372,22 @@
                                       const float* const* uvar_a, const float* const* mean_b,
                                       const float* const* uvar_b, float momentum, void* stream) {
   NSID_REQUIRE(n > 0 && C && running_mean && running_var && mean_a && uvar_a);
-  for (int base = 0; base < n; base += RU_LAYERS) {
+  const long tuned = nsid_tune(NSID_T_bn_run_chunk);
+  const int chunk = tuned < 1 ? 1 : (tuned > RU_LAYERS ? RU_LAYERS : (int)tuned);
+  for (int base = 0; base < n; base += chunk) {
     RunUpdArgs a{};
-    const int cnt = n - base < RU_LAYERS ? n - base : RU_LAYERS;
+    const int cnt = n - base < chunk ? n - base : chunk;
     for (int i = 0; i < cnt; ++i) {
-      NSID_REQUIRE(C[base + i] > 0 && running_mean[base + i] && running_var[base + i] && mean_a[base + i] && uvar_a[base + i]);
+      NSID_REQUIRE(C[base + i] > 0 && C[base + i] <= 65535 && running_mean[base + i] && running_var[base + i] && mean_a[base + i] && uvar_a[base + i]);
       a.rm[i] = running_mean[base + i]; a.rv[i] = running_var[base + i];
       a.nbt[i] = num_batches_tracked ? num_batches_tracked[base + i] : nullptr;
       a.mean_a[i] = mean_a[base + i]; a.uvar_a[i] = uvar_a[base + i];
       a.mean_b[i] = mean_b ? mean_b[base + i] : nullptr; a.uvar_b[i] = uvar_b ? uvar_b[base + i] : nullptr;
       NSID_REQUIRE((a.mean_b[i] == nullptr) == (a.uvar_b[i] == nullptr));
-      a.C[i] = C[base + i];
+      a.C[i] = (uint16_t)C[base + i];
     }
     a.momentum = momentum;
+    nsid_count(NSID_C_bn_running_update);
     NSID_LAUNCH(bn_running_update_kernel, dim3(cnt), dim3(256), 0, static_cast<hipStream_t>(stream), a);
     const int rc = nsid_launch_status();
     if (rc != NSID_OK) return rc;
diff --git a/neuralsampleid_amd/csrc/gemm.hip b/neuralsampleid_amd/csrc/gemm.hip
--- a/neuralsampleid_amd/csrc/gemm.hip
+++ b/neuralsampleid_amd/csrc/gemm.hip
@@ -738,8 +738,9 @@
   gemm_body<BM, BN, false, false, H, ST, false, false, FULL, false, FULL ? 2 : 1, PADX>(p, bid, split, g);
 }
 
-__global__ void elu_inplace_kernel(float* __restrict__ x, long rows, int cols, long ld) {
+__global__ void elu_inplace_kernel(float* __restrict__ x, long rows, int cols, long ld, f32x4* __restrict__ zero, long zero16) {
   const long n = rows * cols;
+  if (zero != nullptr) nsid_zero_fold(zero, zero16);
   for (long i = (long)blockIdx.x * blockDim.x + threadIdx.x; i < n; i += (long)gridDim.x * blockDim.x) {
     float* q = x + (i / cols) * ld + (i % cols);
     const float v = *q;
@@ -960,13 +961,22 @@
 static int linear_fwd_impl(const void* x, int ldx, const void* w, int w_dtype, const float* bias, void* out, int ldo,
                            int M, int Nout, int K, int groups, const float* in_scale, const float* in_shift, int act_in,
                            int act_out, float* stat, int ksplit, int act_dtype, const void* addend, int ldadd,
-                           void* stream);
+                           void* stream, float* zero = nullptr, long zero_floats = 0);
 
 extern "C" int nsid_linear_fwd(const void* x, int ldx, const void* w, int w_dtype, const float* bias, void* out, int ldo,
                                int M, int Nout, int K, int groups, const float* in_scale, const float* in_shift,
                                int act_in, int act_out, float* stat, int ksplit, int act_dtype, void* stream) {
   return linear_fwd_impl(x, ldx, w, w_dtype, bias, out, ldo, M, Nout, K, groups, in_scale, in_shift, act_in, act_out, stat,
                          ksplit, act_dtype, nullptr, 0, stream);
+}
+
+extern "C" int nsid_linear_fwd_z(const void* x, int ldx, const void* w, int w_dtype, const float* bias, void* out, int ldo,
+                                 int M, int Nout, int K, int groups, const float* in_scale, const float* in_shift,
+                                 int act_in, int act_out, float* stat, int ksplit, int act_dtype, float* zero, long zero_floats,
+                                 void* stream) {
+  NSID_REQUIRE(act_out == NSID_ACT_ELU && zero && zero != out && zero_floats > 0 && zero_floats % 4 == 0 && nsid_aligned16(zero));
+  return linear_fwd_impl(x, ldx, w, w_dtype, bias, out, ldo, M, Nout, K, groups, in_scale, in_shift, act_in, act_out, stat,
+                         ksplit, act_dtype, nullptr, 0, stream, zero, zero_floats);
 }
 
 extern "C" int nsid_linear_fwd_res(const void* x, int ldx, const void* w, int w_dtype, const float* bias,
@@ -982,7 +992,7 @@
 static int linear_fwd_impl(const void* x, int ldx, const void* w, int w_dtype, const float* bias, void* out, int ldo,
                            int M, int Nout, int K, int groups, const float* in_scale, const float* in_shift, int act_in,
                            int act_out, float* stat, int ksplit, int act_dtype, const void* addend, int ldadd,
-                           void* stream) {
+                           void* stream, float* zero, long zero_floats) {
   NSID_REQUIRE(x && w && out && M > 0 && Nout > 0 && K > 0 && groups > 0 && ksplit >= 1 && NSID_DTYPE_OK(act_dtype));
   NSID_REQUIRE(NSID_DTYPE_OK(w_dtype) && (w_dtype == NSID_F32 || (act_dtype == NSID_BF16 && K % 8 == 0)));
   const int ch = act_dtype == NSID_BF16 ? 8 : 4;
@@ -1035,7 +1045,8 @@
   if (rc != NSID_OK || act_out != NSID_ACT_ELU) return rc;
   const long n = (long)M * groups * Nout;
   NSID_LAUNCH(elu_inplace_kernel, dim3((int)((n + 255) / 256 > 2048 ? 2048 : (n + 255) / 256)), dim3(256), 0, s,
-              static_cast<float*>(out), (long)M, groups * Nout, (long)ldo);
+              static_cast<float*>(out), (long)M, groups * Nout, (long)ldo, reinterpret_cast<f32x4*>(zero), zero_floats / 4);
+  if (zero != nullptr) nsid_count(NSID_C_zero_fold);
   return nsid_launch_status();
 }
 
@@ -1045,13 +1056,21 @@
 static int linear_bwd_data_impl(const void* dout, int ldd, const void* w, int w_dtype, const void* addend, int ldadd,
                                 void* din, int ldi, int M, int Nout, int K, int groups, int act_dtype, void* stream,
                                 const void* bn_r, const float* bn_scale, const float* bn_shift, const float* bn_mean,
-                                const float* bn_invstd, int bn_act, float* bn_partial, const AbnArgs* abn = nullptr);
+                                const float* bn_invstd, int bn_act, float* bn_partial, const AbnArgs* abn = nullptr,
+                                bool din_zeroed = false);
 
 extern "C" int nsid_linear_bwd_data(const void* dout, int ldd, const void* w, int w_dtype, const void* addend, int ldadd,
                                     void* din, int ldi, int M, int Nout, int K, int groups, int act_dtype,
                                     void* stream) {
   return linear_bwd_data_impl(dout, ldd, w, w_dtype, addend, ldadd, din, ldi, M, Nout, K, groups, act_dtype, stream,
                               nullptr, nullptr, nullptr, nullptr, nullptr, NSID_ACT_NONE, nullptr);
+}
+
+extern "C" int nsid_linear_bwd_data_z(const void* dout, int ldd, const void* w, int w_dtype, const void* addend, int ldadd,
+                                      void* din, int ldi, int M, int Nout, int K, int groups, int act_dtype,
+                                      void* stream) {
+  return linear_bwd_data_impl(dout, ldd, w, w_dtype, addend, ldadd, din, ldi, M, Nout, K, groups, act_dtype, stream,
+                              nullptr, nullptr, nullptr, nullptr, nullptr, NSID_ACT_NONE, nullptr, nullptr, true);
 }
 
 extern "C" int nsid_linear_bwd_data_bn(const void* dout, int ldd, const void* w, int w_dtype, const void* addend,
@@ -1088,7 +1107,7 @@
 static int linear_bwd_data_impl(const void* dout, int ldd, const void* w, int w_dtype, const void* addend, int ldadd,
                                 void* din, int ldi, int M, int Nout, int K, int groups, int act_dtype, void* stream,
                                 const void* bn_r, const float* bn_scale, const float* bn_shift, const float* bn_mean,
-                                const float* bn_invstd, int bn_act, float* bn_partial, const AbnArgs* abn) {
+                                const float* bn_invstd, int bn_act, float* bn_partial, const AbnArgs* abn, bool din_zeroed) {
   NSID_REQUIRE(dout && w && din && M > 0 && Nout > 0 && K > 0 && groups > 0 && NSID_DTYPE_OK(act_dtype));
   NSID_REQUIRE(NSID_DTYPE_OK(w_dtype) && (w_dtype == NSID_F32 || (act_dtype == NSID_BF16 && K % 8 == 0)));
   const bool wb = w_dtype == NSID_BF16;
@@ -1134,7 +1153,7 @@
     const long maxt = nsid_tune(NSID_T_bwd_split_max_tiles);
     const long S = maxt > 0 && tiles <= maxt ? std::min<long>(256 / tiles, Nout / 256) : 1;
     if (S > 1) {
-      const int rcz = nsid_fill_zero(din, (size_t)M * K * 4, stream);
+      const int rcz = din_zeroed ? NSID_OK : nsid_fill_zero(din, (size_t)M * K * 4, stream);
       if (rcz != NSID_OK) return rcz;
       p.rsplit = (int)S;
       p.rchunk = (int)((Nout + S - 1) / S);
diff --git a/neuralsampleid_amd/csrc/misc.hip b/neuralsampleid_amd/csrc/misc.hip
--- a/neuralsampleid_amd/csrc/misc.hip
+++ b/neuralsampleid_amd/csrc/misc.hip
@@ -414,8 +414,9 @@
 
 template <typename T>
 __global__ __launch_bounds__(256) void node_mean_fwd_kernel(const T* __restrict__ x, int N, int C,
-                                                            float* __restrict__ out) {
+                                                            float* __restrict__ out, f32x4* __restrict__ zero, long zero16) {
   constexpr int NV = Chunk<T>::N;
+  if (zero != nullptr) nsid_zero_fold(zero, zero16);
   const int b = blockIdx.x, CV = C / NV;
   for (int cv = blockIdx.y * blockDim.x + threadIdx.x; cv < CV; cv += gridDim.y * blockDim.x) {
     float s[NV];
@@ -447,7 +448,8 @@
 }
 
 __global__ void elu_bwd_kernel(const float* __restrict__ dout, const float* __restrict__ out, long n,
-                               float* __restrict__ din) {
+                               float* __restrict__ din, f32x4* __restrict__ zero, long zero16) {
+  if (zero != nullptr) nsid_zero_fold(zero, zero16);
   for (long i = (long)blockIdx.x * blockDim.x + threadIdx.x; i < n; i += (long)gridDim.x * blockDim.x) {
     const float o = out[i];
     din[i] = dout[i] * (o > 0.f ? 1.f : o + 1.f);
@@ -695,15 +697,26 @@
   return nsid_launch_status();
 }
 
-extern "C" int nsid_node_mean_fwd(const void* x, int B, int N, int C, float* out, int x_dtype, void* stream) {
+static int node_mean_fwd_impl(const void* x, int B, int N, int C, float* out, int x_dtype, float* zero, long zero_floats,
+                              void* stream) {
   NSID_REQUIRE(x && out && B > 0 && N > 0 && C > 0 && NSID_DTYPE_OK(x_dtype) && nsid_aligned16(x));
   const int nv = x_dtype == NSID_BF16 ? 8 : 4;
   NSID_REQUIRE(C % nv == 0);
   NSID_DISPATCH_DTYPE(x_dtype, T, {
     NSID_LAUNCH((node_mean_fwd_kernel<T>), dim3(B, (C / nv + 255) / 256), dim3(256), 0,
-                static_cast<hipStream_t>(stream), static_cast<const T*>(x), N, C, out);
+                static_cast<hipStream_t>(stream), static_cast<const T*>(x), N, C, out, reinterpret_cast<f32x4*>(zero),
+                zero_floats / 4);
   });
   return nsid_launch_status();
+}
+extern "C" int nsid_node_mean_fwd(const void* x, int B, int N, int C, float* out, int x_dtype, void* stream) {
+  return node_mean_fwd_impl(x, B, N, C, out, x_dtype, nullptr, 0, stream);
+}
+extern "C" int nsid_node_mean_fwd_z(const void* x, int B, int N, int C, float* out, int x_dtype, float* zero, long zero_floats,
+                                    void* stream) {
+  NSID_REQUIRE(zero && zero != out && zero_floats > 0 && zero_floats % 4 == 0 && nsid_aligned16(zero));
+  nsid_count(NSID_C_zero_fold);
+  return node_mean_fwd_impl(x, B, N, C, out, x_dtype, zero, zero_floats, stream);
 }
 extern "C" int nsid_node_mean_bwd(const float* dout, int B, int N, int C, void* dx, int dx_dtype, void* stream) {
   NSID_REQUIRE(dout && dx && B > 0 && N > 0 && C > 0 && NSID_DTYPE_OK(dx_dtype) && nsid_aligned16(dx));
@@ -719,7 +732,16 @@
 extern "C" int nsid_elu_bwd(const float* dout, const float* out, long n, float* din, void* stream) {
   NSID_REQUIRE(dout && out && din && n > 0);
   NSID_LAUNCH(elu_bwd_kernel, dim3(grid_for(n)), dim3(256), 0, static_cast<hipStream_t>(stream), dout, out, n,
-                     din);
+                     din, static_cast<f32x4*>(nullptr), 0L);
+  return nsid_launch_status();
+}
+extern "C" int nsid_elu_bwd_z(const float* dout, const float* out, long n, float* din, float* zero, long zero_floats,
+                              void* stream) {
+  NSID_REQUIRE(dout && out && din && n > 0);
+  NSID_REQUIRE(zero && zero != din && zero_floats > 0 && zero_floats % 4 == 0 && nsid_aligned16(zero));
+  nsid_count(NSID_C_zero_fold);
+  NSID_LAUNCH(elu_bwd_kernel, dim3(grid_for(n)), dim3(256), 0, static_cast<hipStream_t>(stream), dout, out, n,
+                     din, reinterpret_cast<f32x4*>(zero), zero_floats / 4);
   return nsid_launch_status();
 }
 extern "C" int nsid_l2norm_fwd(const float* p, int B, int d, float eps, float* z, float* norm, void* stream) {
@@ -882,6 +904,7 @@
   NSID_REQUIRE(p && bytes > 0 && nsid_aligned16(p));
   const long n16 = (long)(bytes / 16);
   hipStream_t s = static_cast<hipStream_t>(stream);
+  nsid_count(NSID_C_fill_zero);
   if (n16 > 0) {
     NSID_LAUNCH(fill_zero_kernel, dim3(grid_for(n16, 2048)), dim3(256), 0, s, static_cast<f32x4*>(p), n16);
     if (nsid_launch_status() != NSID_OK) return NSID_ELAUNCH;
diff --git a/neuralsampleid_amd/csrc/nsid_common.h b/neuralsampleid_amd/csrc/nsid_common.h
--- a/neuralsampleid_amd/csrc/nsid_common.h
+++ b/neuralsampleid_amd/csrc/nsid_common.h
@@ -99,6 +99,12 @@
 
 __device__ __forceinline__ int lane_id() { return (int)__builtin_amdgcn_mbcnt_hi(~0u, __builtin_amdgcn_mbcnt_lo(~0u, 0u)); }
 __device__ __forceinline__ f32x4 ld4(const float* p) { return *reinterpret_cast<const f32x4*>(p); }
+
+__device__ __forceinline__ void nsid_zero_fold(f32x4* __restrict__ p, long n16) {
+  const long nthr = (long)gridDim.x * gridDim.y * blockDim.x;
+  const f32x4 z = {0.f, 0.f, 0.f, 0.f};
+  for (long q = ((long)blockIdx.y * gridDim.x + blockIdx.x) * blockDim.x + threadIdx.x; q < n16; q += nthr) p[q] = z;
+}
 
 template <int VM, int LGKM = 0xF>
 __device__ __forceinline__ void nsid_waitcnt() {
@@ -197,7 +203,9 @@
   X(wgg_w3, 1)                  \
   X(wgrad256, 1)                \
   X(wgg_rows256, 4096)          \
-  X(ws_gemm, 7)
+  X(ws_gemm, 7)                 \
+  X(ntxent_two_launch, 1)       \
+  X(bn_run_chunk, NSID_BN_RUN_LAYERS)
 
 enum NsidTuneKey {
 #define NSID_TUNE_ENUM(name, def) NSID_T_##name,
@@ -244,6 +252,10 @@
   X(logmel_fft_ragged) X(cqt_ragged) X(unfold_segments_ragged)    \
   X(song_vote) X(song_vote_clf) X(vote_candidates)    \
   X(pair_sim) X(local_align)    \
+  X(ntxent_two_launch) X(ntxent_multi_launch)    \
+  X(bn_running_update)     \
+  X(fill_zero)             \
+  X(zero_fold)             \
   X(flat_l2_topk_excl) X(flat_l2_topk_wide_excl)
 
 constexpr int NSID_STEM7_STAT_MAX = 1024;
diff --git a/neuralsampleid_amd/csrc/ntxent.hip b/neuralsampleid_amd/csrc/ntxent.hip
--- a/neuralsampleid_amd/csrc/ntxent.hip
+++ b/neuralsampleid_amd/csrc/ntxent.hip
@@ -79,8 +79,16 @@
 __global__ __launch_bounds__(256) void ntxent_lse_kernel(const float* __restrict__ z_i, const float* __restrict__ z_j,
                                                          int M, int d, float tau, int cols_per_group,
                                                          float* __restrict__ lse, float* __restrict__ rowloss,
-                                                         float* __restrict__ part_out) {
+                                                         float* __restrict__ part_out, float* __restrict__ zero_a,
+                                                         float* __restrict__ zero_b, long nzero) {
   extern __shared__ __attribute__((aligned(16))) float sm[];
+  if (zero_a != nullptr) {
+    const long nthr = (long)gridDim.x * gridDim.y * blockDim.x;
+    for (long q = ((long)blockIdx.y * gridDim.x + blockIdx.x) * blockDim.x + threadIdx.x; q < nzero; q += nthr) {
+      zero_a[q] = 0.f;
+      zero_b[q] = 0.f;
+    }
+  }
   const int ld = d + 4;
   float* zi_s = sm;
   float* zj_s = sm + RB * ld;
@@ -164,11 +172,9 @@
   }
 }
 
-__global__ void ntxent_lse_merge_kernel(const float* __restrict__ part, int groups, int M, float* __restrict__ lse,
-                                        float* __restrict__ rowloss) {
-  const int i = blockIdx.x * blockDim.x + threadIdx.x;
-  if (i >= M) return;
-  float m = -__builtin_inff(), sacc = 0.f, p = 0.f;
+__device__ __forceinline__ float merge_partials(const float* __restrict__ part, int groups, int M, int i, float& p) {
+  float m = -__builtin_inff(), sacc = 0.f;
+  p = 0.f;
   for (int g = 0; g < groups; ++g) {
     const float m2 = part[(long)g * 3 * M + i], s2 = part[(long)g * 3 * M + M + i];
     const float mn = fmaxf(m, m2);
@@ -178,21 +184,69 @@
     m = mn;
     p += part[(long)g * 3 * M + 2 * M + i];
   }
-  const float l = m + logf(sacc);
+  return m + logf(sacc);
+}
+
+__global__ void ntxent_lse_merge_kernel(const float* __restrict__ part, int groups, int M, float* __restrict__ lse,
+                                        float* __restrict__ rowloss) {
+  const int i = blockIdx.x * blockDim.x + threadIdx.x;
+  if (i >= M) return;
+  float p;
+  const float l = merge_partials(part, groups, M, i, p);
   lse[i] = l;
   rowloss[i] = l - p;
 }
 
-template <int DT>
+__device__ __forceinline__ void loss_mean(const float* rowloss, int row0, int nrows, int M, double* red,
+                                          float* __restrict__ loss_out) {
+  double s = 0.0;
+  for (int i = threadIdx.x; i < nrows; i += blockDim.x) s += (double)rowloss[row0 + i];
+  s = wave_sum_d(s);
+  if ((threadIdx.x & 63) == 0) red[threadIdx.x >> 6] = s;
+  __syncthreads();
+  if (threadIdx.x == 0) loss_out[0] = (float)((red[0] + red[1] + red[2] + red[3]) / (double)M);
+}
+
+constexpr int MERGE_MAX_M = 1024;
+
+template <int DT, bool MERGE>
 __global__ __launch_bounds__(256) void ntxent_grad_kernel(const float* __restrict__ z_i, const float* __restrict__ z_j,
                                                           int M, int d, float tau, const float* __restrict__ lse,
                                                           int row0, int nrows, int cols_per_group,
-                                                          float* __restrict__ dz_i, float* __restrict__ dz_j) {
+                                                          float* __restrict__ dz_i, float* __restrict__ dz_j,
+                                                          const float* __restrict__ part, int groups,
+                                                          float* __restrict__ lse_out, float* __restrict__ rowloss_out,
+                                                          float* __restrict__ loss_out) {
   extern __shared__ __attribute__((aligned(16))) float sm[];
   const int ld = d + 4;
   float* zi_s = sm;
   float* zj_s = sm + RB * ld;
+  float* lse_s = zj_s + CBK * ld + 4 * 3 * 16;
   const int i0 = row0 + blockIdx.x * RB;
+  const int jbeg = blockIdx.y * cols_per_group, jend = min(M, jbeg + cols_per_group);
+  if constexpr (MERGE) {
+    if (blockIdx.x == gridDim.x - 1) {
+      if (blockIdx.y != 0) return;
+      for (int r = threadIdx.x; r < M; r += blockDim.x) {
+        float p;
+        const float l = merge_partials(part, groups, M, r, p);
+        lse_out[r] = l;
+        rowloss_out[r] = l - p;
+        lse_s[r] = l - p;
+      }
+      __syncthreads();
+      loss_mean(lse_s, row0, nrows, M, reinterpret_cast<double*>(sm), loss_out);
+      return;
+    }
+    const int ncol = jend - jbeg;
+    for (int r = threadIdx.x; r < ncol + RB; r += blockDim.x) {
+      const int row = r < ncol ? jbeg + r : i0 + (r - ncol);
+      float p;
+      if (row < M) lse_s[row] = merge_partials(part, groups, M, row, p);
+    }
+    __syncthreads();
+    lse = lse_s;
+  }
   const int lane = threadIdx.x & 63, wave = threadIdx.x >> 6, lr = lane & 15, rq = lane >> 4;
   stage_rows(zi_s, ld, z_i, z_j, i0, RB, M, d);
   const int i = i0 + lr;
@@ -204,7 +258,6 @@
   constexpr int TPW = CBK / 16 / 4;
   const bool pipelined = CBK * (d >> 2) <= PF_MAX * 256;
   Prefetch pf;
-  const int jbeg = blockIdx.y * cols_per_group, jend = min(M, jbeg + cols_per_group);
   if (pipelined) {
     prefetch_rows(pf, z_i, z_j, jbeg, CBK, M, d);
     __syncthreads();
@@ -271,12 +324,7 @@
 __global__ __launch_bounds__(256) void ntxent_loss_kernel(const float* __restrict__ rowloss, int row0, int nrows, int M,
                                                           float* __restrict__ loss_out) {
   __shared__ double red[4];
-  double s = 0.0;
-  for (int i = threadIdx.x; i < nrows; i += blockDim.x) s += (double)rowloss[row0 + i];
-  s = wave_sum_d(s);
-  if ((threadIdx.x & 63) == 0) red[threadIdx.x >> 6] = s;
-  __syncthreads();
-  if (threadIdx.x == 0) loss_out[0] = (float)((red[0] + red[1] + red[2] + red[3]) / (double)M);
+  loss_mean(rowloss, row0, nrows, M, red, loss_out);
 }
 
 }
@@ -294,38 +342,48 @@
   float* rowloss = ws + M;
   hipStream_t s = static_cast<hipStream_t>(stream);
   const size_t bytes = ((size_t)(RB + CBK) * (d + 4) + 4 * 3 * 16) * sizeof(float);
-  {
-    const int row_tiles = (M + RB - 1) / RB, nblocks = (M + CBK - 1) / CBK;
-    int cg = row_tiles >= 512 ? 1 : (512 + row_tiles - 1) / row_tiles;
-    if (cg > nblocks) cg = nblocks;
-    if (cg > LSE_MAX_GROUPS) cg = LSE_MAX_GROUPS;
-    const int cols_per_group = (nblocks + cg - 1) / cg * CBK;
-    cg = (M + cols_per_group - 1) / cols_per_group;
-    float* part = ws + 2 * M + 8;
-    NSID_LAUNCH_LDS(ntxent_lse_kernel, dim3(row_tiles, cg), dim3(256), bytes, s, z_i, z_j, M, d, tau, cols_per_group, lse,
-                    rowloss, part);
+  const int row0 = 2 * p0, nrows = 2 * np;
+  const int nblocks = (M + CBK - 1) / CBK;
+  const int grad_tiles = (nrows + RB - 1) / RB;
+  int gcg = grad_tiles >= 128 ? 1 : (256 + grad_tiles - 1) / grad_tiles;
+  if (gcg > nblocks) gcg = nblocks;
+  const int grad_cols = (nblocks + gcg - 1) / gcg * CBK;
+  gcg = (M + grad_cols - 1) / grad_cols;
+  const int row_tiles = (M + RB - 1) / RB;
+  int cg = row_tiles >= 512 ? 1 : (512 + row_tiles - 1) / row_tiles;
+  if (cg > nblocks) cg = nblocks;
+  if (cg > LSE_MAX_GROUPS) cg = LSE_MAX_GROUPS;
+  const int cols_per_group = (nblocks + cg - 1) / cg * CBK;
+  cg = (M + cols_per_group - 1) / cols_per_group;
+  float* part = ws + 2 * M + 8;
+  const bool two = dz_i != nullptr && nsid_tune(NSID_T_ntxent_two_launch) != 0 && cg > 1 && gcg > 1 && M <= MERGE_MAX_M;
+  nsid_count(two ? NSID_C_ntxent_two_launch : NSID_C_ntxent_multi_launch);
+  float* const nozero = nullptr;
+  NSID_LAUNCH_LDS(ntxent_lse_kernel, dim3(row_tiles, cg), dim3(256), bytes, s, z_i, z_j, M, d, tau, cols_per_group, lse, rowloss,
+                  part, two ? dz_i : nozero, two ? dz_j : nozero, (long)np * d);
+  if (!two) {
     if (cg > 1) NSID_LAUNCH(ntxent_lse_merge_kernel, dim3((M + 255) / 256), dim3(256), 0, s, part, cg, M, lse, rowloss);
-  }
-  NSID_LAUNCH(ntxent_loss_kernel, dim3(1), dim3(256), 0, s, rowloss, 2 * p0, 2 * np, M, loss_out);
+    NSID_LAUNCH(ntxent_loss_kernel, dim3(1), dim3(256), 0, s, rowloss, row0, nrows, M, loss_out);
+  }
   if (dz_i != nullptr) {
-    const int row0 = 2 * p0, nrows = 2 * np;
-    const int row_tiles = (nrows + RB - 1) / RB, nblocks = (M + CBK - 1) / CBK;
-    int cg = row_tiles >= 128 ? 1 : (256 + row_tiles - 1) / row_tiles;
-    if (cg > nblocks) cg = nblocks;
-    const int cols_per_group = (nblocks + cg - 1) / cg * CBK;
-    cg = (M + cols_per_group - 1) / cols_per_group;
-    if (cg > 1) {
+    if (gcg > 1 && !two) {
       if (hipMemsetAsync(dz_i, 0, (size_t)np * d * sizeof(float), s) != hipSuccess ||
           hipMemsetAsync(dz_j, 0, (size_t)np * d * sizeof(float), s) != hipSuccess) {
         (void)nsid_launch_status();
         return NSID_ELAUNCH;
       }
     }
-    dim3 grid(row_tiles, cg);
-#define NSID_NTX_CASE(DTV)                                                                                   \
-  case DTV:                                                                                                  \
-    NSID_LAUNCH_LDS((ntxent_grad_kernel<DTV>), grid, dim3(256), bytes, s, z_i, z_j, M, d, tau, lse, row0,    \
-                    nrows, cols_per_group, dz_i, dz_j);                                                      \
+    const dim3 grid(grad_tiles + (two ? 1 : 0), gcg);
+    const size_t gbytes = bytes + (two ? MERGE_MAX_M * sizeof(float) : 0);
+    const float* const nopart = nullptr;
+#define NSID_NTX_CASE(DTV)                                                                                              \
+  case DTV:                                                                                                             \
+    if (two)                                                                                                            \
+      NSID_LAUNCH_LDS((ntxent_grad_kernel<DTV, true>), grid, dim3(256), gbytes, s, z_i, z_j, M, d, tau, lse, row0,      \
+                      nrows, grad_cols, dz_i, dz_j, (const float*)part, cg, lse, rowloss, loss_out);                    \
+    else                                                                                                                \
+      NSID_LAUNCH_LDS((ntxent_grad_kernel<DTV, false>), grid, dim3(256), gbytes, s, z_i, z_j, M, d, tau, lse, row0,     \
+                      nrows, grad_cols, dz_i, dz_j, nopart, 0, nozero, nozero, nozero);                                 \
     break;
     switch (d / 16) {
       NSID_NTX_CASE(1) NSID_NTX_CASE(2) NSID_NTX_CASE(4) NSID_NTX_CASE(8) NSID_NTX_CASE(16)
diff --git a/neuralsampleid_amd/functional.py b/neuralsampleid_amd/functional.py
--- a/neuralsampleid_amd/functional.py
+++ b/neuralsampleid_amd/functional.py
@@ -530,14 +530,16 @@
 
 HEAD_FC1_KSPLIT = 1
 HEAD_KSPLIT = True
+HEAD_ZERO_FOLD = 1
 
 
 def proj_mean_forward(x: Tensor, P, S: Optional[dict], B: int, N: int) -> Tensor:
     M, C = x.shape
     E = P["weight"].shape[0]
-    xm = ops.node_mean_fwd(x, B, N, C)
-    h, _ = ops.linear_fwd(xm, ops.w2d(P["weight"]), P["bias"], B, E, C,
-                          ksplit=4 if (HEAD_KSPLIT and S is not None and C >= 512 and B <= 512) else 1)
+    ks = 4 if (HEAD_KSPLIT and S is not None and C >= 512 and B <= 512) else 1
+    h = torch.empty((B, E), device=x.device, dtype=torch.float32) if (ks > 1 and HEAD_ZERO_FOLD and E % 4 == 0) else None
+    xm = ops.node_mean_fwd(x, B, N, C, zero=h)
+    h, _ = ops.linear_fwd(xm, ops.w2d(P["weight"]), P["bias"], B, E, C, ksplit=ks, out=h)
     if S is not None:
         S.update(xm=xm, B=B, N=N, C=C, xdtype=x.dtype)
     return h
@@ -555,10 +557,12 @@
 def projector_forward(h: Tensor, P, S: Optional[dict], eps: float = 1e-10) -> Tensor:
     B, Hin = h.shape
     Hid, D = P["0.weight"].shape[0], P["2.weight"].shape[0]
+    ks = 8 if (Hid >= 2048 and S is not None) else 1
+    p = torch.empty((B, D), device=h.device, dtype=torch.float32) if (ks > 1 and HEAD_ZERO_FOLD and D % 4 == 0) else None
     a1, _ = ops.linear_fwd(h, P["0.weight"], P["0.bias"], B, Hid, Hin, act_out=ACT_ELU,
-                           ksplit=HEAD_FC1_KSPLIT if (Hin >= 1024 and B <= 512 and h.dtype == torch.float32) else 1)
-    ks = 8 if (Hid >= 2048 and S is not None) else 1
-    p, _ = ops.linear_fwd(a1, P["2.weight"], P["2.bias"], B, D, Hid, ksplit=ks)
+                           ksplit=HEAD_FC1_KSPLIT if (Hin >= 1024 and B <= 512 and h.dtype == torch.float32) else 1,
+                           zero=p)
+    p, _ = ops.linear_fwd(a1, P["2.weight"], P["2.bias"], B, D, Hid, ksplit=ks, out=p)
     z, norm = ops.l2norm_fwd(p, eps)
     if S is not None:
         S.update(h=h, a1=a1, z=z, norm=norm, eps=eps)
@@ -573,10 +577,11 @@
     _wgrad(dp, a1, G["2.weight"], B, D, Hid)
     _bias_grad(dp, G["2.bias"])
     da1 = ops.linear_bwd_data(dp, P["2.weight"], B, D, Hid)
-    dpre = ops.elu_bwd(da1, a1)
+    dh = torch.empty((B, Hin), device=dz.device, dtype=torch.float32) if (HEAD_ZERO_FOLD and Hid >= 1024 and Hin % 4 == 0) else None
+    dpre = ops.elu_bwd(da1, a1, zero=dh)
     _wgrad(dpre, h, G["0.weight"], B, Hid, Hin)
     _bias_grad(dpre, G["0.bias"])
-    return ops.linear_bwd_data(dpre, P["0.weight"], B, Hid, Hin)
+    return ops.linear_bwd_data(dpre, P["0.weight"], B, Hid, Hin, out=dh, out_zeroed=dh is not None)
 
 
 def patchify_forward(spec: Tensor, P, S: Optional[dict], pb: int, pf: int) -> Tensor:
diff --git a/neuralsampleid_amd/ops.py b/neuralsampleid_amd/ops.py
--- a/neuralsampleid_amd/ops.py
+++ b/neuralsampleid_amd/ops.py
@@ -226,7 +226,7 @@
 
 
 def linear_fwd(x, w, bias, M, Nout, K, groups=1, in_scale=None, in_shift=None, act_in=ACT_NONE, act_out=ACT_NONE,
-               want_stat=False, ksplit=1, out=None, addend=None, in_aff=None) -> Tuple[torch.Tensor, Optional[torch.Tensor]]:
+               want_stat=False, ksplit=1, out=None, addend=None, in_aff=None, zero=None) -> Tuple[torch.Tensor, Optional[torch.Tensor]]:
     if in_aff is not None:
         in_scale, in_shift = in_aff.scale, in_aff.shift
     _chk(w, bias, in_scale, in_shift)
@@ -262,6 +262,13 @@
             "nsid_linear_fwd_res", _p(x), ldx, _p(wop), wdt, _p(bias), _p(addend), addend.shape[-1], _p(out),
             out.shape[-1], M, Nout, K, groups, _p(in_scale), _p(in_shift), act_in, dt, _stream()), (M, Nout, K, groups))
         return out, None
+    if zero is not None:
+        _chk(zero)
+        _timed(name, 2.0 * M * Nout * K * groups,
+               groups * (esz * M * K + float(wop.element_size()) * Nout * K + esz * M * Nout) + 4.0 * zero.numel(), lambda: call(
+            "nsid_linear_fwd_z", _p(x), ldx, _p(wop), wdt, _p(bias), _p(out), out.shape[-1], M, Nout, K, groups, _p(in_scale),
+            _p(in_shift), act_in, act_out, _p(stat), ksplit, dt, _p(zero), zero.numel(), _stream()), (M, Nout, K, groups))
+        return out, stat
     _timed(name, 2.0 * M * Nout * K * groups,
            groups * (esz * M * K + float(wop.element_size()) * Nout * K + esz * M * Nout), lambda: call(
         "nsid_linear_fwd", _p(x), ldx, _p(wop), wdt, _p(bias), _p(out), out.shape[-1], M, Nout, K, groups, _p(in_scale),
@@ -325,7 +332,7 @@
 FUSE_BN_BWD_REDUCE = True
 
 
-def linear_bwd_data(dout, w, M, Nout, K, groups=1, addend=None, out=None, bn=None):
+def linear_bwd_data(dout, w, M, Nout, K, groups=1, addend=None, out=None, bn=None, out_zeroed=False):
     _chk(w)
     dt = _act(dout, addend, out)
     if out is None:
@@ -356,8 +363,10 @@
             _p(aff.scale), _p(aff.shift), _p(aff.mean), _p(aff.invstd), act, _p(partial), _stream()),
             (M, Nout, K, groups))
         return out, partial
+    if out_zeroed and (fuse or out.shape[-1] != K or groups != 1):
+        raise ValueError("out_zeroed is for the plain backward-data GEMM of one group with a dense output")
     _timed(name, 2.0 * M * Nout * K * groups, nbytes, lambda: call(
-        "nsid_linear_bwd_data", _p(dout), dout.shape[-1], _p(wop), wdt, _p(addend),
+        "nsid_linear_bwd_data_z" if out_zeroed else "nsid_linear_bwd_data", _p(dout), dout.shape[-1], _p(wop), wdt, _p(addend),
         0 if addend is None else addend.shape[-1], _p(out), out.shape[-1], M, Nout, K, groups, dt, _stream()),
         (M, Nout, K, groups))
     return (out, None) if want_pair else out
@@ -604,6 +613,9 @@
     return BNAffine(buf[0], buf[1], buf[2], buf[3]), buf[4]
 
 
+BN_RUN_LAYERS = _H["NSID_BN_RUN_LAYERS"]
+
+
 def bn_running_update(layers_a, layers_b=None, momentum=BN_MOMENTUM) -> None:
     import ctypes
     n = len(layers_a)
@@ -990,8 +1002,13 @@
         out.shape[-1], _p(dw), _p(dbias), _act(out, dout), _stream()), (out.shape[0], out.shape[1], pb * pf * 3, 1))
 
 
-def node_mean_fwd(x, B, N, C) -> torch.Tensor:
+def node_mean_fwd(x, B, N, C, zero=None) -> torch.Tensor:
     out = torch.empty((B, C), device=x.device, dtype=torch.float32)
+    if zero is not None:
+        _chk(zero)
+        _tk("node_mean_fwd_kernel", float(x.element_size()) * B * N * C + 4.0 * zero.numel(), lambda: call(
+            "nsid_node_mean_fwd_z", _p(x), B, N, C, _p(out), _act(x), _p(zero), zero.numel(), _stream()), (B * N, C, 0, 1))
+        return out
     _tk("node_mean_fwd_kernel", float(x.element_size()) * B * N * C, lambda: call(
         "nsid_node_mean_fwd", _p(x), B, N, C, _p(out), _act(x), _stream()), (B * N, C, 0, 1))
     return out
@@ -1005,9 +1022,12 @@
     return dx
 
 
-def elu_bwd(dout, out) -> torch.Tensor:
-    _chk(dout, out)
+def elu_bwd(dout, out, zero=None) -> torch.Tensor:
+    _chk(dout, out, zero)
     din = torch.empty_like(dout)
+    if zero is not None:
+        call("nsid_elu_bwd_z", _p(dout), _p(out), out.numel(), _p(din), _p(zero), zero.numel(), _stream())
+        return din
     call("nsid_elu_bwd", _p(dout), _p(out), out.numel(), _p(din), _stream())
     return din
 
```
